# Young768/KungFu

Measured on AMD Instinct MI355X. Metric: images/sec/GPU ResNet-50 SynchronousSGD at 1/2/4/8 MI355X; scaling efficiency, higher is better.
Workload: dtype bf16

## Files before the change

csrc/kernels/bind_bn.cpp:

```cpp
#include "bind_util.hpp"

#include <vector>

using namespace kfb;

namespace {

const auto kCL = at::MemoryFormat::ChannelsLast;

kfk::BNShape bn_shape(const at::Tensor &x, const char *op) {
    check_cl4(x, op, "x", kAnyGpu);
    const int C = narrow(x.size(1), op, "x");
    TORCH_CHECK(kfk::bn_supported_channels(C), op, ": unsupported channel count ", C);
    return kfk::BNShape{x.numel() / C, C};
}

struct BNCommon {
    float *rm = nullptr, *rv = nullptr;
    int64_t *nbt = nullptr;
};

BNCommon bn_common(const char *op, int C, const Dev &dev, const at::Tensor &weight, const at::Tensor &bias,
                   const OptTensor &running_mean, const OptTensor &running_var, const OptTensor &num_batches,
                   bool training) {
    check_dense(weight, op, "weight", dev, at::kFloat, C);
    check_dense(bias, op, "bias", dev, at::kFloat, C);
    BNCommon b;
    if (has(running_mean)) {
        TORCH_CHECK(has(running_var), op, ": running_var missing");
        b.rm = running_mean->data_ptr<float>();
        b.rv = running_var->data_ptr<float>();
    }
    TORCH_CHECK(training || b.rm, op, ": eval mode needs running stats");
    if (training && has(num_batches)) {
        TORCH_CHECK(num_batches->scalar_type() == at::kLong && num_batches->numel() == 1 && num_batches->is_cuda(),
                    op, ": num_batches_tracked must be a 1-element int64 GPU tensor");
        b.nbt = num_batches->data_ptr<int64_t>();
    }
    return b;
}

at::Tensor bn_dy(at::Tensor dy, const at::Tensor &x, int C, int64_t *ld) {
    *ld = 0;
    if (dy.is_contiguous(kCL)) return dy;
    const int64_t s3 = dy.stride(3);
    const bool slice = dy.stride(1) == 1 && s3 >= C && s3 % 8 == 0 && dy.stride(2) == dy.size(3) * s3 &&
                       dy.stride(0) == dy.size(2) * dy.size(3) * s3 &&
                       reinterpret_cast<uintptr_t>(dy.data_ptr()) % 16 == 0;
    if (!slice) return dy.contiguous(kCL);
    *ld = s3;
    return dy;
}

void check_bn_dy(const at::Tensor &dy, const at::Tensor &x, const char *op) {
    TORCH_CHECK(dy.scalar_type() == at::kBFloat16 && dy.sizes() == x.sizes() && dy.device() == x.device(), op,
                ": dy must be a bf16 tensor of x's shape on its device");
}

std::vector<std::vector<at::Tensor>> bn_finalize_multi(std::vector<at::Tensor> xs, std::vector<at::Tensor> sums,
                                                       std::vector<at::Tensor> weights, std::vector<at::Tensor> biases,
                                                       std::vector<OptTensor> running_means,
                                                       std::vector<OptTensor> running_vars,
                                                       std::vector<OptTensor> num_batches,
                                                       std::vector<double> momentum, std::vector<double> eps) {
    const char *op = "bn_finalize_multi";
    const size_t n = xs.size();
    TORCH_CHECK(n >= 1 && n <= static_cast<size_t>(kfk::kBnFinMax) && sums.size() == n && weights.size() == n &&
                    biases.size() == n && running_means.size() == n && running_vars.size() == n &&
                    num_batches.size() == n && momentum.size() == n && eps.size() == n,
                "bn_finalize_multi: 1..8 BNs, every list of the same length");
    kfk::BnFinBatch b{};
    b.n = static_cast<int>(n);
    for (size_t i = 0; i < n; ++i) {
        auto sh = bn_shape(xs[i], op);
        const Dev dev = xs[0].device();
        TORCH_CHECK(xs[i].device() == *dev, "bn_finalize_multi: xs must be on one device");
        auto c = bn_common(op, sh.channels, dev, weights[i], biases[i], running_means[i], running_vars[i],
                           num_batches[i], true);
        kfk::BnFinDesc &d = b.d[i];
        TORCH_CHECK(sums[i].defined(), "bn_finalize_multi: sums must be defined");
        d.sums = stats_ptr(sums[i], op, sh.channels, dev, "sums");
        d.gamma = weights[i].data_ptr<float>(), d.beta = biases[i].data_ptr<float>();
        d.run_mean = c.rm, d.run_var = c.rv, d.nbt = c.nbt;
        d.rows = sh.rows, d.C = sh.channels;
        d.momentum = static_cast<float>(momentum[i]), d.eps = static_cast<float>(eps[i]);
    }
    std::vector<std::vector<at::Tensor>> out;
    for (size_t i = 0; i < n; ++i) {
        kfk::BnFinDesc &d = b.d[i];
        auto fopt = xs[i].options().dtype(at::kFloat);
        at::Tensor mean = at::empty({d.C}, fopt), invstd = at::empty({d.C}, fopt), coef = at::empty({2 * d.C}, fopt);
        d.mean = mean.data_ptr<float>(), d.invstd = invstd.data_ptr<float>(), d.coef = coef.data_ptr<float>();
        out.push_back({mean, invstd, coef});
    }
    c10::DeviceGuard gd(xs[0].device());
    kfk::launch_bn_sums_finalize_multi(b, stream_of(xs[0], 0));
    return out;
}

std::vector<at::Tensor> bn_forward(at::Tensor x, OptTensor res, at::Tensor weight, at::Tensor bias,
                                   OptTensor running_mean, OptTensor running_var, double momentum, double eps,
                                   bool training, bool relu, OptTensor num_batches, OptTensor sums, OptTensor res_coef,
                                   bool apply, OptTensor out, c10::optional<std::vector<at::Tensor>> pre) {
    const char *op = "bn_forward";
    auto sh = bn_shape(x, op);
    const int C = sh.channels;
    const Dev dev = x.device();
    auto b = bn_common(op, C, dev, weight, bias, running_mean, running_var, num_batches, training);
    const uint16_t *rp = nullptr;
    if (has(res)) {
        check_cl4(*res, op, "res", dev, x.sizes());
        rp = bf16(*res);
    }
    const float *rc = nullptr;
    if (has(res_coef)) {
        TORCH_CHECK(rp, "bn_forward: res_coef (the residual BN's f32 [scale(C); shift(C)]) needs res");
        check_dense(*res_coef, op, "res_coef", dev, at::kFloat, 2 * C);
        rc = res_coef->data_ptr<float>();
    }
    int64_t y_ld = 0;
    if (has(out)) {
        TORCH_CHECK(apply && !rp && relu && out->scalar_type() == at::kBFloat16 && out->sizes() == x.sizes() &&
                        out->stride(1) == 1 && out->stride(3) >= C && out->stride(3) % 8 == 0 &&
                        out->stride(2) == out->size(3) * out->stride(3) &&
                        out->stride(0) == out->size(2) * out->stride(2) &&
                        reinterpret_cast<uintptr_t>(out->data_ptr()) % 16 == 0 && out->device() == x.device(),
                    "bn_forward: out must be a 16-byte aligned channel slice of a channels_last bf16 tensor "
                    "(BN+ReLU, no residual)");
        y_ld = out->stride(3);
    }
    const bool prefin = pre.has_value();
    if (prefin) {
        TORCH_CHECK(pre->size() == 3 && training && has(sums), "bn_forward: pre must be (mean, invstd, coef) with sums");
        check_dense((*pre)[0], op, "pre[0]", dev, at::kFloat, C);
        check_dense((*pre)[1], op, "pre[1]", dev, at::kFloat, C);
        check_dense((*pre)[2], op, "pre[2]", dev, at::kFloat, 2 * C);
    }
    double *sp = training ? stats_ptr(sums, op, C, dev, "sums") : nullptr;

    c10::DeviceGuard gd(x.device());
    auto fopt = x.options().dtype(at::kFloat);
    at::Tensor y;
    if (has(out)) y = *out;
    else if (apply) y = at::empty_like(x, kCL);
    at::Tensor mean, invstd, coef;
    if (prefin) mean = (*pre)[0], invstd = (*pre)[1], coef = (*pre)[2];
    else mean = at::empty({C}, fopt), invstd = at::empty({C}, fopt), coef = at::empty({2 * C}, fopt);
    at::Tensor mask;
    if (apply && rp && relu) mask = at::empty({sh.rows * (C / 8)}, x.options().dtype(at::kByte));
    at::Tensor partial;
    if (training && !sp) partial = at::empty({2 * static_cast<int64_t>(kfk::bn_num_chunks(sh)) * C}, fopt);
    kfk::launch_bn_forward(bf16(x), rp, weight.data_ptr<float>(), bias.data_ptr<float>(),
                           apply ? bf16_mut(y) : nullptr, mask.defined() ? mask.data_ptr<uint8_t>() : nullptr, sh, relu,
                           training, b.rm, b.rv, static_cast<float>(momentum), static_cast<float>(eps),
                           partial.defined() ? partial.data_ptr<float>() : nullptr, mean.data_ptr<float>(),
                           invstd.data_ptr<float>(), coef.data_ptr<float>(), b.nbt, stream_of(x, 0), sp, rc, apply, y_ld,
                           prefin);
    return {y, mean, invstd, coef, mask};
}

std::vector<at::Tensor> bn_backward(at::Tensor dy, at::Tensor x, at::Tensor mean, at::Tensor invstd, at::Tensor weight,
                                    at::Tensor fcoef, OptTensor mask, bool relu, bool training, bool want_dres,
                                    OptTensor sums, OptTensor dres_x, OptTensor dres_sums) {
    const char *op = "bn_backward";
    auto sh = bn_shape(x, op);
    const int C = sh.channels;
    const Dev dev = x.device();
    check_bn_dy(dy, x, op);
    check_dense(mean, op, "mean", dev, at::kFloat, C);
    check_dense(invstd, op, "invstd", dev, at::kFloat, C);
    check_dense(weight, op, "weight", dev, at::kFloat, C);
    check_dense(fcoef, op, "fcoef", dev, at::kFloat, 2 * C);
    const uint8_t *mp = nullptr;
    if (has(mask)) {
        check_dense(*mask, op, "mask", dev, at::kByte, sh.rows * (C / 8));
        mp = mask->data_ptr<uint8_t>();
    }
    double *sp = stats_ptr(sums, op, C, dev, "sums");
    const uint16_t *dsx = nullptr;
    double *dsp = nullptr;
    if (has(dres_x)) {
        TORCH_CHECK(want_dres && has(dres_sums),
                    "bn_backward: dres_x (second BN's input) needs want_dres and its f64 sums workspace dres_sums");
        check_cl4(*dres_x, op, "dres_x", dev, x.sizes());
        dsx = bf16(*dres_x);
        dsp = stats_ptr(dres_sums, op, C, dev, "dres_sums");
    }
    c10::DeviceGuard gd(x.device());
    int64_t dy_ld;
    dy = bn_dy(dy, x, C, &dy_ld);
    auto fopt = x.options().dtype(at::kFloat);
    auto dx = at::empty_like(x, kCL);
    at::Tensor dres;
    if (want_dres) dres = at::empty_like(x, kCL);
    at::Tensor dw = at::empty({C}, fopt), db = at::empty({C}, fopt), coef = at::empty({3 * C}, fopt);
    at::Tensor partial;
    if (!sp) partial = at::empty({2 * static_cast<int64_t>(kfk::bn_num_chunks(sh)) * C}, fopt);
    kfk::launch_bn_backward(bf16(dy), bf16(x), fcoef.data_ptr<float>(), mp, mean.data_ptr<float>(),
                            invstd.data_ptr<float>(), weight.data_ptr<float>(), sh, relu, training,
                            partial.defined() ? partial.data_ptr<float>() : nullptr, dw.data_ptr<float>(),
                            db.data_ptr<float>(), coef.data_ptr<float>(), bf16_mut(dx),
                            want_dres ? bf16_mut(dres) : nullptr, stream_of(x, 0), sp, dsx, dsp, dy_ld);
    return {dx, dres, dw, db};
}

std::vector<std::vector<at::Tensor>> bn_backward_multi(std::vector<at::Tensor> dys, std::vector<at::Tensor> xs,
                                                       std::vector<at::Tensor> means, std::vector<at::Tensor> invstds,
                                                       std::vector<at::Tensor> weights, std::vector<at::Tensor> fcoefs) {
    const char *op = "bn_backward_multi";
    const size_t n = xs.size();
    TORCH_CHECK(n >= 1 && n <= static_cast<size_t>(kfk::kBnFinMax) && dys.size() == n && means.size() == n &&
                    invstds.size() == n && weights.size() == n && fcoefs.size() == n,
                "bn_backward_multi: 1..8 BNs, every list of the same length");
    struct Piece {
        at::Tensor dy, dx, dw, db, coef, partial;
        int64_t ld;
        kfk::BNShape sh;
    };
    std::vector<Piece> ps(n);
    const Dev dev = xs[0].device();
    for (size_t i = 0; i < n; ++i) {
        ps[i].sh = bn_shape(xs[i], op);
        const int C = ps[i].sh.channels;
        TORCH_CHECK(xs[i].device() == *dev, "bn_backward_multi: xs must be on one device");
        check_bn_dy(dys[i], xs[i], op);
        check_dense(fcoefs[i], op, "fcoefs", dev, at::kFloat, 2 * C);
        check_dense(means[i], op, "means", dev, at::kFloat, C);
        check_dense(invstds[i], op, "invstds", dev, at::kFloat, C);
        check_dense(weights[i], op, "weights", dev, at::kFloat, C);
    }
    c10::DeviceGuard gd(xs[0].device());
    kfk::BnBwdFinBatch fb{};
    fb.n = static_cast<int>(n);
    for (size_t i = 0; i < n; ++i) {
        Piece &p = ps[i];
        const int C = p.sh.channels;
        p.dy = bn_dy(dys[i], xs[i], C, &p.ld);
        auto fopt = xs[i].options().dtype(at::kFloat);
        p.dx = at::empty_like(xs[i], kCL);
        p.dw = at::empty({C}, fopt), p.db = at::empty({C}, fopt), p.coef = at::empty({3 * C}, fopt);
        p.partial = at::empty({2 * static_cast<int64_t>(kfk::bn_num_chunks(p.sh)) * C}, fopt);
        kfk::BnBwdFinDesc &d = fb.d[i];
        d.partial = p.partial.data_ptr<float>();
        d.nchunks = kfk::bn_num_chunks(p.sh), d.C = C, d.rows = p.sh.rows;
        d.gamma = weights[i].data_ptr<float>(), d.mean = means[i].data_ptr<float>(), d.invstd = invstds[i].data_ptr<float>();
        d.dgamma = p.dw.data_ptr<float>(), d.dbeta = p.db.data_ptr<float>(), d.coef = p.coef.data_ptr<float>();
    }
    const hipStream_t st = stream_of(xs[0], 0);
    for (int phase : {1, 2}) {
        if (phase == 2) kfk::launch_bn_bwd_finalize_multi(fb, st);
        for (size_t i = 0; i < n; ++i) {
            Piece &p = ps[i];
            kfk::launch_bn_backward(bf16(p.dy), bf16(xs[i]), fcoefs[i].data_ptr<float>(), nullptr,
                                    means[i].data_ptr<float>(), invstds[i].data_ptr<float>(),
                                    weights[i].data_ptr<float>(), p.sh, true, true, p.partial.data_ptr<float>(),
                                    p.dw.data_ptr<float>(), p.db.data_ptr<float>(), p.coef.data_ptr<float>(),
                                    bf16_mut(p.dx), nullptr, st, nullptr, nullptr, nullptr, p.ld, phase);
        }
    }
    std::vector<std::vector<at::Tensor>> out;
    for (auto &p : ps) out.push_back({p.dx, p.dw, p.db});
    return out;
}

std::vector<at::Tensor> bn_pool_forward(at::Tensor x, at::Tensor weight, at::Tensor bias, OptTensor running_mean,
                                        OptTensor running_var, double momentum, double eps, bool training,
                                        OptTensor num_batches, OptTensor sums) {
    const char *op = "bn_pool_forward";
    auto sh = bn_shape(x, op);
    const int C = sh.channels;
    const Dev dev = x.device();
    const int H = narrow(x.size(2), op, "x"), W = narrow(x.size(3), op, "x");
    TORCH_CHECK(kfk::bn_pool_supported(sh, H, W), "bn_pool_forward: unsupported shape");
    double *sp = training ? stats_ptr(sums, op, C, dev, "sums") : nullptr;
    auto b = bn_common(op, C, dev, weight, bias, running_mean, running_var, num_batches, training);
    c10::DeviceGuard gd(x.device());
    auto fopt = x.options().dtype(at::kFloat);
    const int OH = kfk::pool_out(H), OW = kfk::pool_out(W);
    auto yp = at::empty({x.size(0), C, OH, OW}, x.options().memory_format(kCL));
    auto arg = at::empty({x.size(0) * OH * OW * C}, x.options().dtype(at::kByte));
    auto mean = at::empty({C}, fopt), invstd = at::empty({C}, fopt), coef = at::empty({2 * C}, fopt);
    at::Tensor partial, xarg;
    if (training) {
        partial = at::empty({2 * static_cast<int64_t>(kfk::bn_num_chunks(sh)) * C}, fopt);
        xarg = at::empty_like(yp, kCL);
    }
    kfk::launch_bn_pool_forward(bf16(x), weight.data_ptr<float>(), bias.data_ptr<float>(), bf16_mut(yp),
                                arg.data_ptr<uint8_t>(), sh, H, W, training, b.rm, b.rv, static_cast<float>(momentum),
                                static_cast<float>(eps), training ? partial.data_ptr<float>() : nullptr,
                                mean.data_ptr<float>(), invstd.data_ptr<float>(), coef.data_ptr<float>(), b.nbt,
                                stream_of(x, 0), sp, xarg.defined() ? bf16_mut(xarg) : nullptr);
    return {yp, mean, invstd, coef, arg, xarg};
}

std::vector<at::Tensor> bn_pool_backward(at::Tensor dyp, at::Tensor arg, at::Tensor x, at::Tensor mean,
                                         at::Tensor invstd, at::Tensor weight, at::Tensor fcoef, bool training,
                                         OptTensor xarg, bool apply) {
    const char *op = "bn_pool_backward";
    auto sh = bn_shape(x, op);
    const int C = sh.channels;
    const Dev dev = x.device();
    const int H = narrow(x.size(2), op, "x"), W = narrow(x.size(3), op, "x");
    const int64_t psz[4] = {x.size(0), C, kfk::pool_out(H), kfk::pool_out(W)};
    TORCH_CHECK(dyp.scalar_type() == at::kBFloat16 && dyp.sizes() == at::IntArrayRef(psz) && dyp.device() == x.device(),
                "bn_pool_backward: dy must be the pooled [N, C, PH, PW] bf16 gradient on x's device");
    check_dense(arg, op, "arg", dev, at::kByte, dyp.numel());
    check_dense(mean, op, "mean", dev, at::kFloat, C);
    check_dense(invstd, op, "invstd", dev, at::kFloat, C);
    check_dense(weight, op, "weight", dev, at::kFloat, C);
    check_dense(fcoef, op, "fcoef", dev, at::kFloat, 2 * C);
    const bool pooled = training && has(xarg);
    if (pooled) check_cl4(*xarg, op, "xarg", dev, psz);
    c10::DeviceGuard gd(x.device());
    if (!dyp.is_contiguous(kCL)) dyp = dyp.contiguous(kCL);
    auto fopt = x.options().dtype(at::kFloat);
    auto dx = apply ? at::empty_like(x, kCL) : at::empty({0}, x.options());
    auto dw = at::empty({C}, fopt), db = at::empty({C}, fopt), coef = at::empty({3 * C}, fopt);
    auto partial = at::empty({2 * static_cast<int64_t>(kfk::bn_num_chunks(sh)) * C}, fopt);
    at::Tensor sums;
    if (pooled) sums = at::zeros({2 * C * kfk::kStatSlots}, x.options().dtype(at::kDouble));
    kfk::launch_bn_pool_backward(bf16(dyp), arg.data_ptr<uint8_t>(), bf16(x), fcoef.data_ptr<float>(),
                                 mean.data_ptr<float>(), invstd.data_ptr<float>(), weight.data_ptr<float>(), sh, H, W,
                                 training, partial.data_ptr<float>(), dw.data_ptr<float>(), db.data_ptr<float>(),
                                 coef.data_ptr<float>(), apply ? bf16_mut(dx) : nullptr, stream_of(x, 0),
                                 pooled ? bf16(*xarg) : nullptr, pooled ? sums.data_ptr<double>() : nullptr, apply);
    return {dx, dw, db, coef};
}

}

void bind_bn(py::module_ &m) {
    m.def("bn_supported_channels", &kfk::bn_supported_channels);
    m.def("bn_forward", &bn_forward,
          "fused NHWC BN(+residual)(+ReLU) forward -> (y, mean, invstd, coef, relu mask or None)", py::arg("x"),
          py::arg("res"), py::arg("weight"), py::arg("bias"), py::arg("running_mean"), py::arg("running_var"),
          py::arg("momentum"), py::arg("eps"), py::arg("training"), py::arg("relu"),
          py::arg("num_batches") = py::none(), py::arg("sums") = py::none(), py::arg("res_coef") = py::none(),
          py::arg("apply") = true, py::arg("out") = py::none(), py::arg("pre") = py::none());
    m.def("bn_backward_multi", &bn_backward_multi,
          "backward of several BN+ReLUs (slices of one concatenation's gradient): one batched finalize");
    m.def("bn_finalize_multi", &bn_finalize_multi,
          "batched sums-finalize of several training BNs in one launch -> [[mean, invstd, coef], ...]");
    m.def("bn_backward", &bn_backward, "fused NHWC BN(+residual)(+ReLU) backward -> (dx, dres, dweight, dbias)",
          py::arg("dy"), py::arg("x"), py::arg("mean"), py::arg("invstd"), py::arg("weight"), py::arg("fcoef"),
          py::arg("mask"), py::arg("relu"), py::arg("training"), py::arg("want_dres"), py::arg("sums") = py::none(),
          py::arg("dres_x") = py::none(), py::arg("dres_sums") = py::none());
    m.def("bn_pool_supported", [](int64_t C, int64_t H, int64_t W) {
        const char *op = "bn_pool_supported";
        return kfk::bn_pool_supported(kfk::BNShape{H * W, narrow(C, op, "C")}, narrow(H, op, "H"), narrow(W, op, "W"));
    });
    m.def("bn_pool_forward", &bn_pool_forward,
          "stem BN+ReLU+MaxPool(3,2,1) forward -> (y_pool, mean, invstd, coef, argmax)", py::arg("x"),
          py::arg("weight"), py::arg("bias"), py::arg("running_mean"), py::arg("running_var"), py::arg("momentum"),
          py::arg("eps"), py::arg("training"), py::arg("num_batches") = py::none(), py::arg("sums") = py::none());
    m.def("bn_pool_backward", &bn_pool_backward, "stem BN+ReLU+MaxPool backward -> (dx, dweight, dbias, coef)",
          py::arg("dy"), py::arg("arg"), py::arg("x"), py::arg("mean"), py::arg("invstd"), py::arg("weight"),
          py::arg("fcoef"), py::arg("training"), py::arg("xarg") = py::none(), py::arg("apply") = true);
}
```

csrc/kernels/bind_conv.cpp:

```cpp
#include "bind_util.hpp"

#include <array>
#include <optional>
#include <vector>

using namespace kfb;

namespace {

const auto kCL = at::MemoryFormat::ChannelsLast;

at::Tensor conv(at::Tensor x, at::Tensor w, int64_t stride, OptTensor stats, OptTensor out, int64_t variant,
                OptTensor bn_x, OptTensor bn_fcoef, OptTensor bn_mask, OptTensor bias, bool gate, OptTensor acc_mask,
                bool acc_even) {
    const char *op = "conv";
    check_cl4(x, op, "x", kAnyGpu);
    const Dev dev = x.device();
    check_cl4(w, op, "w", dev);
    TORCH_CHECK(w.size(2) == w.size(3) && w.size(1) == x.size(1), "conv: w must be [Cout, Cin, KS, KS] with x's Cin");
    const auto [N, C, H, W] = dims4(x, op, "x");
    const int K = narrow(w.size(0), op, "w"), ks = narrow(w.size(2), op, "w"), st = narrow(stride, op, "stride");
    TORCH_CHECK(kfk::conv_supported(C, K, ks, st), "conv: unsupported channels/kernel/stride");
    const int pad = (ks - 1) / 2;
    const int OH = (H + 2 * pad - ks) / st + 1, OW = (W + 2 * pad - ks) / st + 1;
    TORCH_CHECK(OH > 0 && OW > 0, "conv: empty output");
    check_extent32(op, "x", {N, H, W, C});
    check_extent32(op, "the output", {N, OH, OW, K});
    const int64_t ysz[4] = {N, K, OH, OW};
    const int64_t ynumel = c10::multiply_integers(at::IntArrayRef(ysz));
    double *sp = stats_ptr(stats, op, K, dev);
    const bool accum = has(out), bwd = has(bn_x);
    kfk::EpiArgs ea;
    ea.stats = sp;
    int epi = accum ? kfk::kEpiAccum : 0;
    if (has(bias)) {
        TORCH_CHECK(!accum && !sp && !bwd && !gate, "conv: bias epilogue excludes out/stats/bn_x/gate");
        check_dense(*bias, op, "bias", dev, at::kBFloat16, K);
        ea.bias = bf16(*bias);
        epi = kfk::kEpiBiasRelu;
    } else if (gate) {
        TORCH_CHECK(!accum && sp && bwd && !has(bn_mask) && !has(bn_fcoef),
                    "conv: gate needs stats and bn_x (the ReLU output), no out/bn_mask/bn_fcoef");
        check_cl4(*bn_x, op, "bn_x", dev, ysz);
        ea.bx = bf16(*bn_x);
        epi = kfk::kEpiGate;
    } else if (bwd) {
        epi |= bn_bwd_epilogue(op, ea, ysz, K, dev, sp, bn_x, bn_fcoef, bn_mask);
    } else if (sp) {
        epi |= kfk::kEpiFwdStats;
    }
    TORCH_CHECK(!(epi & kfk::kEpiFwdStats) || !(epi & kfk::kEpiAccum), "conv: stats + accumulate unsupported");
    if (has(acc_mask)) {
        TORCH_CHECK(accum && !(epi & kfk::kEpiBwdCoef), "conv: acc_mask needs out and excludes bn_fcoef");
        check_dense(*acc_mask, op, "acc_mask", dev, at::kByte, ynumel / 8);
        ea.amask = acc_mask->data_ptr<uint8_t>();
        epi |= kfk::kEpiAccMask;
    }
    if (acc_even) {
        TORCH_CHECK(accum && st == 1 && !(epi & (kfk::kEpiAccMask | kfk::kEpiBwdCoef)),
                    "conv: acc_even needs out, stride 1 and no acc_mask / bn_fcoef");
        epi |= kfk::kEpiAccEven;
    }
    const int var = narrow(variant, op, "variant");
    c10::DeviceGuard gd(x.device());
    auto y = out_or_empty(out, ysz, x.options().memory_format(kCL), op).first;
    kfk::launch_conv(bf16(x), bf16(w), bf16_mut(y), N, H, W, C, K, ks, st, ea, epi, stream_of(x, 0), var);
    return y;
}

std::vector<at::Tensor> gemm(at::Tensor x, at::Tensor w, OptTensor bias, OptTensor out, OptTensor gelu_u,
                             OptTensor stats, int64_t variant) {
    const char *op = "gemm";
    TORCH_CHECK(x.dim() == 2, "gemm: x must be 2-D [M, K]");
    check_dense(x, op, "x", kAnyGpu, at::kBFloat16, x.numel());
    const Dev dev = x.device();
    TORCH_CHECK(w.dim() == 2 && w.size(1) == x.size(1), "gemm: w must be 2-D [N, K] with x's K");
    check_dense(w, op, "w", dev, at::kBFloat16, w.numel());
    const int64_t M = x.size(0), K = x.size(1), N = w.size(0);
    TORCH_CHECK(M < (int64_t(1) << 31) && K < (int64_t(1) << 31) && N < (int64_t(1) << 31) &&
                    kfk::gemm_supported(static_cast<int>(M), static_cast<int>(K), static_cast<int>(N)),
                "gemm: unsupported shape (K, N multiples of 64)");
    kfk::EpiArgs ea;
    int epi = 0;
    auto check_mn = [&](const at::Tensor &t, const char *what) {
        TORCH_CHECK(t.dim() == 2 && t.size(0) == M && t.size(1) == N, "gemm: ", what, " must be 2-D [M, N]");
        check_dense(t, op, what, dev, at::kBFloat16, M * N);
    };
    if (has(out)) {
        TORCH_CHECK(!has(bias) && !has(gelu_u), "gemm: out (accumulate) excludes bias / gelu_u");
        check_mn(*out, "out");
        epi = kfk::kEpiAccum;
    }
    if (has(bias)) {
        check_dense(*bias, op, "bias", dev, at::kBFloat16, N);
        ea.bias = bf16(*bias);
        epi = kfk::kEpiBias;
    }
    if (has(gelu_u)) {
        TORCH_CHECK(epi == 0, "gemm: gelu_u excludes bias / out");
        check_mn(*gelu_u, "gelu_u");
        TORCH_CHECK(has(stats), "gemm: stats must be given with gelu_u (the f64 kStatSlots x 2 x N workspace)");
        ea.bx = bf16(*gelu_u);
        ea.stats = stats_ptr(stats, op, N, dev);
        epi = kfk::kEpiGeluGrad;
    }
    const int var = narrow(variant, op, "variant");
    c10::DeviceGuard gd(x.device());
    auto y = out_or_empty(out, {M, N}, x.options(), op).first;
    kfk::launch_gemm(bf16(x), bf16(w), bf16_mut(y), static_cast<int>(M), static_cast<int>(K), static_cast<int>(N), ea,
                     epi, stream_of(x, 0), var);
    return {y};
}

at::Tensor conv_dgrad_s2(at::Tensor dy, at::Tensor wt, int64_t ks, OptTensor stats, OptTensor bn_x, OptTensor bn_fcoef,
                         OptTensor bn_mask, int64_t variant, int64_t dh, int64_t dw, int64_t pad) {
    const char *op = "conv_dgrad_s2";
    check_cl4(dy, op, "dy", kAnyGpu);
    const Dev dev = dy.device();
    TORCH_CHECK(ks == 1 || ks == 3, "conv_dgrad_s2: ks must be 1 or 3");
    check_cl4(wt, op, "wt", dev);
    check_cl4(wt, op, "wt", dev, {wt.size(0), dy.size(1), ks, ks});
    const auto [N, K, OH, OW] = dims4(dy, op, "dy");
    const int C = narrow(wt.size(0), op, "wt");
    if (dh <= 0) {
        TORCH_CHECK(kfk::conv_supported(K, C, static_cast<int>(ks), 1), "conv_dgrad_s2: unsupported channels");
        dh = 2 * OH, dw = 2 * OW, pad = ks == 3 ? 1 : 0;
    } else {
        TORCH_CHECK(ks == 3 && (pad == 0 || pad == 1) && K % 8 == 0 && C % 8 == 0 && K >= 16 && C >= 16 && dw > 0 &&
                        (dh + 2 * pad - 3) / 2 + 1 == OH && (dw + 2 * pad - 3) / 2 + 1 == OW,
                    "conv_dgrad_s2: dh/dw/pad do not match a 3x3 stride-2 convolution of dy's size (channels % 8)");
    }
    check_extent32(op, "dx", {N, dh, dw, C});
    const int64_t dxsz[4] = {N, C, dh, dw};
    kfk::EpiArgs ea;
    int epi = 0;
    if (has(bn_x)) {
        TORCH_CHECK(ks == 3, "conv_dgrad_s2: BN sums need every pixel (ks = 3)");
        epi = bn_bwd_epilogue(op, ea, dxsz, C, dev, stats_ptr(stats, op, C, dev), bn_x, bn_fcoef, bn_mask);
    }
    const int var = narrow(variant, op, "variant");
    c10::DeviceGuard gd(dy.device());
    auto dx = at::empty(dxsz, dy.options().memory_format(kCL));
    kfk::launch_conv_dgrad_s2(bf16(dy), bf16(wt), bf16_mut(dx), N, OH, OW, K, C, static_cast<int>(ks), ea, epi,
                              stream_of(dy, 0), var, static_cast<int>(dh), static_cast<int>(dw), static_cast<int>(pad));
    return dx;
}

at::Tensor wgrad_launch(const char *op, const at::Tensor &dy, const at::Tensor &x, const kfk::WgradPlan &plan,
                        OptTensor out, bool accumulate, bool atomics) {
    const kfk::WgradShape &sh = plan.shape;
    const bool f32 = has(out) && out->scalar_type() == at::kFloat;
    c10::DeviceGuard gd(x.device());
    auto dw = out_or_empty(out, {sh.Cout, sh.Cin, sh.kh, sh.kw},
                           x.options().dtype(f32 ? at::kFloat : at::kBFloat16).memory_format(kCL), op).first;
    at::Tensor ws;
    if (plan.ws_floats > 0) ws = at::empty({plan.ws_floats}, x.options().dtype(at::kFloat));
    kfk::launch_conv_wgrad(bf16(dy), bf16(x), dw.data_ptr(), plan.ws_floats > 0 ? ws.data_ptr<float>() : nullptr, plan,
                           f32, accumulate, stream_of(x, 0), atomics);
    return dw;
}

void wgrad_check(const char *op, const at::Tensor &dy, const at::Tensor &x, const kfk::WgradShape &sh) {
    check_cl4(dy, op, "dy", x.device(), {sh.N, sh.Cout, sh.OH(), sh.OW()});
    check_extent32(op, "x", {sh.N, sh.H, sh.W, sh.Cin});
    check_extent32(op, "dy", {sh.N, sh.OH(), sh.OW(), sh.Cout});
}

at::Tensor conv_wgrad(at::Tensor dy, at::Tensor x, int64_t ks, int64_t stride, OptTensor out, bool accumulate,
                      int64_t variant, int64_t splits, bool atomics) {
    const char *op = "conv_wgrad";
    check_cl4(x, op, "x", kAnyGpu);
    check_cl4(dy, op, "dy", Dev(x.device()));
    const auto [N, C, H, W] = dims4(x, op, "x");
    const auto sh = kfk::wgrad_square_shape(N, H, W, C, narrow(dy.size(1), op, "dy"), narrow(ks, op, "ks"),
                                            narrow(stride, op, "stride"));
    TORCH_CHECK(kfk::conv_wgrad_supported(sh.Cin, sh.Cout, sh.kh, sh.stride), "conv_wgrad: unsupported channels/kernel/stride");
    wgrad_check(op, dy, x, sh);
    TORCH_CHECK(has(out) || !accumulate, "conv_wgrad: accumulate needs out");
    const auto plan = kfk::conv_wgrad_plan(sh, kfk::WgradFamily::Square, narrow(variant, op, "variant"),
                                           narrow(splits, op, "splits"));
    return wgrad_launch(op, dy, x, plan, out, accumulate, atomics);
}

at::Tensor conv_wgrad_rect(at::Tensor dy, at::Tensor x, int64_t kh, int64_t kw, int64_t stride, int64_t ph, int64_t pw,
                           int64_t variant) {
    const char *op = "conv_wgrad_rect";
    check_cl4(x, op, "x", kAnyGpu);
    check_cl4(dy, op, "dy", Dev(x.device()));
    const auto [N, C, H, W] = dims4(x, op, "x");
    const kfk::WgradShape sh{N, H, W, C, narrow(dy.size(1), op, "dy"), narrow(kh, op, "kh"), narrow(kw, op, "kw"),
                             narrow(ph, op, "ph"), narrow(pw, op, "pw"), narrow(stride, op, "stride")};
    TORCH_CHECK(kfk::conv_wgrad_rect_supported(sh.Cin, sh.Cout, sh.kh, sh.kw, sh.stride) && sh.ph >= 0 && sh.pw >= 0 &&
                    sh.ph < sh.kh && sh.pw < sh.kw,
                "conv_wgrad_rect: unsupported channels/window/stride/padding");
    wgrad_check(op, dy, x, sh);
    const auto plan = kfk::conv_wgrad_plan(sh, kfk::WgradFamily::Rect, narrow(variant, op, "variant"));
    return wgrad_launch(op, dy, x, plan, OptTensor(), false, true);
}

at::Tensor conv_flip_weight(at::Tensor w) {
    const char *op = "conv_flip_weight";
    check_cl4(w, op, "w", kAnyGpu);
    const auto [K, C, kh, kw] = dims4(w, op, "w");
    c10::DeviceGuard gd(w.device());
    auto wt = at::empty({C, K, kh, kw}, w.options().memory_format(kCL));
    kfk::launch_conv_flip_weight_taps(bf16(w), bf16_mut(wt), K, C, kh * kw, stream_of(w, 0));
    return wt;
}

at::Tensor conv_rect(at::Tensor x, at::Tensor w, int64_t stride, int64_t ph, int64_t pw, OptTensor stats, OptTensor out,
                     OptTensor bn_x, OptTensor bn_fcoef) {
    const char *op = "conv_rect";
    check_cl4(x, op, "x", kAnyGpu);
    const Dev dev = x.device();
    check_cl4(w, op, "w", dev);
    TORCH_CHECK(w.size(1) == x.size(1), "conv_rect: w must be [Cout, Cin, KH, KW] with x's Cin");
    const auto [N, C, H, W] = dims4(x, op, "x");
    const auto [K, wc, kh, kw] = dims4(w, op, "w");
    const int st = narrow(stride, op, "stride"), PH = narrow(ph, op, "ph"), PW = narrow(pw, op, "pw");
    TORCH_CHECK(kfk::conv_rect_supported(C, K, kh, kw, st) && PH >= 0 && PW >= 0 && PH < kh && PW < kw,
                "conv_rect: unsupported channels/window/stride/padding");
    const int OH = (H + 2 * PH - kh) / st + 1, OW = (W + 2 * PW - kw) / st + 1;
    TORCH_CHECK(OH > 0 && OW > 0, "conv_rect: empty output");
    check_extent32(op, "x", {N, H, W, C});
    check_extent32(op, "the output", {N, OH, OW, K});
    const int64_t ysz[4] = {N, K, OH, OW};
    kfk::EpiArgs ea;
    ea.stats = stats_ptr(stats, op, K, dev);
    int epi = ea.stats ? kfk::kEpiFwdStats : 0;
    const bool bwd = has(bn_x);
    if (bwd) epi = bn_bwd_epilogue(op, ea, ysz, K, dev, ea.stats, bn_x, bn_fcoef, OptTensor());
    TORCH_CHECK(!has(out) || epi == 0 || bwd, "conv_rect: out must not be combined with forward stats");
    c10::DeviceGuard gd(x.device());
    auto [y, accum] = out_or_empty(out, ysz, x.options().memory_format(kCL), op);
    if (accum) epi |= kfk::kEpiAccum;
    kfk::launch_conv_rect(bf16(x), bf16(w), bf16_mut(y), N, H, W, C, K, kh, kw, PH, PW, st, ea, epi, stream_of(x, 0));
    return y;
}

void conv_flip_weights(std::vector<at::Tensor> srcs, std::vector<at::Tensor> dsts) {
    const char *op = "conv_flip_weights";
    TORCH_CHECK(srcs.size() == dsts.size(), "conv_flip_weights: length mismatch");
    if (srcs.empty()) return;
    c10::DeviceGuard gd(srcs[0].device());
    auto s = stream_of(srcs[0], 0);
    kfk::FlipTable tab;
    tab.start[0] = 0;
    for (size_t i = 0; i < srcs.size(); ++i) {
        const auto &w = srcs[i];
        const auto &d = dsts[i];
        check_cl4(w, op, "srcs", i ? Dev(srcs[0].device()) : kAnyGpu);
        check_cl4(d, op, "dsts", w.device(), {w.size(1), w.size(0), w.size(2), w.size(3)});
        const auto [K, C, kh, kw] = dims4(w, op, "srcs");
        const int k = tab.n;
        tab.src[k] = bf16(w);
        tab.dst[k] = bf16_mut(d);
        tab.cout[k] = K;
        tab.cin[k] = C;
        tab.taps[k] = kh * kw;
        tab.start[k + 1] = tab.start[k] + w.numel();
        tab.n = k + 1;
        if (tab.n == kfk::FlipTable::kMax) {
            kfk::launch_conv_flip_multi(tab, s);
            tab.n = 0;
        }
    }
    kfk::launch_conv_flip_multi(tab, s);
}

}

void bind_conv(py::module_ &m) {
    m.def("conv", &conv, "1x1/3x3 NHWC bf16 convolution (MFMA implicit GEMM) with fused BN-statistics and "
          "accumulate epilogues", py::arg("x"), py::arg("w"), py::arg("stride") = 1, py::arg("stats") = py::none(),
          py::arg("out") = py::none(), py::arg("variant") = -1, py::arg("bn_x") = py::none(),
          py::arg("bn_fcoef") = py::none(), py::arg("bn_mask") = py::none(), py::arg("bias") = py::none(),
          py::arg("gate") = false, py::arg("acc_mask") = py::none(), py::arg("acc_even") = false);
    m.def("conv_variants", &kfk::conv_variants);
    m.def("conv_supported", &kfk::conv_supported);
    m.attr("conv_stat_slots") = kfk::kStatSlots;
    m.def("conv_rect", &conv_rect, "KH x KW NHWC bf16 convolution with zero padding (MFMA implicit GEMM; "
          "Inception-v3 windows) with an optional BN-statistics epilogue", py::arg("x"), py::arg("w"),
          py::arg("stride") = 1, py::arg("ph") = 0, py::arg("pw") = 0, py::arg("stats") = py::none(),
          py::arg("out") = py::none(), py::arg("bn_x") = py::none(), py::arg("bn_fcoef") = py::none());
    m.def("conv_rect_supported", &kfk::conv_rect_supported);
    m.def("gemm", &gemm, "linear layer x @ w^T on the MFMA kernel with bias / GELU-gradient(+bias-gradient "
          "sums) / accumulate epilogues", py::arg("x"), py::arg("w"), py::arg("bias") = py::none(),
          py::arg("out") = py::none(), py::arg("gelu_u") = py::none(),
          py::arg("stats") = py::none(), py::arg("variant") = -1);
    m.def("gemm_supported", &kfk::gemm_supported);
    m.def("conv_dgrad_s2", &conv_dgrad_s2, "data gradient of a stride-2 1x1/3x3 NHWC bf16 convolution (parity-phase "
          "MFMA implicit GEMMs)", py::arg("dy"), py::arg("wt"), py::arg("ks"), py::arg("stats") = py::none(),
          py::arg("bn_x") = py::none(), py::arg("bn_fcoef") = py::none(), py::arg("bn_mask") = py::none(),
          py::arg("variant") = -1, py::arg("dh") = 0, py::arg("dw") = 0, py::arg("pad") = 1);
    m.def("conv_wgrad_rect", &conv_wgrad_rect, "weight gradient of a KH x KW padded NHWC bf16 convolution "
          "(split-K MFMA GEMM, any channel count % 8)", py::arg("dy"), py::arg("x"), py::arg("kh"), py::arg("kw"),
          py::arg("stride") = 1, py::arg("ph") = 0, py::arg("pw") = 0, py::arg("variant") = -1);
    m.def("conv_wgrad", &conv_wgrad, "weight gradient of the 1x1/3x3 NHWC bf16 convolution (split-K MFMA GEMM)",
          py::arg("dy"), py::arg("x"), py::arg("ks"), py::arg("stride") = 1, py::arg("out") = py::none(),
          py::arg("accumulate") = false, py::arg("variant") = -1, py::arg("splits") = -1,
          py::arg("atomics") = true);
    m.def("conv_wgrad_supported", &kfk::conv_wgrad_supported);
    m.def("conv_wgrad_rect_supported", &kfk::conv_wgrad_rect_supported);
    m.def("conv_wgrad_variants", [] { return kfk::kWgradSquareVariants; });
    m.def("conv_wgrad_rows_rect_supported", [](int N, int H, int W, int Cin, int Cout, int kh, int kw, int ph, int pw,
                                               int stride) {
        return kfk::conv_wgrad_rows_rect_supported({N, H, W, Cin, Cout, kh, kw, ph, pw, stride});
    }, "a row-image weight-gradient kernel covers this multi-tap window (args: N, H, W, Cin, Cout, kh, kw, ph, pw, stride)");
    m.def("conv_wgrad_rows_rect_auto", [](int N, int H, int W, int Cin, int Cout, int kh, int kw, int ph, int pw,
                                          int stride) {
        return kfk::conv_wgrad_rows_rect_auto({N, H, W, Cin, Cout, kh, kw, ph, pw, stride});
    }, "the row-image variant conv_wgrad_rect(..., WGRAD_ROWS_AUTO) picks for this shape (args: N, H, W, Cin, Cout, kh, "
       "kw, ph, pw, stride)");
    m.def("conv_wgrad_plan", [](int N, int H, int W, int Cin, int Cout, int ks, int stride, int variant, int splits,
                                std::optional<std::array<int, 4>> window) {
        const auto p = window ? kfk::conv_wgrad_plan({N, H, W, Cin, Cout, (*window)[0], (*window)[1], (*window)[2],
                                                      (*window)[3], stride}, kfk::WgradFamily::Rect, variant)
                              : kfk::conv_wgrad_plan(kfk::wgrad_square_shape(N, H, W, Cin, Cout, ks, stride),
                                                     kfk::WgradFamily::Square, variant, splits);
        return py::make_tuple(p.variant, p.splits, p.kps, p.ws_floats, kfk::wgrad_kernel_name(p.kernel));
    }, "(variant, splits, kps, ws_floats, kernel) of conv_wgrad's plan, or with window = (kh, kw, ph, pw) of "
       "conv_wgrad_rect's (ks and splits are then unused)", py::arg("N"), py::arg("H"), py::arg("W"), py::arg("Cin"),
          py::arg("Cout"), py::arg("ks"), py::arg("stride"), py::arg("variant") = -1, py::arg("splits") = -1,
          py::arg("window") = py::none());
    m.def("conv_wgrad_route", [](int N, int H, int W, int Cin, int Cout, int kh, int kw, int ph, int pw, int stride) {
        const auto r = kfk::conv_wgrad_route({N, H, W, Cin, Cout, kh, kw, ph, pw, stride});
        return py::make_tuple(kfk::wgrad_route_name(r.route), r.variant, r.max_pixels);
    }, "(route, variant, max_pixels): 'library', or the family ('square': conv_wgrad, 'rect': conv_wgrad_rect) and the "
       "variant code that take this convolution's weight gradient, and the output pixels one launch handles",
          py::arg("N"), py::arg("H"), py::arg("W"), py::arg("Cin"), py::arg("Cout"), py::arg("kh"), py::arg("kw"),
          py::arg("ph"), py::arg("pw"), py::arg("stride"));
    m.attr("WGRAD_AUTO") = static_cast<int>(kfk::kWgradAuto);
    m.attr("WGRAD_TILE_128x128") = static_cast<int>(kfk::kWgradTile128x128);
    m.attr("WGRAD_TILE_128x64") = static_cast<int>(kfk::kWgradTile128x64);
    m.attr("WGRAD_TILE_64x128") = static_cast<int>(kfk::kWgradTile64x128);
    m.attr("WGRAD_TILE_64x64") = static_cast<int>(kfk::kWgradTile64x64);
    m.attr("WGRAD_TILE_256x128") = static_cast<int>(kfk::kWgradTile256x128);
    m.attr("WGRAD_TILE_128x256") = static_cast<int>(kfk::kWgradTile128x256);
    m.attr("WGRAD_ROWS") = static_cast<int>(kfk::kWgradRows);
    m.attr("WGRAD_TILE_256x256") = static_cast<int>(kfk::kWgradTile256x256);
    m.attr("WGRAD_RING_32x2") = static_cast<int>(kfk::kWgradRing32x2);
    m.attr("WGRAD_RING_32x3") = static_cast<int>(kfk::kWgradRing32x3);
    m.attr("WGRAD_RING_32x4") = static_cast<int>(kfk::kWgradRing32x4);
    m.attr("WGRAD_RING_64x3") = static_cast<int>(kfk::kWgradRing64x3);
    m.attr("WGRAD_RING_64x4") = static_cast<int>(kfk::kWgradRing64x4);
    m.attr("WGRAD_ROWS_AUTO") = static_cast<int>(kfk::kWgradRowsAuto);
    m.def("conv_flip_weight", &conv_flip_weight, "w[co,ci,kh,kw] -> w[ci,co,KS-1-kh,KS-1-kw] (data-gradient weights)");
    m.def("conv_flip_weights", &conv_flip_weights, "multi-tensor conv_flip_weight into preallocated outputs");
}
```

csrc/kernels/bind_util.hpp:

```cpp
#pragma once

#include <ATen/hip/HIPContext.h>
#include <c10/core/DeviceGuard.h>
#include <torch/extension.h>

#include "kernels.hpp"

#include <climits>
#include <initializer_list>
#include <utility>

namespace kfb {

using OptTensor = c10::optional<at::Tensor>;
using Dev = c10::optional<at::Device>;
inline const Dev kAnyGpu{};

inline int dtype_code(const at::Tensor &t) {
    switch (t.scalar_type()) {
    case at::kByte: return 0;
    case at::kChar: return 4;
    case at::kInt: return 6;
    case at::kLong: return 7;
    case at::kHalf: return 8;
    case at::kBFloat16: return 9;
    case at::kFloat: return 10;
    case at::kDouble: return 11;
    case at::kBool: return 12;
    default: TORCH_CHECK(false, "kungfu_amd._hip: unsupported dtype ", t.scalar_type());
    }
    return -1;
}

inline hipStream_t stream_of(const at::Tensor &t, int64_t stream) {
    if (stream) return reinterpret_cast<hipStream_t>(stream);
    return c10::hip::getCurrentHIPStream(t.device().index()).stream();
}

inline void check_gpu(const at::Tensor &t, const char *name) {
    TORCH_CHECK(t.is_cuda(), name, " must be a GPU tensor");
    TORCH_CHECK(t.is_contiguous(), name, " must be contiguous");
}

inline void hcheck(hipError_t e, const char *what) {
    TORCH_CHECK(e == hipSuccess, "hip ", what, ": ", hipGetErrorString(e));
}

inline bool has(const OptTensor &o) { return o && o->defined(); }

inline const uint16_t *bf16(const at::Tensor &t) { return reinterpret_cast<const uint16_t *>(t.data_ptr()); }
inline uint16_t *bf16_mut(const at::Tensor &t) { return reinterpret_cast<uint16_t *>(t.data_ptr()); }

inline int narrow(int64_t v, const char *op, const char *what) {
    TORCH_CHECK(v >= INT_MIN && v <= INT_MAX, op, ": ", what, " must be a 32-bit integer, got ", v);
    return static_cast<int>(v);
}

inline bool on_dev(const at::Tensor &t, const Dev &dev) { return dev ? t.device() == *dev : t.is_cuda(); }
inline const char *where(const Dev &dev) { return dev ? "on the leading tensor's device" : "on a GPU"; }

inline void check_cl4(const at::Tensor &t, const char *op, const char *name, const Dev &dev,
                      at::ScalarType dt = at::kBFloat16) {
    TORCH_CHECK(t.dim() == 4 && t.scalar_type() == dt && t.is_contiguous(at::MemoryFormat::ChannelsLast) &&
                    on_dev(t, dev),
                op, ": ", name, " must be a 4-D channels_last ", dt, " tensor ", where(dev));
}

inline void check_cl4(const at::Tensor &t, const char *op, const char *name, const Dev &dev, at::IntArrayRef nchw,
                      at::ScalarType dt = at::kBFloat16) {
    TORCH_CHECK(t.dim() == 4 && t.scalar_type() == dt && t.is_contiguous(at::MemoryFormat::ChannelsLast) &&
                    on_dev(t, dev) && t.sizes() == nchw,
                op, ": ", name, " must be a ", nchw, " channels_last ", dt, " tensor ", where(dev));
}

struct Dims4 {
    int n, c, h, w;
};
inline Dims4 dims4(const at::Tensor &t, const char *op, const char *name) {
    return {narrow(t.size(0), op, name), narrow(t.size(1), op, name), narrow(t.size(2), op, name),
            narrow(t.size(3), op, name)};
}

inline void check_dense(const at::Tensor &t, const char *op, const char *name, const Dev &dev, at::ScalarType dt,
                        int64_t numel, bool at_least = false) {
    TORCH_CHECK(t.scalar_type() == dt && t.is_contiguous() && (at_least ? t.numel() >= numel : t.numel() == numel) &&
                    on_dev(t, dev),
                op, ": ", name, " must be a contiguous ", dt, " tensor of ", at_least ? "at least " : "", numel,
                " elements ", where(dev));
}

inline double *stats_ptr(const OptTensor &o, const char *op, int64_t C, const Dev &dev, const char *name = "stats") {
    if (!has(o)) return nullptr;
    check_dense(*o, op, name, dev, at::kDouble, kfk::kStatSlots * 2 * C);
    return o->data_ptr<double>();
}

inline void check_extent32(const char *op, const char *name, std::initializer_list<int64_t> dims) {
    int64_t n = 1;
    for (int64_t d : dims) {
        TORCH_CHECK(d >= 0 && d <= INT_MAX, op, ": ", name, " too large for 32-bit offsets");
        n *= d;
        TORCH_CHECK(n <= INT_MAX, op, ": ", name, " too large for 32-bit offsets");
    }
}

inline int bn_bwd_epilogue(const char *op, kfk::EpiArgs &ea, at::IntArrayRef y_sizes, int64_t K, const Dev &dev,
                           double *stats, const OptTensor &bn_x, const OptTensor &bn_fcoef, const OptTensor &bn_mask) {
    if (!has(bn_x)) return 0;
    TORCH_CHECK(stats, op, ": stats must be given with bn_x (it receives the BN-backward sums)");
    check_cl4(*bn_x, op, "bn_x", dev, y_sizes);
    ea.stats = stats;
    ea.bx = bf16(*bn_x);
    if (has(bn_mask)) {
        check_dense(*bn_mask, op, "bn_mask", dev, at::kByte, c10::multiply_integers(y_sizes) / 8);
        ea.bmask = bn_mask->data_ptr<uint8_t>();
        return kfk::kEpiBwdBits;
    }
    TORCH_CHECK(has(bn_fcoef), op, ": bn_fcoef must be given with bn_x (forward [scale; shift], f32) unless bn_mask is");
    check_dense(*bn_fcoef, op, "bn_fcoef", dev, at::kFloat, 2 * K, true);
    ea.fcoef = bn_fcoef->data_ptr<float>();
    return kfk::kEpiBwdCoef;
}

inline std::pair<at::Tensor, bool> out_or_empty(const OptTensor &out, at::IntArrayRef sizes, const at::TensorOptions &opt,
                                                const char *op, const char *name = "out") {
    if (!has(out)) return {at::empty(sizes, opt), false};
    const auto dt = c10::typeMetaToScalarType(opt.dtype());
    if (opt.memory_format_opt() == at::MemoryFormat::ChannelsLast) check_cl4(*out, op, name, opt.device(), sizes, dt);
    else check_dense(*out, op, name, opt.device(), dt, c10::multiply_integers(sizes));
    return {*out, true};
}

}
```

csrc/kernels/bn.hip:

```cpp
#include "bn_fin.hpp"
#include "common.hpp"
#include "kernels.hpp"

#include <cstdlib>
#include <stdexcept>

namespace kfk {

namespace {

__device__ __forceinline__ void unpack8(const uint4 &v, float (&f)[8]) {
    const uint32_t w[4] = {v.x, v.y, v.z, v.w};
#pragma unroll
    for (int i = 0; i < 4; ++i) {
        f[2 * i] = __uint_as_float(w[i] << 16);
        f[2 * i + 1] = __uint_as_float(w[i] & 0xffff0000u);
    }
}

__device__ __forceinline__ uint4 pack8(const float (&f)[8]) {
    uint32_t w[4];
#pragma unroll
    for (int i = 0; i < 4; ++i)
        w[i] = pack_bf16x2(f[2 * i], f[2 * i + 1]);
// ... 328 lines not shown
        sc[k] = coef[cv * 8 + k];
        sh[k] = coef[C + cv * 8 + k];
    }
    const int64_t stride = static_cast<int64_t>(gridDim.x) * bn_threads<CVEC>();
    for (int64_t i = tid; i < nout_vec; i += stride) {
        const int64_t p = i / CVEC;
        const int ow = static_cast<int>(p % OW);
        const int64_t t = p / OW;
        const int oh = static_cast<int>(t % OH);
        const int64_t n = t / OH;
        float best[8], xb[8];
        uint32_t a[8];
#pragma unroll
        for (int k = 0; k < 8; ++k) {
            best[k] = -1.f;
            a[k] = 0;
            xb[k] = 0.f;
        }
#pragma unroll
        for (int kh = 0; kh < 3; ++kh) {
            const int h = 2 * oh - 1 + kh;
            if (h < 0 || h >= H) continue;
#pragma unroll
            for (int kw = 0; kw < 3; ++kw) {
                const int w = 2 * ow - 1 + kw;
                if (w < 0 || w >= W) continue;
                float f[8];
                unpack8(x[((n * H + h) * W + w) * CVEC + cv], f);
#pragma unroll
                for (int k = 0; k < 8; ++k) {
                    float v = f[k] * sc[k] + sh[k];
                    v = v > 0.f ? v : 0.f;
                    if (v > best[k]) {
                        best[k] = v;
                        a[k] = kh * 3 + kw;
                        xb[k] = f[k];
                    }
                }
            }
        }
        yp[i] = pack8(best);
        arg[i] = make_uint2(a[0] | (a[1] << 8) | (a[2] << 16) | (a[3] << 24),
                            a[4] | (a[5] << 8) | (a[6] << 16) | (a[7] << 24));
        if (xarg) xarg[i] = pack8(xb);
    }
}

template <int CVEC>
__global__ __launch_bounds__(kBlock) void bn_pool_bwd_sums_kernel(const uint4 *__restrict__ dy,
                                                                  const uint4 *__restrict__ xarg,
                                                                  const float *__restrict__ fcoef,
                                                                  double *__restrict__ sums, int64_t nvec) {
    constexpr int C = CVEC * 8, NT = bn_threads<CVEC>();
    const int64_t tid = static_cast<int64_t>(blockIdx.x) * NT + threadIdx.x;
    const int cv = static_cast<int>(tid % CVEC);
    float sc[8], sh[8], s1[8], s2[8];
#pragma unroll
    for (int k = 0; k < 8; ++k) {
        sc[k] = fcoef[cv * 8 + k];
        sh[k] = fcoef[C + cv * 8 + k];
        s1[k] = s2[k] = 0.f;
    }
    const int64_t stride = static_cast<int64_t>(gridDim.x) * NT;
    for (int64_t i = tid; i < nvec; i += stride) {
        float g[8], xv[8];
        unpack8(dy[i], g);
        unpack8(xarg[i], xv);
#pragma unroll
        for (int k = 0; k < 8; ++k) {
            const float dz = xv[k] * sc[k] + sh[k] > 0.f ? g[k] : 0.f;
            s1[k] += dz;
            s2[k] += dz * xv[k];
        }
    }
    __shared__ float red[kBlock][17];
    if (threadIdx.x < NT) {
#pragma unroll
        for (int k = 0; k < 8; ++k) {
            red[threadIdx.x][k] = s1[k];
            red[threadIdx.x][8 + k] = s2[k];
        }
    }
    __syncthreads();
    for (int c = threadIdx.x; c < C; c += NT) {
        const int cvi = c >> 3, k = c & 7;
        double a1 = 0, a2 = 0;
        for (int u = cvi; u < NT; u += CVEC) {
            a1 += red[u][k];
            a2 += red[u][8 + k];
        }
        double *sl = sums + (blockIdx.x % kStatSlots) * 2 * C;
        atomicAdd(sl + c, a1);
        atomicAdd(sl + C + c, a2);
    }
}


struct DirectGrad {
    const uint4 *dy;
    bool nt = false;
    using Raw = uint4;
    template <int CVEC>
    __device__ __forceinline__ Raw fetch(int64_t i, int64_t , int ) const {
        return ld16(dy + i, nt);
    }
    __device__ __forceinline__ void get(const Raw &r, float (&g)[8]) const { unpack8(r, g); }
};

struct StridedGrad {
    const uint4 *dy;
    int64_t ldv;
    using Raw = uint4;
    template <int CVEC>
    __device__ __forceinline__ Raw fetch(int64_t , int64_t row, int cv) const {
        return dy[row * ldv + cv];
    }
    __device__ __forceinline__ void get(const Raw &r, float (&g)[8]) const { unpack8(r, g); }
};

struct PoolGrad {
    const uint4 *dyp;
    const uint2 *arg;
    int H, W, OH, OW;
    uint64_t m_hw, m_w;
    struct Raw {
        uint2 am[4];
        uint4 d[4];
        uint32_t kk;
    };
    __device__ __forceinline__ void get(const Raw &r, float (&g)[8]) const {
#pragma unroll
        for (int k = 0; k < 8; ++k) g[k] = 0.f;
#pragma unroll
        for (int c = 0; c < 4; ++c) {
            const uint32_t kk = (r.kk >> (8 * c)) & 0xffu;
            float d[8];
            unpack8(r.d[c], d);
#pragma unroll
            for (int k = 0; k < 8; ++k) {
                const uint32_t ak = ((k < 4 ? r.am[c].x : r.am[c].y) >> (8 * (k & 3))) & 0xffu;
                g[k] += ak == kk ? d[k] : 0.f;
            }
        }
    }
    template <int CVEC>
    __device__ __forceinline__ Raw fetch(int64_t , int64_t row64, int cv) const {
        const uint32_t row = static_cast<uint32_t>(row64);
        const uint32_t hw = static_cast<uint32_t>(H) * static_cast<uint32_t>(W);
        const uint32_t n = static_cast<uint32_t>((static_cast<uint64_t>(row) * m_hw) >> 40);
        const uint32_t rem = row - n * hw;
        const int h = static_cast<int>((static_cast<uint64_t>(rem) * m_w) >> 40);
        const int w = static_cast<int>(rem) - h * W;
        const int oh_lo = h >> 1, oh_hi = (h + 1) >> 1;
        const int ow_lo = w >> 1, ow_hi = (w + 1) >> 1;
        Raw r;
        r.kk = 0;
        const uint32_t base = (n * OH) * OW;
#pragma unroll
        for (int c = 0; c < 4; ++c) {
            const int oh = (c & 2) ? oh_hi : oh_lo, ow = (c & 1) ? ow_hi : ow_lo;
            const bool ok = (!(c & 2) || oh_hi != oh_lo) && (!(c & 1) || ow_hi != ow_lo) && oh < OH && ow < OW;
            const uint32_t kk = ok ? static_cast<uint32_t>((h + 1 - 2 * oh) * 3 + (w + 1 - 2 * ow)) : 0xffu;
            const uint32_t o = ((base + (ok ? oh : oh_lo) * OW + (ok ? ow : ow_lo)) * CVEC) + cv;
            r.am[c] = arg[o];
            r.d[c] = dyp[o];
            r.kk |= kk << (8 * c);
        }
        return r;
    }
    template <int CVEC>
    __device__ __forceinline__ void load(int64_t i, int64_t row, int cv, float (&g)[8]) const {
        get(fetch<CVEC>(i, row, cv), g);
    }
};

enum ReluMode : int { RM_NONE = 0, RM_COEF = 1, RM_BITS = 2 };

template <int RM>
__device__ __forceinline__ void relu_gate(float (&g)[8], const float (&xv)[8], const float (&sc)[8],
                                          const float (&sh)[8], const uint8_t *mask, int64_t i) {
    if (RM == RM_COEF) {
#pragma unroll
        for (int k = 0; k < 8; ++k) g[k] = (xv[k] * sc[k] + sh[k]) > 0.f ? g[k] : 0.f;
    } else if (RM == RM_BITS) {
        const uint32_t m = mask[i];
#pragma unroll
        for (int k = 0; k < 8; ++k) g[k] = ((m >> k) & 1u) ? g[k] : 0.f;
    }
}

template <int CVEC, int RM>
__device__ __forceinline__ void load_fwd_coef(const float *fcoef, int cv, float (&sc)[8], float (&sh)[8]) {
    constexpr int C = CVEC * 8;
#pragma unroll
    for (int k = 0; k < 8; ++k) {
        sc[k] = RM == RM_COEF ? fcoef[cv * 8 + k] : 0.f;
        sh[k] = RM == RM_COEF ? fcoef[C + cv * 8 + k] : 0.f;
    }
}


template <int CVEC, int RM, class G>
__global__ __launch_bounds__(kBlock) void bn_bwd_reduce_kernel(G grad, const uint4 *__restrict__ x,
                                                               const float *__restrict__ fcoef,
                                                               const uint8_t *__restrict__ mask, int64_t rows,
                                                               int64_t rows_per_chunk, float *partial, int ntm = 0) {
    const bool ntl = ntm & 1;
    constexpr int RPI = kBlock / CVEC;
    constexpr int C = CVEC * 8;
    __shared__ float lds[2 * RPI * C];
    const int tid = threadIdx.x, cv = tid % CVEC, r0 = tid / CVEC;
    float sc[8], sh[8];
    load_fwd_coef<CVEC, RM>(fcoef, cv, sc, sh);
    float acc[2][8];
#pragma unroll
    for (int k = 0; k < 8; ++k) acc[0][k] = acc[1][k] = 0.f;
    const int64_t r_begin = static_cast<int64_t>(blockIdx.x) * rows_per_chunk;
    int64_t r_end = r_begin + rows_per_chunk;
    if (r_end > rows) r_end = rows;
    int64_t r = r_begin + r0;
    constexpr int U = 4;
    for (; r + (U - 1) * RPI < r_end; r += U * RPI) {
        typename G::Raw gr[U];
        uint4 xr[U];
#pragma unroll
        for (int u = 0; u < U; ++u) {
            const int64_t row = r + u * RPI, i = row * CVEC + cv;
            gr[u] = grad.template fetch<CVEC>(i, row, cv);
            xr[u] = ld16(x + i, ntl);
        }
#pragma unroll
        for (int u = 0; u < U; ++u) {
            float g[8], xv[8];
            grad.get(gr[u], g);
            unpack8(xr[u], xv);
            relu_gate<RM>(g, xv, sc, sh, mask, (r + u * RPI) * CVEC + cv);
#pragma unroll
            for (int k = 0; k < 8; ++k) {
                acc[0][k] += g[k];
                acc[1][k] += g[k] * xv[k];
            }
        }
    }
    for (; r < r_end; r += RPI) {
        const int64_t i = r * CVEC + cv;
        float g[8], xv[8];
        grad.get(grad.template fetch<CVEC>(i, r, cv), g);
        unpack8(x[i], xv);
        relu_gate<RM>(g, xv, sc, sh, mask, i);
#pragma unroll
        for (int k = 0; k < 8; ++k) {
            acc[0][k] += g[k];
            acc[1][k] += g[k] * xv[k];
        }
    }
    reduce_to_partials<CVEC, 2>(acc, lds, partial, C, gridDim.x);
}

__global__ __launch_bounds__(kBlock) void bn_bwd_finalize(const float *partial, int nchunks, int C, int64_t rows,
                                                          const float *gamma, const float *mean, const float *invstd,
                                                          float *dgamma, float *dbeta, float *coef, bool training) {
    const int c = blockIdx.x * kFoldCh + threadIdx.x % kFoldCh, kl = threadIdx.x / kFoldCh;
    double sums[2];
    fold_partials<2>(partial, nchunks, C, c, kl, sums);
    if (kl != 0 || c >= C) return;
    double db = sums[0], dg = static_cast<double>(invstd[c]) * (sums[1] - static_cast<double>(mean[c]) * db);
    dgamma[c] = static_cast<float>(dg);
    dbeta[c] = static_cast<float>(db);
    float g = gamma ? gamma[c] : 1.f;
    float a = g * invstd[c];
    if (training) {
        float inv_m = 1.f / static_cast<float>(rows);
        float k2 = -a * static_cast<float>(dg) * invstd[c] * inv_m;
        coef[c] = a;
        coef[C + c] = k2;
        coef[2 * C + c] = -a * static_cast<float>(db) * inv_m - k2 * mean[c];
    } else {
        coef[c] = a;
        coef[C + c] = 0.f;
        coef[2 * C + c] = 0.f;
    }
}

__global__ __launch_bounds__(kBlock) void bn_bwd_finalize_multi(BnBwdFinBatch b) {
    const BnBwdFinDesc &d = b.d[blockIdx.y];
    const int C = d.C;
    if (static_cast<int>(blockIdx.x) * kFoldCh >= C) return;
    const int c = blockIdx.x * kFoldCh + threadIdx.x % kFoldCh, kl = threadIdx.x / kFoldCh;
    double sums[2];
    fold_partials<2>(d.partial, d.nchunks, C, c, kl, sums);
    if (kl != 0 || c >= C) return;
    double db = sums[0], dg = static_cast<double>(d.invstd[c]) * (sums[1] - static_cast<double>(d.mean[c]) * db);
    d.dgamma[c] = static_cast<float>(dg);
    d.dbeta[c] = static_cast<float>(db);
    float g = d.gamma ? d.gamma[c] : 1.f;
    float a = g * d.invstd[c];
    const float inv_m = 1.f / static_cast<float>(d.rows);
    const float k2 = -a * static_cast<float>(dg) * d.invstd[c] * inv_m;
    d.coef[c] = a;
    d.coef[C + c] = k2;
    d.coef[2 * C + c] = -a * static_cast<float>(db) * inv_m - k2 * d.mean[c];
}

__global__ __launch_bounds__(256) void bn_bwd_finalize_sums(double *__restrict__ sums, int C, int64_t rows,
                                                            const float *__restrict__ gamma,
                                                            const float *__restrict__ mean,
                                                            const float *__restrict__ invstd, float *dgamma,
                                                            float *dbeta, float *coef, bool training) {
    const int c = blockIdx.x * blockDim.x + threadIdx.x;
    if (c >= C) return;
    const float g = gamma ? gamma[c] : 1.f, mu = mean[c], is = invstd[c];
    const double *sp = sums + c;
    double v0[kStatSlots], v1[kStatSlots];
#pragma unroll
    for (int k = 0; k < kStatSlots; ++k) {
        v0[k] = sp[k * 2 * C];
        v1[k] = sp[k * 2 * C + C];
    }
    double s0 = 0, s1 = 0;
#pragma unroll
    for (int k = 0; k < kStatSlots; ++k) {
        s0 += v0[k];
        s1 += v1[k];
    }
    double *zp = sums + c;
#pragma unroll
    for (int k = 0; k < kStatSlots; ++k) {
        zp[k * 2 * C] = 0.0;
        zp[k * 2 * C + C] = 0.0;
    }
    bn_fin_bwd_channel(c, C, s0, s1, rows, g, mu, is, dgamma, dbeta, coef, training);
}


template <int CVEC, int RM, bool DRES, class G>
__global__ __launch_bounds__(kBlock) void bn_bwd_apply_kernel(G grad, const uint4 *__restrict__ x,
                                                              const float *__restrict__ fcoef,
                                                              const uint8_t *__restrict__ mask,
                                                              const float *__restrict__ coef, uint4 *__restrict__ dx,
                                                              uint4 *__restrict__ dres, int64_t nvec,
                                                              const uint4 *__restrict__ dsx = nullptr,
                                                              double *__restrict__ dsums = nullptr, int ntm = 0) {
    constexpr int C = CVEC * 8;
    const bool ntl = ntm & 1, nts = ntm & 2;
    const int64_t tid = static_cast<int64_t>(blockIdx.x) * bn_threads<CVEC>() + threadIdx.x;
    const int cv = static_cast<int>(tid % CVEC);
    float k1[8], k2[8], k3[8], sc[8], sh[8];
#pragma unroll
    for (int k = 0; k < 8; ++k) {
        k1[k] = coef[cv * 8 + k];
        k2[k] = coef[C + cv * 8 + k];
        k3[k] = coef[2 * C + cv * 8 + k];
    }
    load_fwd_coef<CVEC, RM>(fcoef, cv, sc, sh);
    float d1[8], d2[8];
#pragma unroll
    for (int k = 0; k < 8; ++k) d1[k] = d2[k] = 0.f;
    const bool dsum = DRES && dsx != nullptr;
    const int64_t stride = static_cast<int64_t>(gridDim.x) * bn_threads<CVEC>();
    constexpr int U = 2;
    for (int64_t i0 = tid; i0 < nvec; i0 += U * stride) {
        typename G::Raw gr[U];
        uint4 xr[U];
#pragma unroll
        for (int u = 0; u < U; ++u) {
            const int64_t i = i0 + u * stride;
            if (i < nvec) {
                gr[u] = grad.template fetch<CVEC>(i, i / CVEC, cv);
                xr[u] = ld16(x + i, ntl);
            }
        }
#pragma unroll
        for (int u = 0; u < U; ++u) {
            const int64_t i = i0 + u * stride;
            if (i >= nvec) break;
            float g[8], xv[8];
            grad.get(gr[u], g);
            unpack8(xr[u], xv);
            relu_gate<RM>(g, xv, sc, sh, mask, i);
            if (DRES) {
                const uint4 gr = pack8(g);
                st16(dres + i, gr, nts);
                if (dsum) {
                    float gq[8], sx[8];
                    unpack8(gr, gq);
                    unpack8(dsx[i], sx);
#pragma unroll
                    for (int k = 0; k < 8; ++k) {
                        d1[k] += gq[k];
                        d2[k] += gq[k] * sx[k];
                    }
                }
            }
            float o[8];
#pragma unroll
            for (int k = 0; k < 8; ++k) o[k] = k1[k] * g[k] + k2[k] * xv[k] + k3[k];
            st16(dx + i, pack8(o), nts);
        }
    }
    if (dsum) {
        constexpr int NT = bn_threads<CVEC>();
        __shared__ float red[kBlock][17];
        if (threadIdx.x < NT) {
#pragma unroll
            for (int k = 0; k < 8; ++k) {
                red[threadIdx.x][k] = d1[k];
                red[threadIdx.x][8 + k] = d2[k];
            }
        }
        __syncthreads();
        for (int c = threadIdx.x; c < C; c += NT) {
            const int cvi = c >> 3, k = c & 7;
            double a1 = 0, a2 = 0;
            for (int u = cvi; u < NT; u += CVEC) {
                a1 += red[u][k];
                a2 += red[u][8 + k];
            }
            double *sl = dsums + (blockIdx.x % kStatSlots) * 2 * C;
            atomicAdd(sl + c, a1);
            atomicAdd(sl + C + c, a2);
        }
    }
}

template <typename F>
void dispatch_cvec(int cvec, F &&f) {
    switch (cvec) {
    case 4: f(std::integral_constant<int, 4>()); break;
    case 6: f(std::integral_constant<int, 6>()); break;
    case 10: f(std::integral_constant<int, 10>()); break;
    case 12: f(std::integral_constant<int, 12>()); break;
    case 20: f(std::integral_constant<int, 20>()); break;
    case 24: f(std::integral_constant<int, 24>()); break;
    case 40: f(std::integral_constant<int, 40>()); break;
    case 48: f(std::integral_constant<int, 48>()); break;
    case 56: f(std::integral_constant<int, 56>()); break;
    case 8: f(std::integral_constant<int, 8>()); break;
    case 16: f(std::integral_constant<int, 16>()); break;
    case 32: f(std::integral_constant<int, 32>()); break;
    case 64: f(std::integral_constant<int, 64>()); break;
    case 128: f(std::integral_constant<int, 128>()); break;
    case 256: f(std::integral_constant<int, 256>()); break;
    default: break;
    }
}

int apply_grid(int64_t nvec, int cvec) {
    const int nt = (kBlock / cvec) * cvec;
    int64_t g = (nvec + nt - 1) / nt;
    if (g > kMaxGrid) g = kMaxGrid;
    if (g < 1) g = 1;
    return static_cast<int>(g);
}

void launch_stats(const uint16_t *x, BNShape sh, const float *gamma, const float *beta, float *run_mean,
                  float *run_var, float momentum, float eps, float *partial, float *mean, float *invstd, float *coef,
                  int64_t *num_batches, hipStream_t s) {
    const int C = sh.channels, cvec = C / 8;
    Chunking ch = chunking(sh);
    dispatch_cvec(cvec, [&](auto cvc) {
        constexpr int CV = decltype(cvc)::value;
        bn_stats_kernel<CV><<<ch.nchunks, bn_threads<CV>(), 0, s>>>(reinterpret_cast<const uint4 *>(x), sh.rows,
                                                          ch.rows_per_chunk, partial);
    });
    bn_stats_finalize<<<(C + kFoldCh - 1) / kFoldCh, kBlock, 0, s>>>(partial, ch.nchunks, C, sh.rows, gamma, beta,
                                                                     mean, invstd, run_mean, run_var, momentum, eps,
                                                                     coef, num_batches);
}

template <class G>
void launch_backward_impl(G grad, const uint16_t *x, const float *fcoef, const uint8_t *mask, const float *mean,
                          const float *invstd, const float *gamma, BNShape sh, int rm, bool training, float *partial,
                          float *dgamma, float *dbeta, float *coef, uint16_t *dx, uint16_t *dres, hipStream_t s,
                          double *sums = nullptr, const uint16_t *dres_x = nullptr, double *dres_sums = nullptr,
                          int phase = 0) {
    const int C = sh.channels, cvec = C / 8;
    const int64_t nvec = sh.rows * cvec;
    Chunking ch = chunking(sh);
    const uint4 *xx = reinterpret_cast<const uint4 *>(x);
    if (phase == 2) {
    } else if (sums) {
        bn_bwd_finalize_sums<<<(C + 255) / 256, 256, 0, s>>>(sums, C, sh.rows, gamma, mean, invstd, dgamma, dbeta,
                                                             coef, training);
    } else {
    dispatch_cvec(cvec, [&](auto cvc) {
        constexpr int CV = decltype(cvc)::value;
        auto go = [&](auto rmc) {
            constexpr int RM = decltype(rmc)::value;
            bn_bwd_reduce_kernel<CV, RM, G>
                <<<ch.nchunks, bn_threads<CV>(), 0, s>>>(grad, xx, fcoef, mask, sh.rows, ch.rows_per_chunk, partial,
                                                          bn_nt_mode());
        };
        if (rm == RM_COEF) go(std::integral_constant<int, RM_COEF>());
        else if (rm == RM_BITS) go(std::integral_constant<int, RM_BITS>());
        else go(std::integral_constant<int, RM_NONE>());
    });
    if (phase == 1) return;
    bn_bwd_finalize<<<(C + kFoldCh - 1) / kFoldCh, kBlock, 0, s>>>(partial, ch.nchunks, C, sh.rows, gamma, mean,
                                                                   invstd, dgamma, dbeta, coef, training);
    }
    if (phase == 3) return;
    const int g = apply_grid(nvec, cvec);
    uint4 *o = reinterpret_cast<uint4 *>(dx), *r = reinterpret_cast<uint4 *>(dres);
    dispatch_cvec(cvec, [&](auto cvc) {
        constexpr int CV = decltype(cvc)::value;
        auto go = [&](auto rmc, auto drc) {
            constexpr int RM = decltype(rmc)::value;
            constexpr bool DR = decltype(drc)::value;
            bn_bwd_apply_kernel<CV, RM, DR, G><<<g, bn_threads<CV>(), 0, s>>>(
                grad, xx, fcoef, mask, coef, o, r, nvec, DR ? reinterpret_cast<const uint4 *>(dres_x) : nullptr,
                DR ? dres_sums : nullptr, bn_nt_mode());
        };
        using T = std::true_type;
        using F = std::false_type;
        if (rm == RM_COEF) {
            if (dres) go(std::integral_constant<int, RM_COEF>(), T());
            else go(std::integral_constant<int, RM_COEF>(), F());
        } else if (rm == RM_BITS) {
            if (dres) go(std::integral_constant<int, RM_BITS>(), T());
            else go(std::integral_constant<int, RM_BITS>(), F());
        } else {
            if (dres) go(std::integral_constant<int, RM_NONE>(), T());
            else go(std::integral_constant<int, RM_NONE>(), F());
        }
    });
}

}

void launch_bn_bwd_finalize_multi(const BnBwdFinBatch &b, hipStream_t s) {
    if (b.n <= 0) return;
    if (b.n > kBnFinMax) throw std::invalid_argument("bn_bwd_finalize_multi: too many BNs");
    int cmax = 0;
    for (int i = 0; i < b.n; ++i) cmax = b.d[i].C > cmax ? b.d[i].C : cmax;
    bn_bwd_finalize_multi<<<dim3((cmax + kFoldCh - 1) / kFoldCh, b.n), kBlock, 0, s>>>(b);
}

void launch_bn_sums_finalize_multi(const BnFinBatch &b, hipStream_t s) {
    if (b.n <= 0) return;
    if (b.n > kBnFinMax) throw std::invalid_argument("bn_sums_finalize_multi: too many BNs");
    int cmax = 0;
    for (int i = 0; i < b.n; ++i) cmax = b.d[i].C > cmax ? b.d[i].C : cmax;
    bn_sums_finalize_multi<<<dim3((cmax + 255) / 256, b.n), 256, 0, s>>>(b);
}

bool bn_supported_channels(int C) {
    if (C % 8) return false;
    switch (C / 8) {
    case 4: case 6: case 8: case 10: case 12: case 16: case 20: case 24: case 32: case 40: case 48: case 56:
    case 64: case 128: case 256:
        return true;
    default:
        return false;
    }
}

int bn_num_chunks(BNShape sh) { return chunking(sh).nchunks; }

void launch_bn_forward(const uint16_t *x, const uint16_t *res, const float *gamma, const float *beta, uint16_t *y,
                       uint8_t *mask, BNShape sh, bool relu, bool training, float *run_mean, float *run_var,
                       float momentum, float eps, float *partial, float *mean, float *invstd, float *coef,
                       int64_t *num_batches, hipStream_t s, double *sums, const float *res_coef, bool apply,
                       int64_t y_ld, bool prefinalized) {
    const int C = sh.channels, cvec = C / 8;
    if (y_ld > 0 && (y_ld % 8 || y_ld < C || res || !relu))
        throw std::invalid_argument("bn_forward: a strided output needs BN+ReLU without residual, row stride % 8");
    const int64_t nvec = sh.rows * cvec;
    if (training && sums) {
        if (!prefinalized)
            bn_sums_finalize<<<(C + 255) / 256, 256, 0, s>>>(sums, C, sh.rows, gamma, beta, mean, invstd, run_mean,
                                                             run_var, momentum, eps, coef, num_batches);
    } else if (training) {
        launch_stats(x, sh, gamma, beta, run_mean, run_var, momentum, eps, partial, mean, invstd, coef, num_batches,
                     s);
    } else {
        bn_eval_coef<<<(C + 255) / 256, 256, 0, s>>>(C, gamma, beta, run_mean, run_var, eps, mean, invstd, coef);
    }
    if (!apply) return;
    const int g = apply_grid(nvec, cvec);
    const int ntm = bn_nt_mode();
    dispatch_cvec(cvec, [&](auto cvc) {
        constexpr int CV = decltype(cvc)::value;
        constexpr int NT = bn_threads<CV>();
        const uint4 *xv = reinterpret_cast<const uint4 *>(x);
        const uint4 *rv = reinterpret_cast<const uint4 *>(res);
        uint4 *yv = reinterpret_cast<uint4 *>(y);
        if (res && res_coef) {
            if (relu) bn_apply_kernel<CV, true, true, true><<<g, NT, 0, s>>>(xv, rv, coef, yv, mask, nvec, res_coef, ntm);
            else bn_apply_kernel<CV, true, false, true><<<g, NT, 0, s>>>(xv, rv, coef, yv, mask, nvec, res_coef, ntm);
        } else if (res) {
            if (relu) bn_apply_kernel<CV, true, true><<<g, NT, 0, s>>>(xv, rv, coef, yv, mask, nvec, nullptr, ntm);
            else bn_apply_kernel<CV, true, false><<<g, NT, 0, s>>>(xv, rv, coef, yv, mask, nvec, nullptr, ntm);
        } else if (y_ld > 0 && y_ld != C) {
            bn_apply_kernel<CV, false, true, false, true><<<g, NT, 0, s>>>(xv, rv, coef, yv, mask, nvec, nullptr, ntm,
                                                                          y_ld / 8);
        } else {
            if (relu) bn_apply_kernel<CV, false, true><<<g, NT, 0, s>>>(xv, rv, coef, yv, mask, nvec, nullptr, ntm);
            else bn_apply_kernel<CV, false, false><<<g, NT, 0, s>>>(xv, rv, coef, yv, mask, nvec, nullptr, ntm);
        }
    });
}

void launch_bn_backward(const uint16_t *dy, const uint16_t *x, const float *fcoef, const uint8_t *mask,
                        const float *mean, const float *invstd, const float *gamma, BNShape sh, bool relu,
                        bool training, float *partial, float *dgamma, float *dbeta, float *coef, uint16_t *dx,
                        uint16_t *dres, hipStream_t s, double *sums, const uint16_t *dres_x, double *dres_sums,
                        int64_t dy_ld, int phase) {
    const int rm = !relu ? RM_NONE : (mask ? RM_BITS : RM_COEF);
    if (dy_ld > 0 && dy_ld != sh.channels) {
        if (dy_ld % 8) throw std::invalid_argument("bn_backward: dy row stride must be a multiple of 8");
        launch_backward_impl(StridedGrad{reinterpret_cast<const uint4 *>(dy), dy_ld / 8}, x, fcoef, mask, mean, invstd,
                             gamma, sh, rm, training, partial, dgamma, dbeta, coef, dx, dres, s, sums, dres_x,
                             dres_sums, phase);
        return;
    }
    launch_backward_impl(DirectGrad{reinterpret_cast<const uint4 *>(dy), (bn_nt_mode() & 1) != 0}, x, fcoef, mask, mean, invstd, gamma, sh, rm,
                         training, partial, dgamma, dbeta, coef, dx, dres, s, sums, dres_x, dres_sums, phase);
}

bool bn_pool_supported(BNShape sh, int H, int W) {
    return bn_supported_channels(sh.channels) && H >= 2 && W >= 2 && sh.rows % (static_cast<int64_t>(H) * W) == 0 &&
           sh.rows * (sh.channels / 8) < (int64_t(1) << 31);
}

void launch_bn_pool_forward(const uint16_t *x, const float *gamma, const float *beta, uint16_t *yp, uint8_t *arg,
                            BNShape sh, int H, int W, bool training, float *run_mean, float *run_var, float momentum,
                            float eps, float *partial, float *mean, float *invstd, float *coef, int64_t *num_batches,
                            hipStream_t s, double *sums, uint16_t *xarg) {
    const int C = sh.channels, cvec = C / 8;
    if (training && sums) {
        bn_sums_finalize<<<(C + 255) / 256, 256, 0, s>>>(sums, C, sh.rows, gamma, beta, mean, invstd, run_mean,
                                                         run_var, momentum, eps, coef, num_batches);
    } else if (training) {
        launch_stats(x, sh, gamma, beta, run_mean, run_var, momentum, eps, partial, mean, invstd, coef, num_batches,
                     s);
    } else {
        bn_eval_coef<<<(C + 255) / 256, 256, 0, s>>>(C, gamma, beta, run_mean, run_var, eps, mean, invstd, coef);
    }
    const int OH = pool_out(H), OW = pool_out(W);
    const int64_t N = sh.rows / (static_cast<int64_t>(H) * W);
    const int64_t nout = N * OH * OW * cvec;
    const int g = apply_grid(nout, cvec);
    dispatch_cvec(cvec, [&](auto cvc) {
        constexpr int CV = decltype(cvc)::value;
        bn_pool_apply_kernel<CV><<<g, bn_threads<CV>(), 0, s>>>(reinterpret_cast<const uint4 *>(x), coef,
                                                      reinterpret_cast<uint4 *>(yp), reinterpret_cast<uint2 *>(arg), H,
                                                      W, OH, OW, nout, reinterpret_cast<uint4 *>(xarg));
    });
}

void launch_bn_pool_backward(const uint16_t *dyp, const uint8_t *arg, const uint16_t *x, const float *fcoef,
                             const float *mean, const float *invstd, const float *gamma, BNShape sh, int H, int W,
                             bool training, float *partial, float *dgamma, float *dbeta, float *coef, uint16_t *dx,
                             hipStream_t s, const uint16_t *xarg, double *sums, bool apply) {
    if (xarg && sums && training) {
        const int C = sh.channels, cvec = C / 8;
        const int64_t nvec = sh.rows / (static_cast<int64_t>(H) * W) * pool_out(H) * pool_out(W) * cvec;
        const int g = apply_grid(nvec, cvec);
        dispatch_cvec(cvec, [&](auto cvc) {
            constexpr int CV = decltype(cvc)::value;
            bn_pool_bwd_sums_kernel<CV><<<g, bn_threads<CV>(), 0, s>>>(
                reinterpret_cast<const uint4 *>(dyp), reinterpret_cast<const uint4 *>(xarg), fcoef, sums, nvec);
        });
    } else {
        sums = nullptr;
    }
    const uint64_t m_hw = (uint64_t(1) << 40) / (static_cast<uint64_t>(H) * W) + 1;
    const uint64_t m_w = (uint64_t(1) << 40) / static_cast<uint64_t>(W) + 1;
    if (static_cast<uint64_t>(sh.rows) * H * W >= (uint64_t(1) << 40))
        throw std::invalid_argument("bn_pool_backward: too many rows for the 40-bit division");
    PoolGrad pg{reinterpret_cast<const uint4 *>(dyp), reinterpret_cast<const uint2 *>(arg), H, W, pool_out(H),
                pool_out(W), m_hw, m_w};
    launch_backward_impl(pg, x, fcoef, nullptr, mean, invstd, gamma, sh, RM_COEF, training, partial, dgamma, dbeta,
                         coef, dx, nullptr, s, sums, nullptr, nullptr, apply ? 0 : 3);
}

}
```

csrc/kernels/bn_fin.hpp:

```cpp
#pragma once

#include <hip/hip_runtime.h>

#include <cstdint>

namespace kfk {

__device__ __forceinline__ void bn_fin_fwd_channel(int c, int C, double s, double q, int64_t rows, float g, float b,
                                                   float rm, float rv, float *mean, float *invstd, float *run_mean,
                                                   float *run_var, float momentum, float eps, float *coef) {
    const double m = s / rows;
    double var = q / rows - m * m;
    if (var < 0) var = 0;
    const float is = rsqrtf(static_cast<float>(var) + eps);
    const float sc = g * is;
    mean[c] = static_cast<float>(m);
    invstd[c] = is;
    if (run_mean) {
        const double unbiased = rows > 1 ? var * rows / (rows - 1) : var;
        run_mean[c] = (1.f - momentum) * rm + momentum * static_cast<float>(m);
        run_var[c] = (1.f - momentum) * rv + momentum * static_cast<float>(unbiased);
    }
    coef[c] = sc;
    coef[C + c] = b - static_cast<float>(m) * sc;
}

__device__ __forceinline__ void bn_fin_bwd_channel(int c, int C, double s0, double s1, int64_t rows, float g,
                                                   float mu, float is, float *dgamma, float *dbeta, float *coef,
                                                   bool training) {
    const double db = s0, dg = static_cast<double>(is) * (s1 - static_cast<double>(mu) * db);
    dgamma[c] = static_cast<float>(dg);
    dbeta[c] = static_cast<float>(db);
    const float a = g * is;
    if (training) {
        const float inv_m = 1.f / static_cast<float>(rows);
        const float k2 = -a * static_cast<float>(dg) * is * inv_m;
        coef[c] = a;
        coef[C + c] = k2;
        coef[2 * C + c] = -a * static_cast<float>(db) * inv_m - k2 * mu;
    } else {
        coef[c] = a;
        coef[C + c] = 0.f;
        coef[2 * C + c] = 0.f;
    }
}

}
```

csrc/kernels/conv_wgrad.hip:

```cpp
#include "common.hpp"
#include "kernels.hpp"

#include <stdexcept>

namespace kfk {

const void *zero_page();

namespace {

typedef __attribute__((ext_vector_type(8))) __bf16 bf16x8;
typedef __attribute__((ext_vector_type(4))) short s16x4;
typedef __attribute__((ext_vector_type(8))) short s16x8;
typedef __attribute__((ext_vector_type(4))) float f32x4;
typedef __attribute__((address_space(3))) s16x4 lds_s16x4;

constexpr int kBK = 64;

constexpr int kWgradAux = 2;

__device__ __forceinline__ int fdiv(int p, uint64_t m) {
    return static_cast<int>((static_cast<uint64_t>(static_cast<uint32_t>(p)) * m) >> 40);
}

template <int N>
__device__ __forceinline__ void wait_vmcnt() {
    asm volatile("s_waitcnt vmcnt(%0)" ::"n"(N) : "memory");
}

template <int ROW>
__device__ __forceinline__ int hswz(int row) {
    if constexpr (ROW >= 256) return (row & 3) | (((row >> 3) & 1) << 2);
    else if constexpr (ROW == 64) return (row >> 3) & 1;
    else return ((row >> 1) & 1) | (((row >> 3) & 1) << 1);
}

__device__ __forceinline__ bf16x8 tr_frag(const uint8_t *p0, const uint8_t *p1) {
    const s16x4 lo = __builtin_amdgcn_ds_read_tr16_b64_v4i16((lds_s16x4 *)(p0));
    const s16x4 hi = __builtin_amdgcn_ds_read_tr16_b64_v4i16((lds_s16x4 *)(p1));
    const s16x8 v = __builtin_shufflevector(lo, hi, 0, 1, 2, 3, 4, 5, 6, 7);
    return __builtin_bit_cast(bf16x8, v);
}

template <int KS, int S, int WM, int WN, int STAGES, int TN = 4, int KB = 64>
__global__ __launch_bounds__(64 * WM * WN) void wgrad_kernel(const uint16_t *__restrict__ dy,
                                                             const uint16_t *__restrict__ x,
                                                             float *__restrict__ part, void *__restrict__ dw,
                                                             const uint16_t *__restrict__ zero, WGeo g,
                                                             int out_f32, int accumulate, int atomic_out,
                                                             int stagger = 0) {
    constexpr int BM = 64 * WM, BN = 16 * TN * WN, NW = WM * WN, NT = 64 * NW;
    constexpr int PAD = KS > 0 ? (KS - 1) / 2 : 0;
    constexpr int ROWA = BM * 2, ROWB = BN * 2;
    constexpr int CPRA = ROWA / 16, CPRB = ROWB / 16;
    constexpr int RPIA = 64 / CPRA, RPIB = 64 / CPRB;
    constexpr int A_BYTES = KB * ROWA, B_BYTES = KB * ROWB, STAGE = A_BYTES + B_BYTES;
    constexpr int A_INST = KB / RPIA / NW, B_INST = KB / RPIB / NW;
    constexpr int LOADS = A_INST + B_INST;
    static_assert(A_INST >= 1 && B_INST >= 1 && A_INST * NW * RPIA == KB && B_INST * NW * RPIB == KB, "split");
    static_assert(KB == 32 || KB == 64, "K-step of 32 or 64 pixels");
    constexpr bool IDENT = KS == 1 && S == 1;
    __shared__ __attribute__((aligned(1024))) uint8_t lds[STAGES * STAGE];

    const int tid = threadIdx.x, lane = tid & 63, wave = tid >> 6;
    const int nwg = gridDim.x, orig = blockIdx.x;
    const int q8 = nwg >> 3, rr = nwg & 7, xcd = orig & 7;
    const int wg = (xcd < rr ? xcd * (q8 + 1) : rr * (q8 + 1) + (xcd - rr) * q8) + (orig >> 3);
    const int split = wg / g.tiles, tile = wg - split * g.tiles;
    const int mn = g.mtiles * g.ntiles;
    const int tap = tile / mn, rem = tile - tap * mn;
    const int mt = rem / g.ntiles, nt = rem - mt * g.ntiles;
    const int kwin = KS > 0 ? KS : g.kwin;
    const int kh = tap / kwin, kw = tap - kh * kwin;
    const int pad_h = KS > 0 ? PAD : g.ph, pad_w = KS > 0 ? PAD : g.pw;
    const int m0 = mt * BM, n0 = nt * BN;
    const int p_begin = split * g.kps * kBK;
    int nsteps = (g.P - p_begin + KB - 1) / KB;
    if (nsteps > g.kps * (kBK / KB)) nsteps = g.kps * (kBK / KB);

    int a_row[A_INST], a_col[A_INST];
#pragma unroll
    for (int j = 0; j < A_INST; ++j) {
        const int r = (wave * A_INST + j) * RPIA + lane / CPRA;
        const int pc = lane % CPRA;
        const int lc = (((pc >> 1) ^ hswz<ROWA>(r)) << 1) | (pc & 1);
        a_row[j] = r;
        a_col[j] = m0 + lc * 8;
    }
    int b_row[B_INST], b_col[B_INST];
#pragma unroll
    for (int j = 0; j < B_INST; ++j) {
        const int r = (wave * B_INST + j) * RPIB + lane / CPRB;
        const int pc = lane % CPRB;
        const int lc = (((pc >> 1) ^ hswz<ROWB>(r)) << 1) | (pc & 1);
        b_row[j] = r;
        b_col[j] = n0 + lc * 8;
    }

    auto stage = [&](int ks, int buf) {
        const int p0 = p_begin + ks * KB;
        uint8_t *abase = lds + buf * STAGE;
        uint8_t *bbase = abase + A_BYTES;
#pragma unroll
        for (int j = 0; j < A_INST; ++j) {
            const int p = p0 + a_row[j];
            const uint16_t *src = p < g.P && a_col[j] < g.K ? dy + static_cast<uint32_t>(p * g.K + a_col[j]) : zero;
            __builtin_amdgcn_global_load_lds(src, abase + (wave * A_INST + j) * 1024, 16, 0, kWgradAux);
        }
#pragma unroll
        for (int j = 0; j < B_INST; ++j) {
            const int p = p0 + b_row[j];
            uint32_t eo = 0xFFFFFFFFu;
            if constexpr (IDENT) {
                if (p < g.P && b_col[j] < g.C) eo = static_cast<uint32_t>(p * g.C + b_col[j]);
            } else {
                const int n = fdiv(p, g.m_hw);
                const int r = p - n * g.HW;
                const int oh = fdiv(r, g.m_ow);
                const int ow = r - oh * g.OW;
                const int ih = oh * S + kh - pad_h, iw = ow * S + kw - pad_w;
                if (p < g.P && b_col[j] < g.C && static_cast<unsigned>(ih) < static_cast<unsigned>(g.H) &&
                    static_cast<unsigned>(iw) < static_cast<unsigned>(g.W))
                    eo = static_cast<uint32_t>(((n * g.H + ih) * g.W + iw) * g.C + b_col[j]);
            }
            const uint16_t *src = eo == 0xFFFFFFFFu ? zero : x + eo;
            __builtin_amdgcn_global_load_lds(src, bbase + (wave * B_INST + j) * 1024, 16, 0, kWgradAux);
        }
    };

    const int wm = wave / WN, wn = wave % WN;
    const int fg = lane >> 4, fq = (lane >> 2) & 3, fp = lane & 3;
    const int rowa0 = 8 * fg + fq;
    int aoff[4], boff[TN];
#pragma unroll
    for (int i = 0; i < 4; ++i) aoff[i] = rowa0 * ROWA + 32 * ((wm * 4 + i) ^ hswz<ROWA>(rowa0)) + 8 * fp;
#pragma unroll
    for (int j = 0; j < TN; ++j) boff[j] = rowa0 * ROWB + 32 * ((wn * TN + j) ^ hswz<ROWB>(rowa0)) + 8 * fp;

    f32x4 acc[4][TN];
#pragma unroll
    for (int i = 0; i < 4; ++i)
#pragma unroll
        for (int j = 0; j < TN; ++j) acc[i][j] = f32x4{0.f, 0.f, 0.f, 0.f};

    auto mfma_block = [&](const bf16x8 (&af)[4], const bf16x8 (&bfr)[TN]) {
#pragma unroll
        for (int i = 0; i < 4; ++i)
#pragma unroll
            for (int j = 0; j < TN; ++j)
                acc[i][j] = __builtin_amdgcn_mfma_f32_16x16x32_bf16(af[i], bfr[j], acc[i][j], 0, 0, 0);
    };

#pragma unroll
    for (int p = 0; p < STAGES - 1; ++p)
        if (p < nsteps) stage(p, p);
    int buf = 0;
    const bool upper = NW >= 8 && ((wave >> 2) & 1);
    const bool early = (stagger & 3) == 1 && upper, late = (stagger & 3) == 2 && upper;
    if ((stagger & 4) && upper) __builtin_amdgcn_s_setprio(1);
    for (int ks = 0; ks < nsteps; ++ks) {
        if (ks + STAGES - 1 <= nsteps) wait_vmcnt<LOADS * (STAGES - 2)>();
        else wait_vmcnt<0>();
        asm volatile("s_waitcnt lgkmcnt(0)" ::: "memory");
        __builtin_amdgcn_s_barrier();
        __builtin_amdgcn_sched_barrier(0);
        if (early && ks + STAGES - 1 < nsteps) {
            int nb = buf + STAGES - 1;
            if (nb >= STAGES) nb -= STAGES;
            stage(ks + STAGES - 1, nb);
        }
        __builtin_amdgcn_sched_barrier(0);
        const uint8_t *abase = lds + buf * STAGE;
        const uint8_t *bbase = abase + A_BYTES;
        bf16x8 af0[4], bf0[TN];
#pragma unroll
        for (int i = 0; i < 4; ++i) af0[i] = tr_frag(abase + aoff[i], abase + aoff[i] + 4 * ROWA);
#pragma unroll
        for (int j = 0; j < TN; ++j) bf0[j] = tr_frag(bbase + boff[j], bbase + boff[j] + 4 * ROWB);
        if constexpr (KB == 64) {
            bf16x8 af1[4], bf1[TN];
#pragma unroll
            for (int i = 0; i < 4; ++i) af1[i] = tr_frag(abase + aoff[i] + 32 * ROWA, abase + aoff[i] + 36 * ROWA);
#pragma unroll
            for (int j = 0; j < TN; ++j) bf1[j] = tr_frag(bbase + boff[j] + 32 * ROWB, bbase + boff[j] + 36 * ROWB);
            mfma_block(af0, bf0);
            __builtin_amdgcn_sched_barrier(0);
            if (!early && !late && ks + STAGES - 1 < nsteps) {
                int nb = buf + STAGES - 1;
                if (nb >= STAGES) nb -= STAGES;
                stage(ks + STAGES - 1, nb);
            }
            __builtin_amdgcn_sched_barrier(0);
            mfma_block(af1, bf1);
        } else {
            if (!early && !late && ks + STAGES - 1 < nsteps) {
                int nb = buf + STAGES - 1;
                if (nb >= STAGES) nb -= STAGES;
                stage(ks + STAGES - 1, nb);
            }
            __builtin_amdgcn_sched_barrier(0);
            mfma_block(af0, bf0);
        }
        if (late && ks + STAGES - 1 < nsteps) {
            __builtin_amdgcn_sched_barrier(0);
            int nb = buf + STAGES - 1;
            if (nb >= STAGES) nb -= STAGES;
            stage(ks + STAGES - 1, nb);
        }
        buf = buf + 1 == STAGES ? 0 : buf + 1;
    }
    wait_vmcnt<0>();

    if (atomic_out) {
#pragma unroll
        for (int i = 0; i < 4; ++i)
#pragma unroll
            for (int j = 0; j < TN; ++j)
#pragma unroll
                for (int r = 0; r < 4; ++r) {
                    const int co = m0 + wm * 64 + i * 16 + (lane >> 4) * 4 + r;
                    const int ci = n0 + wn * 16 * TN + j * 16 + (lane & 15);
                    if (co >= g.K || ci >= g.C) continue;
                    const int64_t e = (static_cast<int64_t>(co) * g.taps + tap) * g.C + ci;
                    atomicAdd(static_cast<float *>(dw) + e, acc[i][j][r]);
                }
    } else if (g.splits == 1) {
#pragma unroll
        for (int i = 0; i < 4; ++i)
#pragma unroll
            for (int j = 0; j < TN; ++j)
#pragma unroll
                for (int r = 0; r < 4; ++r) {
                    const int co = m0 + wm * 64 + i * 16 + (lane >> 4) * 4 + r;
                    const int ci = n0 + wn * 16 * TN + j * 16 + (lane & 15);
                    if (co >= g.K || ci >= g.C) continue;
                    const int64_t e = (static_cast<int64_t>(co) * g.taps + tap) * g.C + ci;
                    float v = acc[i][j][r];
                    if (out_f32) {
                        float *o = static_cast<float *>(dw) + e;
                        *o = accumulate ? *o + v : v;
                    } else {
                        uint16_t *o = static_cast<uint16_t *>(dw) + e;
                        if (accumulate) v += bf16_to_f32(*o);
                        *o = f32_to_bf16(v);
                    }
                }
    } else {
        f32x4 *dst = reinterpret_cast<f32x4 *>(part + static_cast<int64_t>(wg) * (BM * BN)) + tid;
#pragma unroll
        for (int i = 0; i < 4; ++i)
#pragma unroll
            for (int j = 0; j < TN; ++j) dst[(i * TN + j) * NT] = acc[i][j];
    }
}

template <int STAGES>
__global__ __launch_bounds__(576) void wgrad_rows_kernel(const uint16_t *__restrict__ dy,
                                                         const uint16_t *__restrict__ x,
                                                         float *__restrict__ part, void *__restrict__ dw,
                                                         const uint16_t *__restrict__ zero, RGeo g, int out_f32,
                                                         int accumulate, int atomic_out, int stagger = 0) {
    constexpr int ROW = 128;
    constexpr int MAXP = 4;
    constexpr int STAGE = (8 + 25 + 1) * 1024;
    constexpr int DUMMY = (8 + 25) * 1024;
    __shared__ __attribute__((aligned(1024))) uint8_t lds[STAGES * STAGE];

    const int tid = threadIdx.x, lane = tid & 63;
    const int wave = __builtin_amdgcn_readfirstlane(tid >> 6);
    const int kh = wave / 3, kw = wave - 3 * (wave / 3);
    const int nwg = gridDim.x, orig = blockIdx.x;
    const int q8 = nwg >> 3, rr8 = nwg & 7, xcd = orig & 7;
    const int wg = (xcd < rr8 ? xcd * (q8 + 1) : rr8 * (q8 + 1) + (xcd - rr8) * q8) + (orig >> 3);
    const int mn = g.mtiles * g.ntiles;
    const int split = wg / mn, ctile = wg - split * mn;
    const int mt = ctile / g.ntiles, nt = ctile - mt * g.ntiles;
    const int m0 = mt * 64, n0 = nt * 64;
    const int seg0 = split * g.kps;
    int nsteps = g.nseg - seg0;
    if (nsteps > g.kps) nsteps = g.kps;

    const int total = 8 + g.xpieces;
    int p_kind[MAXP], p_r[MAXP], p_c[MAXP], p_col[MAXP];
#pragma unroll
    for (int u = 0; u < MAXP; ++u) {
        const int pq = wave + 9 * u;
        const int pc = lane & 7;
        if (pq < 8) {
            const int t = pq * 8 + (lane >> 3);
            p_kind[u] = 0;
            p_r[u] = t / g.L;
            p_c[u] = t - p_r[u] * g.L;
            if (p_r[u] >= g.R) p_r[u] = 1 << 20;
            p_col[u] = m0 + ((((pc >> 1) ^ hswz<ROW>(t)) << 1) | (pc & 1)) * 8;
        } else if (pq < total) {
            const int t = (pq - 8) * 8 + (lane >> 3);
            p_kind[u] = 1;
            p_r[u] = t / g.XW;
            p_c[u] = t - p_r[u] * g.XW;
            if (t >= g.xrows) p_r[u] = 1 << 20;
            p_col[u] = n0 + ((((pc >> 1) ^ hswz<ROW>(t)) << 1) | (pc & 1)) * 8;
        } else {
// ... 111 lines not shown
                    const int co = m0 + i * 16 + (lane >> 4) * 4 + r;
                    const int ci = n0 + j * 16 + (lane & 15);
                    const int64_t e = (static_cast<int64_t>(co) * taps + tap) * g.C + ci;
                    float v = acc[i][j][r];
                    if (atomic_out) {
                        atomicAdd(static_cast<float *>(dw) + e, v);
                    } else if (out_f32) {
                        float *o = static_cast<float *>(dw) + e;
                        *o = accumulate ? *o + v : v;
                    } else {
                        uint16_t *o = static_cast<uint16_t *>(dw) + e;
                        if (accumulate) v += bf16_to_f32(*o);
                        *o = f32_to_bf16(v);
                    }
                }
    } else {
        const int tile = tap * mn + mt * g.ntiles + nt;
        f32x4 *dst = reinterpret_cast<f32x4 *>(part + (static_cast<int64_t>(split) * g.tiles + tile) * 4096) + lane;
#pragma unroll
        for (int i = 0; i < 4; ++i)
#pragma unroll
            for (int j = 0; j < 4; ++j) dst[(i * 4 + j) * 64] = acc[i][j];
    }
}

template <int S>
__device__ __forceinline__ void wait_ring(int n) {
    if constexpr (S <= 2) {
        wait_vmcnt<0>();
    } else {
        switch (n) {
            case 1: wait_vmcnt<1 * (S - 2)>(); break;
            case 2: wait_vmcnt<2 * (S - 2)>(); break;
            case 3: wait_vmcnt<3 * (S - 2)>(); break;
            case 4: wait_vmcnt<4 * (S - 2)>(); break;
            case 5: wait_vmcnt<5 * (S - 2)>(); break;
            default: wait_vmcnt<0>();
        }
    }
}

template <int NWV, int STAGES, int CT = 64, bool DENSE = (CT == 32)>
__global__ __launch_bounds__(64 * NWV) void wgrad_rows_rect_kernel(const uint16_t *__restrict__ dy,
                                                                   const uint16_t *__restrict__ x,
                                                                   float *__restrict__ part, void *__restrict__ dw,
                                                                   const uint16_t *__restrict__ zero, RRGeo g,
                                                                   int out_f32, int accumulate, int atomic_out,
                                                                   int stagger = 0) {
    constexpr int ROW = 2 * CT;
    constexpr int TI = CT / 16;
    constexpr int LPR = ROW / 16;
    constexpr int RPP = 64 / LPR;
    constexpr int DYP = 64 / RPP;
    constexpr int DYB = DYP * 1024;
    constexpr int MAXP = (DYP + 25 + NWV - 1) / NWV;
    static_assert(MAXP <= 5, "wait_ring covers 5 loads per stage");
    extern __shared__ __attribute__((aligned(1024))) uint8_t lds[];
    const int STAGE = g.stage;
    const int DUMMY = g.stage - 1024;

    const int tid = threadIdx.x, lane = tid & 63;
    const int wave = __builtin_amdgcn_readfirstlane(tid >> 6);
    const int nwg = gridDim.x, orig = blockIdx.x;
    const int q8 = nwg >> 3, rr8 = nwg & 7, xcd = orig & 7;
    const int wg = (xcd < rr8 ? xcd * (q8 + 1) : rr8 * (q8 + 1) + (xcd - rr8) * q8) + (orig >> 3);
    const int mn = g.mtiles * g.ntiles;
    const int per_split = mn * g.tgroups;
    const int split = wg / per_split, rem0 = wg - split * per_split;
    const int tg = rem0 / mn, ctile = rem0 - tg * mn;
    const int mt = ctile / g.ntiles, nt = ctile - mt * g.ntiles;
    const int m0 = mt * CT, n0 = nt * CT;
    const int tap = tg * NWV + wave;
    const bool has_tap = tap < g.taps;
    const int kh = has_tap ? tap / g.KW : 0, kw = has_tap ? tap - kh * g.KW : 0;
    const int seg0 = split * g.kps;
    int nsteps = g.nseg - seg0;
    if (nsteps > g.kps) nsteps = g.kps;

    const int total = DYP + g.xpieces;
    const int nload = (total + NWV - 1) / NWV;
    int p_kind[MAXP], p_r[MAXP], p_c[MAXP], p_col[MAXP];
    bool p_cok[MAXP];
#pragma unroll
    for (int u = 0; u < MAXP; ++u) {
        const int pq = wave + NWV * u;
        const int pc = lane % LPR;
        p_cok[u] = false;
        if (pq < DYP) {
            const int t = pq * RPP + lane / LPR;
            p_kind[u] = 0;
            p_r[u] = t / g.L;
            p_c[u] = t - p_r[u] * g.L;
            if (p_r[u] >= g.R) p_r[u] = 1 << 20;
            p_col[u] = m0 + ((((pc >> 1) ^ hswz<ROW>(t)) << 1) | (pc & 1)) * 8;
            p_cok[u] = p_col[u] < g.K;
        } else if (pq < total) {
            const int t = (pq - DYP) * RPP + lane / LPR;
            p_kind[u] = 1;
            p_r[u] = t / g.XW;
            p_c[u] = t - p_r[u] * g.XW;
            if (t >= g.xrows) p_r[u] = 1 << 20;
            p_col[u] = n0 + ((((pc >> 1) ^ hswz<ROW>(t)) << 1) | (pc & 1)) * 8;
            p_cok[u] = p_col[u] < g.C;
        } else {
            p_kind[u] = 2;
            p_r[u] = p_c[u] = p_col[u] = 0;
        }
    }
    const int segs_img = g.gpi * g.spr;
    auto stage = [&](int ks, int buf) {
        const int seg = seg0 + ks;
        const int n = seg / segs_img, rem = seg - n * segs_img;
        const int grp = rem / g.spr, sidx = rem - grp * g.spr;
        const int oh0 = grp * g.R, ow0 = sidx * g.L;
        uint8_t *base = lds + buf * STAGE;
#pragma unroll
        for (int u = 0; u < MAXP; ++u) {
            if (u >= nload) break;
            const int pq = wave + NWV * u;
            if constexpr (STAGES == 2) {
                if (p_kind[u] == 2 || !p_cok[u]) continue;
            }
            const uint16_t *src = zero;
            uint8_t *dst = base + DUMMY;
            if (p_kind[u] == 0) {
                const int oh = oh0 + p_r[u], ow = ow0 + p_c[u];
                if (oh < g.OH && ow < g.OW && p_cok[u])
                    src = dy + static_cast<uint32_t>(((n * g.OH + oh) * g.OW + ow) * g.K + p_col[u]);
                dst = base + pq * 1024;
            } else if (p_kind[u] == 1) {
                const int ih = oh0 * g.S + p_r[u] - g.ph, iw = ow0 * g.S + p_c[u] - g.pw;
                if (static_cast<unsigned>(ih) < static_cast<unsigned>(g.H) &&
                    static_cast<unsigned>(iw) < static_cast<unsigned>(g.W) && p_cok[u])
                    src = x + static_cast<uint32_t>(((n * g.H + ih) * g.W + iw) * g.C + p_col[u]);
                dst = base + pq * 1024;
            }
            __builtin_amdgcn_global_load_lds(src, dst, 16, 0, 0);
        }
    };

    const int fg = lane >> 4, fq = (lane >> 2) & 3, fp = lane & 3;
    const int rowa0 = 8 * fg + fq;
    int aoff[TI];
#pragma unroll
    for (int i = 0; i < TI; ++i) aoff[i] = rowa0 * ROW + 32 * (i ^ hswz<ROW>(rowa0)) + 8 * fp;
    int boff[4][TI];
#pragma unroll
    for (int s = 0; s < 4; ++s) {
        const int j = rowa0 + (s & 1) * 4 + (s >> 1) * 32;
        const int r = j / g.L, c = j - r * g.L;
        const int jrow = r < g.R ? r * g.S * g.XW + g.S * c : 0;
        const int trow = jrow + kh * g.XW + kw;
        const int h = hswz<ROW>(trow);
#pragma unroll
        for (int i = 0; i < TI; ++i) boff[s][i] = DYB + trow * ROW + 32 * (i ^ h) + 8 * fp;
    }

    f32x4 acc[TI][TI];
#pragma unroll
    for (int i = 0; i < TI; ++i)
#pragma unroll
        for (int j = 0; j < TI; ++j) acc[i][j] = f32x4{0.f, 0.f, 0.f, 0.f};
    auto mfma_block = [&](const bf16x8 (&af)[TI], const bf16x8 (&bfr)[TI]) {
#pragma unroll
        for (int i = 0; i < TI; ++i)
#pragma unroll
            for (int j = 0; j < TI; ++j)
                acc[i][j] = __builtin_amdgcn_mfma_f32_16x16x32_bf16(af[i], bfr[j], acc[i][j], 0, 0, 0);
    };

#pragma unroll
    for (int p = 0; p < STAGES - 1; ++p)
        if (p < nsteps) stage(p, p);
    int buf = 0;
    const bool early = stagger && ((wave >> 2) & 1);
    for (int ks = 0; ks < nsteps; ++ks) {
        if (ks + STAGES - 1 <= nsteps) wait_ring<STAGES>(nload);
        else wait_vmcnt<0>();
        asm volatile("s_waitcnt lgkmcnt(0)" ::: "memory");
        __builtin_amdgcn_s_barrier();
        __builtin_amdgcn_sched_barrier(0);
        if ((early || !has_tap) && ks + STAGES - 1 < nsteps) {
            int nb = buf + STAGES - 1;
            if (nb >= STAGES) nb -= STAGES;
            stage(ks + STAGES - 1, nb);
        }
        __builtin_amdgcn_sched_barrier(0);
        const uint8_t *base = lds + buf * STAGE;
        if (has_tap) {
            bf16x8 af0[TI], bf0[TI], af1[TI], bf1[TI];
#pragma unroll
            for (int i = 0; i < TI; ++i) {
                af0[i] = tr_frag(base + aoff[i], base + aoff[i] + 4 * ROW);
                bf0[i] = tr_frag(base + boff[0][i], base + boff[1][i]);
            }
#pragma unroll
            for (int i = 0; i < TI; ++i) {
                af1[i] = tr_frag(base + aoff[i] + 32 * ROW, base + aoff[i] + 36 * ROW);
                bf1[i] = tr_frag(base + boff[2][i], base + boff[3][i]);
            }
            mfma_block(af0, bf0);
            __builtin_amdgcn_sched_barrier(0);
            if (!early && ks + STAGES - 1 < nsteps) {
                int nb = buf + STAGES - 1;
                if (nb >= STAGES) nb -= STAGES;
                stage(ks + STAGES - 1, nb);
            }
            __builtin_amdgcn_sched_barrier(0);
            mfma_block(af1, bf1);
        }
        buf = buf + 1 == STAGES ? 0 : buf + 1;
    }
    wait_vmcnt<0>();
    if (!has_tap) return;

    if constexpr (DENSE) {
        if (!atomic_out && g.splits > 1) {
            float *dst = part + static_cast<int64_t>(split) * g.K * g.taps * g.C;
#pragma unroll
            for (int i = 0; i < TI; ++i)
#pragma unroll
                for (int j = 0; j < TI; ++j)
#pragma unroll
                    for (int r = 0; r < 4; ++r) {
                        const int co = m0 + i * 16 + (lane >> 4) * 4 + r;
                        const int ci = n0 + j * 16 + (lane & 15);
                        if (co < g.K && ci < g.C) dst[(static_cast<int64_t>(co) * g.taps + tap) * g.C + ci] = acc[i][j][r];
                    }
            return;
        }
    }
    if (atomic_out || g.splits == 1) {
#pragma unroll
        for (int i = 0; i < TI; ++i)
#pragma unroll
            for (int j = 0; j < TI; ++j)
#pragma unroll
                for (int r = 0; r < 4; ++r) {
                    const int co = m0 + i * 16 + (lane >> 4) * 4 + r;
                    const int ci = n0 + j * 16 + (lane & 15);
                    if (co >= g.K || ci >= g.C) continue;
                    const int64_t e = (static_cast<int64_t>(co) * g.taps + tap) * g.C + ci;
                    float v = acc[i][j][r];
                    if (atomic_out) {
                        atomicAdd(static_cast<float *>(dw) + e, v);
                    } else if (out_f32) {
                        float *o = static_cast<float *>(dw) + e;
                        *o = accumulate ? *o + v : v;
                    } else {
                        uint16_t *o = static_cast<uint16_t *>(dw) + e;
                        if (accumulate) v += bf16_to_f32(*o);
                        *o = f32_to_bf16(v);
                    }
                }
    } else if constexpr (!DENSE) {
        const int tile = tap * mn + mt * g.ntiles + nt;
        f32x4 *dst = reinterpret_cast<f32x4 *>(part + (static_cast<int64_t>(split) * g.tiles + tile) * 4096) + lane;
#pragma unroll
        for (int i = 0; i < 4; ++i)
#pragma unroll
            for (int j = 0; j < 4; ++j) dst[(i * 4 + j) * 64] = acc[i][j];
    }
}

__global__ __launch_bounds__(256) void wgrad_dense_reduce_kernel(const float *__restrict__ part, int splits, int64_t n,
                                                                 void *__restrict__ dw, int out_f32, int accumulate,
                                                                 int sgl) {
    __shared__ f32x4 red[256];
    const int G = 1 << sgl, COLS = 256 >> sgl;
    const int t = threadIdx.x, c = t & (COLS - 1), grp = t >> (8 - sgl);
    const int64_t n4 = n / 4, col = static_cast<int64_t>(blockIdx.x) * COLS + c;
    f32x4 a = f32x4{0.f, 0.f, 0.f, 0.f};
    if (col < n4) {
        const f32x4 *src = reinterpret_cast<const f32x4 *>(part) + col;
        int sp = grp;
        for (; sp + G < splits; sp += 2 * G) {
            const f32x4 u = src[sp * n4], v = src[(sp + G) * n4];
            a += u;
            a += v;
        }
        if (sp < splits) a += src[sp * n4];
    }
    red[t] = a;
    __syncthreads();
    if (grp != 0 || col >= n4) return;
    f32x4 sum = red[c];
    for (int k = 1; k < G; ++k) sum += red[k * COLS + c];
    const int64_t e = col * 4;
    if (out_f32) {
        f32x4 *o = reinterpret_cast<f32x4 *>(static_cast<float *>(dw) + e);
        if (accumulate) sum += *o;
        *o = sum;
    } else {
        uint16_t *o = static_cast<uint16_t *>(dw) + e;
#pragma unroll
        for (int k = 0; k < 4; ++k) {
            float v = sum[k];
            if (accumulate) v += bf16_to_f32(o[k]);
            o[k] = f32_to_bf16(v);
        }
    }
}

template <int WM, int WN, int TN = 4>
__global__ __launch_bounds__(256) void wgrad_reduce_kernel(const float *__restrict__ part, void *__restrict__ dw,
                                                           WGeo g, int out_f32, int accumulate, int sg_log2) {
    constexpr int BM = 64 * WM, BN = 16 * TN * WN, NT = 64 * WM * WN;
    constexpr int TILE4 = BM * BN / 4;
    __shared__ f32x4 red[256];
    const int SG = 1 << sg_log2, OUT = 256 >> sg_log2;
    const int t = threadIdx.x, o = t & (OUT - 1), sg = t >> (8 - sg_log2);
    const int64_t total = static_cast<int64_t>(g.tiles) * TILE4;
    const int64_t idx = static_cast<int64_t>(blockIdx.x) * OUT + o;
    const int64_t stride_split = total;
    f32x4 s = f32x4{0.f, 0.f, 0.f, 0.f};
    if (idx < total) {
        const f32x4 *src = reinterpret_cast<const f32x4 *>(part) + idx;
        int sp = sg;
        for (; sp + 3 * SG < g.splits; sp += 4 * SG) {
            const f32x4 a = src[sp * stride_split];
            const f32x4 b = src[(sp + SG) * stride_split];
            const f32x4 c = src[(sp + 2 * SG) * stride_split];
            const f32x4 d = src[(sp + 3 * SG) * stride_split];
            s += (a + b) + (c + d);
        }
        for (; sp < g.splits; sp += SG) s += src[sp * stride_split];
    }
    red[t] = s;
    __syncthreads();
    if (sg == 0 && idx < total) {
        for (int k = 1; k < SG; ++k) s += red[o + k * OUT];
        const int tile = static_cast<int>(idx / TILE4);
        const int rem = static_cast<int>(idx - static_cast<int64_t>(tile) * TILE4);
        const int ij = rem / NT, tid = rem - ij * NT;
        const int mn = g.mtiles * g.ntiles;
        const int tap = tile / mn, r2 = tile - tap * mn;
        const int mt = r2 / g.ntiles, nt = r2 - mt * g.ntiles;
        const int lane = tid & 63, wave = tid >> 6;
        const int wm = wave / WN, wn = wave % WN;
        const int i = ij / TN, j = ij % TN;
        const int ci = nt * BN + wn * 16 * TN + j * 16 + (lane & 15);
#pragma unroll
        for (int r = 0; r < 4; ++r) {
            const int co = mt * BM + wm * 64 + i * 16 + (lane >> 4) * 4 + r;
            if (co >= g.K || ci >= g.C) continue;
            const int64_t e = (static_cast<int64_t>(co) * g.taps + tap) * g.C + ci;
            float v = s[r];
            if (out_f32) {
                float *d = static_cast<float *>(dw) + e;
                *d = accumulate ? *d + v : v;
            } else {
                uint16_t *d = static_cast<uint16_t *>(dw) + e;
                if (accumulate) v += bf16_to_f32(*d);
                *d = f32_to_bf16(v);
            }
        }
    }
}


template <int WM, int WN, int TN = 4>
void reduce_tiles(const float *part, void *dw, const WGeo &g, bool out_f32, bool accumulate, hipStream_t s) {
    const WgradReduceLaunch r = wgrad_reduce_launch(static_cast<int64_t>(g.tiles) * (64 * WM) * (16 * TN * WN) / 4, g.splits);
    wgrad_reduce_kernel<WM, WN, TN><<<r.grid, 256, 0, s>>>(part, dw, g, out_f32, accumulate, r.sg_log2);
}

WGeo reduce_geo(int Cin, int Cout, int mtiles, int ntiles, int taps, int tiles, int splits) {
    WGeo g{};
    g.C = Cin, g.K = Cout, g.mtiles = mtiles, g.ntiles = ntiles, g.taps = taps, g.tiles = tiles, g.splits = splits;
    return g;
}

template <int KS, int S, int WM, int WN, int TN = 4>
void launch_t(const uint16_t *dy, const uint16_t *x, void *dw, float *part, const WGeo &g, bool out_f32,
              bool accumulate, bool atomic_out, hipStream_t s) {
    constexpr int STAGE_BYTES = 64 * (64 * WM + 16 * TN * WN) * 2;
    constexpr int STAGES = 3 * STAGE_BYTES <= 160 * 1024 ? 3 : 2;
    const int stagger = TN == 8 ? 1 : 0;
    wgrad_kernel<KS, S, WM, WN, STAGES, TN><<<g.tiles * g.splits, 64 * WM * WN, 0, s>>>(
        dy, x, part, dw, reinterpret_cast<const uint16_t *>(zero_page()), g, out_f32, accumulate, atomic_out, stagger);
    if (g.splits > 1 && !atomic_out) reduce_tiles<WM, WN, TN>(part, dw, g, out_f32, accumulate, s);
}

template <int KS, int S>
void launch_ks(const uint16_t *dy, const uint16_t *x, void *dw, float *part, const WGeo &g, int variant,
               bool out_f32, bool accumulate, bool atomic_out, hipStream_t s) {
    switch (variant) {
    case kWgradTile128x128: launch_t<KS, S, 2, 2>(dy, x, dw, part, g, out_f32, accumulate, atomic_out, s); break;
    case kWgradTile128x64: launch_t<KS, S, 2, 1>(dy, x, dw, part, g, out_f32, accumulate, atomic_out, s); break;
    case kWgradTile64x128: launch_t<KS, S, 1, 2>(dy, x, dw, part, g, out_f32, accumulate, atomic_out, s); break;
    case kWgradTile64x64: launch_t<KS, S, 1, 1>(dy, x, dw, part, g, out_f32, accumulate, atomic_out, s); break;
    case kWgradTile256x128: launch_t<KS, S, 4, 2>(dy, x, dw, part, g, out_f32, accumulate, atomic_out, s); break;
    case kWgradTile128x256: launch_t<KS, S, 2, 4>(dy, x, dw, part, g, out_f32, accumulate, atomic_out, s); break;
    default: launch_t<KS, S, 4, 2, 8>(dy, x, dw, part, g, out_f32, accumulate, atomic_out, s); break;
    }
}

void launch_tiled(const uint16_t *dy, const uint16_t *x, void *dw, float *part, const WgradPlan &plan, bool out_f32,
                  bool accumulate, bool atomic_out, hipStream_t s) {
    const WGeo &g = plan.tiled;
    const int64_t P = plan.shape.P();
    if (P * g.HW >= (int64_t(1) << 40) || P >= (1 << 23))
        throw std::invalid_argument("conv_wgrad: too many pixels for the 40-bit division");
    const bool k1 = g.taps == 1 && g.ph == 0 && g.pw == 0, k3 = g.taps == 9 && g.kwin == 3 && g.ph == 1 && g.pw == 1;
    if (plan.shape.stride == 1) {
        if (k1) launch_ks<1, 1>(dy, x, dw, part, g, plan.variant, out_f32, accumulate, atomic_out, s);
        else if (k3) launch_ks<3, 1>(dy, x, dw, part, g, plan.variant, out_f32, accumulate, atomic_out, s);
        else launch_ks<0, 1>(dy, x, dw, part, g, plan.variant, out_f32, accumulate, atomic_out, s);
    } else {
        if (k1) launch_ks<1, 2>(dy, x, dw, part, g, plan.variant, out_f32, accumulate, atomic_out, s);
        else if (k3) launch_ks<3, 2>(dy, x, dw, part, g, plan.variant, out_f32, accumulate, atomic_out, s);
        else launch_ks<0, 2>(dy, x, dw, part, g, plan.variant, out_f32, accumulate, atomic_out, s);
    }
}

void launch_rows_rect(const uint16_t *dy, const uint16_t *x, void *dw, float *part, const WgradPlan &plan, bool out_f32,
                      bool accumulate, bool atomic_out, hipStream_t s) {
    const RRGeo &g = plan.rect;
    const int grid = g.mtiles * g.ntiles * g.tgroups * g.splits;
    const uint16_t *z = reinterpret_cast<const uint16_t *>(zero_page());
    const int lds = plan.stages * g.stage;
    const bool t7 = g.taps % 7 == 0;
    static bool attr_set[kWgradRing64x4 + 1][2] = {};
    auto go = [&](auto kern, int nwv) {
        bool &done = attr_set[plan.variant][t7 ? 1 : 0];
        if (!done) {
            (void)hipFuncSetAttribute(reinterpret_cast<const void *>(kern), hipFuncAttributeMaxDynamicSharedMemorySize,
                                      160 * 1024);
            done = true;
        }
        kern<<<grid, 64 * nwv, lds, s>>>(dy, x, part, dw, z, g, out_f32, accumulate, atomic_out, 1);
    };
    switch (plan.variant) {
    case kWgradRows: t7 ? go(wgrad_rows_rect_kernel<7, 2>, 7) : go(wgrad_rows_rect_kernel<9, 2>, 9); break;
    case kWgradRing32x2: t7 ? go(wgrad_rows_rect_kernel<7, 2, 32, true>, 7) : go(wgrad_rows_rect_kernel<9, 2, 32, true>, 9); break;
    case kWgradRing32x3: t7 ? go(wgrad_rows_rect_kernel<7, 3, 32, true>, 7) : go(wgrad_rows_rect_kernel<9, 3, 32, true>, 9); break;
    case kWgradRing32x4: t7 ? go(wgrad_rows_rect_kernel<7, 4, 32, true>, 7) : go(wgrad_rows_rect_kernel<9, 4, 32, true>, 9); break;
    case kWgradRing64x3: t7 ? go(wgrad_rows_rect_kernel<7, 3, 64, true>, 7) : go(wgrad_rows_rect_kernel<9, 3, 64, true>, 9); break;
    default: t7 ? go(wgrad_rows_rect_kernel<7, 4, 64, true>, 7) : go(wgrad_rows_rect_kernel<9, 4, 64, true>, 9); break;
    }
    if (g.splits == 1 || atomic_out) return;
    if (plan.kernel == WgradKernel::RowsRect) {
        reduce_tiles<1, 1>(part, dw, reduce_geo(g.C, g.K, g.mtiles, g.ntiles, g.taps, g.tiles, g.splits), out_f32, accumulate, s);
    } else {
        const int64_t n = static_cast<int64_t>(g.K) * g.taps * g.C;
        int sgl = 0;
        while (sgl < 6 && (8 << sgl) < g.splits && (n / 4) * (2 << sgl) <= int64_t(1024) * 256) ++sgl;
        const int cols = 256 >> sgl;
        wgrad_dense_reduce_kernel<<<static_cast<int>((n / 4 + cols - 1) / cols), 256, 0, s>>>(part, g.splits, n, dw, out_f32,
                                                                                           accumulate, sgl);
    }
}

}

void launch_conv_wgrad(const uint16_t *dy, const uint16_t *x, void *dw, float *part, const WgradPlan &plan, bool out_f32,
                       bool accumulate, hipStream_t s, bool atomics) {
    const bool atomic_out = atomics && out_f32 && accumulate && plan.splits > 1;
    if (plan.splits > 1 && !atomic_out && part == nullptr) throw std::invalid_argument("conv_wgrad: split-K needs the workspace");
    switch (plan.kernel) {
    case WgradKernel::Tiled: launch_tiled(dy, x, dw, part, plan, out_f32, accumulate, atomic_out, s); break;
    case WgradKernel::Rows3x3: {
        const RGeo &g = plan.rows;
        wgrad_rows_kernel<2><<<g.mtiles * g.ntiles * g.splits, 576, 0, s>>>(
            dy, x, part, dw, reinterpret_cast<const uint16_t *>(zero_page()), g, out_f32, accumulate, atomic_out, 1);
        if (g.splits > 1 && !atomic_out)
            reduce_tiles<1, 1>(part, dw, reduce_geo(g.C, g.K, g.mtiles, g.ntiles, 9, g.tiles, g.splits), out_f32, accumulate, s);
        break;
    }
    default: launch_rows_rect(dy, x, dw, part, plan, out_f32, accumulate, atomic_out, s); break;
    }
}

}
```

csrc/kernels/kernels.hpp:

```cpp
#pragma once

#include <hip/hip_runtime.h>

#include "wgrad_plan.hpp"

#include <cstddef>
#include <cstdint>
#include <string>
#include <vector>

namespace kfk {

constexpr int kMaxGridHost = 2048;

void launch_reduce(void *z, const void *x, const void *y, size_t n, int dtype, int op, hipStream_t s);

void launch_embedding_backward(float *grad, const int64_t *ids, const void *dy, bool dy_bf16, int64_t T, int D,
                               int64_t V, hipStream_t s, int ch = 0);

void set_dropout_seed_base(const uint32_t *p);
const uint32_t *dropout_seed_base();

constexpr int kGemmBias = 1, kGemmAccum = 2, kGemmGeluGrad = 4;
bool gemm_nt_supported(int64_t M, int64_t N, int64_t K);
int gemm_nt_pick_bn(int64_t M, int64_t N);
void launch_gemm_nt(const uint16_t *a, const uint16_t *b, uint16_t *c, const uint16_t *bias, int M, int N, int K,
                    int epi, int bn, hipStream_t s);
bool gemm_nt_ld_supported(int64_t M, int64_t N, int64_t K, int64_t ldc);
void launch_gemm_nt_ld(const uint16_t *a, const uint16_t *b, uint16_t *c, const uint16_t *bias, int M, int N, int K,
                       int ldc, int epi, int bn, hipStream_t s);
int gemm_nt_gelu_grad_rows(int M);
void launch_gemm_nt_gelu_grad(const uint16_t *a, const uint16_t *b, uint16_t *c, const uint16_t *u, float *part, int M,
                              int N, int K, hipStream_t s);
void launch_colsum_fold(const float *part, int rows, int O, float *out_f32, uint16_t *out_bf16, hipStream_t s);

void launch_comm_emulate(const void *bucket, void *scratch, int64_t bytes, int64_t traffic_bytes, int ctas,
                         double seconds, hipStream_t s);

void launch_sgd(float *w, const float *g, float *m, uint16_t *shadow, size_t n, float lr, const float *lr_dev,
                float mu, float damp, float wd, float gscale, bool nesterov, bool first, hipStream_t s);

void launch_adam(float *w, const float *g, float *m, float *v, size_t n, float lr, const float *lr_dev, float b1,
                 float b2, float eps, float wd, bool adamw, float gscale, const float *step_dev, hipStream_t s,
                 uint16_t *shadow = nullptr);

void launch_axpby(void *y, const void *x, void *z, size_t n, float a, float b, int dtype, hipStream_t s);

void launch_scale(void *x, size_t n, float alpha, int dtype, hipStream_t s);

void launch_square(float *dst, const void *src, size_t n, int dtype, hipStream_t s);
void launch_cast(void *dst, const void *src, size_t n, int src_dt, int dst_dt, float scale, hipStream_t s);

int colsum_chunks(int64_t T, int O);
void launch_colsum_bf16(const uint16_t *x, int64_t T, int O, float *part, float *out_f32, uint16_t *out_bf16,
                        hipStream_t s);
int gelu_colsum_chunks(int64_t T, int O);
class PairPrefetcher {
  public:
    struct Job {
        uintptr_t pending_ev = 0;
        int64_t pending_ver = 0;
        uintptr_t host_copy = 0;
        int target = 0;
        std::vector<uintptr_t> src_slots;
        int64_t own_ver = 0;
        uintptr_t dst = 0;
        uintptr_t after_ev = 0;
        uintptr_t host_stage = 0;
    };
    struct Result {
        int status = 0;
        int64_t version = 0, own_ver = 0;
        std::string error;
    };
    PairPrefetcher(const std::string &libpath, int device, int self_rank, const std::string &rec_name,
                   const std::string &model_name, int64_t nbytes, int slots);
    ~PairPrefetcher();
    PairPrefetcher(const PairPrefetcher &) = delete;
    PairPrefetcher &operator=(const PairPrefetcher &) = delete;
    void start(const Job &job);
    bool busy();
    Result finish(uintptr_t wait_stream);

  private:
    struct Impl;
    Impl *d_;
};

void launch_xent_forward(const uint16_t *x, const int64_t *labels, int64_t R, int V, float *lse, float *loss,
                         hipStream_t s, int64_t ld = 0);
void launch_xent_backward(const uint16_t *x, const int64_t *labels, const float *lse, const float *scale, int64_t R,
                          int V, uint16_t *dx, hipStream_t s, int64_t ld = 0);

void launch_gelu_bwd_colsum(const uint16_t *dy, const uint16_t *u, uint16_t *du, int64_t T, int O, float *part,
                            float *out_f32, uint16_t *out_bf16, hipStream_t s);
void launch_sumsq2(const void *a, const void *b, size_t n, int dtype, float *partials, float *out, hipStream_t s);

void launch_variance(const float *s1, const float *s2, size_t n, float inv_np, float *partials, float *out,
                     hipStream_t s);

void launch_seg_variance(const float *s1, const float *s2, size_t n, float inv_np, const int64_t *seg_off, int nseg,
                         float *out, hipStream_t s);

void launch_gns_update(const float *sumsq_small, const float *sumsq_big, float b_small, float b_big, float alpha,
                       float *state, hipStream_t s);

void launch_pack(const int64_t *desc, int n_tensors, size_t total, void *flat, int flat_dtype, int src_dtype,
                 float scale, hipStream_t s);
void launch_unpack(const int64_t *desc, int n_tensors, size_t total, const void *flat, int flat_dtype,
                   int dst_dtype, float scale, hipStream_t s);

struct GradAccTable {
    static constexpr int kMax = 48;
    int n = 0;
    int src_dtype = 0;
    float scale = 1.f;
    const void *src[kMax];
    int64_t off[kMax];
    int64_t numel[kMax];
    int blk_start[kMax + 1];
};
int grad_accumulate_blocks(int64_t numel);
void launch_grad_accumulate(const GradAccTable &tab, float *flat, hipStream_t s);

constexpr int kStatSlots = 16;
bool conv_supported(int Cin, int Cout, int ks, int stride);
int conv_variants();
enum ConvEpi : int {
    kEpiFwdStats = 1, kEpiAccum = 2, kEpiBwdCoef = 4, kEpiBwdBits = 8, kEpiBiasRelu = 16, kEpiGate = 32,
    kEpiAccMask = 64, kEpiAccEven = 128, kEpiBias = 256, kEpiGeluGrad = 1024
};
struct EpiArgs {
    const uint8_t *amask = nullptr;
    const uint16_t *bias = nullptr;
    double *stats = nullptr;
    const uint16_t *bx = nullptr;
    const float *fcoef = nullptr;
    const uint8_t *bmask = nullptr;
};
void launch_conv(const uint16_t *x, const uint16_t *w, uint16_t *y, int N, int H, int W, int Cin, int Cout, int ks,
                 int stride, const EpiArgs &ea, int epi, hipStream_t s, int variant = -1);
void launch_conv_dgrad_s2(const uint16_t *dy, const uint16_t *wt, uint16_t *dx, int N, int OH, int OW, int Cout,
                          int Cin, int ks, const EpiArgs &ea, int epi, hipStream_t s, int variant = -1, int DH = 0,
                          int DW = 0, int pad = 1);
bool gemm_supported(int M, int K, int N);
void launch_gemm(const uint16_t *x, const uint16_t *w, uint16_t *y, int M, int K, int N, const EpiArgs &ea, int epi,
                 hipStream_t s, int variant = -1);
bool conv_rect_supported(int Cin, int Cout, int kh, int kw, int stride);
void launch_conv_rect(const uint16_t *x, const uint16_t *w, uint16_t *y, int N, int H, int W, int Cin, int Cout,
                      int kh, int kw, int ph, int pw, int stride, const EpiArgs &ea, int epi, hipStream_t s);
struct FlipTable {
    static constexpr int kMax = 64;
    int n = 0;
    const uint16_t *src[kMax];
    uint16_t *dst[kMax];
    int cout[kMax], cin[kMax], taps[kMax];
    int64_t start[kMax + 1];
    int tstart[kMax + 1];
};
void launch_conv_flip_multi(const FlipTable &tab, hipStream_t s);
void launch_conv_flip_weight(const uint16_t *w, uint16_t *wt, int Cout, int Cin, int ks, hipStream_t s);
void launch_conv_flip_weight_taps(const uint16_t *w, uint16_t *wt, int Cout, int Cin, int taps, hipStream_t s);

void launch_conv_wgrad(const uint16_t *dy, const uint16_t *x, void *dw, float *part, const WgradPlan &plan,
                       bool out_f32, bool accumulate, hipStream_t s, bool atomics = true);

void launch_stem_pad4(const uint16_t *x, uint16_t *x4, int64_t npix, hipStream_t s);
void launch_stem_pad4_f32(const float *x, uint16_t *x4, int64_t npix, hipStream_t s);
void launch_stem_pack_weight(const uint16_t *w, uint16_t *wp, hipStream_t s);
int stem_out(int h);
int stem3_out(int h, int k, int stride, int pad);
void launch_stem3_pack_weight(const uint16_t *w, uint16_t *wp, int Cout, int KH, int KW, hipStream_t s);
void launch_stem3_forward(const void *x, bool x_f32, const uint16_t *wp, uint16_t *y, double *stats, const float *bias,
                          bool relu, int Cout, int N, int H, int W, int KH, int KW, int stride, int ph, int pw,
                          hipStream_t s);
int stem3_wgrad_blocks(int Cout, int N, int H, int W, int KH, int KW, int stride, int ph, int pw);
int64_t stem3_wgrad_workspace(int Cout, int N, int H, int W, int KH, int KW, int stride, int ph, int pw);
void launch_stem3_wgrad(const uint16_t *dy, const void *x, bool x_f32, void *dw, bool out_f32, float *part, int Cout,
                        int N, int H, int W, int KH, int KW, int stride, int ph, int pw, hipStream_t s);
void launch_stem_forward(const uint16_t *x4, const uint16_t *wp, uint16_t *y, double *stats, int N, int H, int W,
                         hipStream_t s);
int stem_wgrad_splits(int N, int H, int W);
int64_t stem_wgrad_workspace(int N, int H, int W, int splits);
bool stem_wgrad_bnp_supported(int N, int H, int W);
void launch_stem_wgrad_bnp(const uint16_t *y, const uint16_t *x4, uint16_t *dw, float *part, int N, int H, int W,
                           int splits, const uint16_t *dyp, const uint8_t *arg, const float *fcoef,
                           const float *bcoef, hipStream_t s);
void launch_stem_wgrad(const uint16_t *dy, const uint16_t *x4, uint16_t *dw, float *part, int N, int H, int W,
                       int splits, hipStream_t s);

struct BNShape {
    int64_t rows;
    int channels;
};
bool bn_supported_channels(int C);
int bn_num_chunks(BNShape sh);
struct BnFinDesc {
    double *sums;
    const float *gamma, *beta;
    float *mean, *invstd, *run_mean, *run_var, *coef;
    int64_t *nbt;
    int64_t rows;
    int C;
    float momentum, eps;
};
constexpr int kBnFinMax = 8;
struct BnFinBatch {
    BnFinDesc d[kBnFinMax];
    int n;
};
void launch_bn_sums_finalize_multi(const BnFinBatch &b, hipStream_t s);
struct BnBwdFinDesc {
    const float *partial;
    int nchunks, C;
    int64_t rows;
    const float *gamma, *mean, *invstd;
    float *dgamma, *dbeta, *coef;
};
struct BnBwdFinBatch {
    BnBwdFinDesc d[kBnFinMax];
    int n;
};
void launch_bn_bwd_finalize_multi(const BnBwdFinBatch &b, hipStream_t s);

void launch_bn_forward(const uint16_t *x, const uint16_t *res, const float *gamma, const float *beta, uint16_t *y,
                       uint8_t *mask, BNShape sh, bool relu, bool training, float *run_mean, float *run_var,
                       float momentum, float eps, float *partial, float *mean, float *invstd, float *coef,
                       int64_t *num_batches, hipStream_t s, double *sums = nullptr, const float *res_coef = nullptr,
                       bool apply = true, int64_t y_ld = 0, bool prefinalized = false);
void launch_bn_backward(const uint16_t *dy, const uint16_t *x, const float *fcoef, const uint8_t *mask,
                        const float *mean, const float *invstd, const float *gamma, BNShape sh, bool relu,
                        bool training, float *partial, float *dgamma, float *dbeta, float *coef, uint16_t *dx,
                        uint16_t *dres, hipStream_t s, double *sums = nullptr, const uint16_t *dres_x = nullptr,
                        double *dres_sums = nullptr, int64_t dy_ld = 0, int phase = 0);

inline int pool_out(int h) { return (h + 2 - 3) / 2 + 1; }
bool bn_pool_supported(BNShape sh, int H, int W);
void launch_bn_pool_forward(const uint16_t *x, const float *gamma, const float *beta, uint16_t *yp, uint8_t *arg,
                            BNShape sh, int H, int W, bool training, float *run_mean, float *run_var, float momentum,
                            float eps, float *partial, float *mean, float *invstd, float *coef, int64_t *num_batches,
                            hipStream_t s, double *sums = nullptr, uint16_t *xarg = nullptr);
void launch_bn_pool_backward(const uint16_t *dyp, const uint8_t *arg, const uint16_t *x, const float *fcoef,
                             const float *mean, const float *invstd, const float *gamma, BNShape sh, int H, int W,
                             bool training, float *partial, float *dgamma, float *dbeta, float *coef, uint16_t *dx,
                             hipStream_t s, const uint16_t *xarg = nullptr, double *sums = nullptr, bool apply = true);

bool bias_act_supported(int C);
void launch_bias_act_forward(uint16_t *y, const float *bias, int64_t rows, int C, bool relu, hipStream_t s);
int bias_act_backward_blocks(int64_t rows, int C);
void launch_bias_act_backward(const uint16_t *dy, const uint16_t *y, uint16_t *dz, float *dbias, float *partial,
                              int64_t rows, int C, bool relu, hipStream_t s);

void launch_maxpool2x2_forward(const uint16_t *x, uint16_t *y, int64_t N, int H, int W, int C, hipStream_t s);
int maxpool3s2_out(int h, int pad);
void launch_maxpool3s2_forward(const uint16_t *x, uint16_t *y, uint8_t *arg, int64_t N, int H, int W, int C, int pad,
                               hipStream_t s);
void launch_maxpool3s2_backward(const uint16_t *dy, const uint8_t *arg, uint16_t *dx, int64_t N, int H, int W, int C,
                                int pad, hipStream_t s);
void launch_avgpool3s1(const uint16_t *x, uint16_t *y, int64_t N, int H, int W, int C, hipStream_t s);
void launch_global_avgpool_forward(const uint16_t *x, uint16_t *y, int64_t N, int HW, int C, hipStream_t s);
void launch_global_avgpool_backward(const uint16_t *dy, uint16_t *dx, int64_t N, int HW, int C, hipStream_t s);

bool layernorm_supported(int D);
int layernorm_bwd_blocks(int64_t rows);
void launch_layernorm_forward(const uint16_t *x, const uint16_t *r, const float *gamma, const float *beta, uint16_t *y,
                              uint16_t *s, float *mean, float *rstd, int64_t rows, int D, float eps, hipStream_t st,
                              float p = 0.f, uint32_t seed = 0);
void launch_layernorm_backward(const uint16_t *dy, const uint16_t *s, const float *gamma, const float *mean,
                               const float *rstd, uint16_t *ds, float *partial, float *dgamma, float *dbeta,
                               int64_t rows, int D, hipStream_t st,
                               uint16_t *dr = nullptr, float p = 0.f, uint32_t seed = 0, float *rb_f32 = nullptr,
                               uint16_t *rb_bf16 = nullptr);
void launch_maxpool2x2_backward(const uint16_t *x, const uint16_t *dy, uint16_t *dx, int64_t N, int H, int W, int C,
                                hipStream_t s, double *gate_stats = nullptr);

bool attention_supported(int S, int head_dim);
void launch_attention_forward(const uint16_t *qkv, uint16_t *out, float *lse, int B, int S, int H, float scale,
                              uint32_t seed, float p_drop, hipStream_t s);
void launch_attention_backward(const uint16_t *qkv, const uint16_t *out, const float *lse, const uint16_t *dout,
                               uint16_t *dqkv, int B, int S, int H, float scale, uint32_t seed, float p_drop,
                               hipStream_t s);

}
```

kungfu_amd/ops/conv.py:

```python
from __future__ import annotations

import os

import torch
import torch.nn as nn
import torch.nn.functional as F

from .._lib import buf_ok, hip, hip_available

_ENABLED = os.environ.get("KUNGFU_CONV3X3", "1") != "0"
_WGRAD = os.environ.get("KUNGFU_WGRAD", "1") != "0"
_WGRAD_MAX_PIXELS = 1 << 31


def set_wgrad_enabled(on: bool) -> bool:
    global _WGRAD
    old, _WGRAD = _WGRAD, bool(on)
    return old


def _cl4(t: torch.Tensor) -> bool:
    return t.dim() == 4 and t.dtype == torch.bfloat16 and t.is_contiguous(memory_format=torch.channels_last)


def wgrad(dy: torch.Tensor, x: torch.Tensor, w: torch.Tensor, stride: int, pad) -> torch.Tensor:
    stride = int(stride)
    ph, pw = _pair(pad)
    route = "library"
    if _WGRAD and x.is_cuda and _cl4(x) and _cl4(dy) and w.dim() == 4 and hip_available():
        n, kh, kw = int(x.shape[0]), int(w.shape[2]), int(w.shape[3])
        route, variant, cap = hip().conv_wgrad_route(n, int(x.shape[2]), int(x.shape[3]), int(x.shape[1]),
                                                     int(dy.shape[1]), kh, kw, ph, pw, stride)
    if route == "rect" and _WGRAD_RECT:
        return hip().conv_wgrad_rect(dy, x, kh, kw, stride, ph, pw, variant)
    if route == "square":
        per_img = int(dy.shape[2]) * int(dy.shape[3])
        cap = min(_WGRAD_MAX_PIXELS, cap)
        if n * per_img < cap:
            return hip().conv_wgrad(dy, x, kh, stride, variant=variant)
        step = max(1, (cap - 1) // per_img)
        acc = torch.zeros(w.shape, dtype=torch.float32, device=x.device).contiguous(
            memory_format=torch.channels_last)
        for i in range(0, n, step):
            hip().conv_wgrad(dy[i:i + step], x[i:i + step], kh, stride, out=acc, accumulate=True,
                             atomics=False)
        return acc.to(torch.bfloat16)
    return torch.ops.aten.convolution_backward(dy, x, w, None, [stride, stride], [ph, pw], [1, 1], False, [0, 0], 1,
                                               [False, True, False])[1]


def set_enabled(on: bool) -> bool:
    global _ENABLED
    old, _ENABLED = _ENABLED, bool(on)
    return old


def eligible(x: torch.Tensor, w: torch.Tensor, stride, padding, dilation, groups) -> bool:
    if not _ENABLED or not x.is_cuda or groups != 1:
        return False
    st = stride if isinstance(stride, int) else (stride[0] if stride[0] == stride[1] else -1)
    pd = padding if isinstance(padding, int) else (padding[0] if padding[0] == padding[1] else -1)
    dl = dilation if isinstance(dilation, int) else (dilation[0] if dilation[0] == dilation[1] else -1)
    if st not in (1, 2) or pd != 1 or dl != 1:
        return False
    if w.dim() != 4 or w.shape[2] != 3 or w.shape[3] != 3 or x.dim() != 4:
        return False
    if x.dtype != torch.bfloat16 or w.dtype != torch.bfloat16:
        return False
    if not x.is_contiguous(memory_format=torch.channels_last):
        return False
    if not w.is_contiguous(memory_format=torch.channels_last):
        return False
    if not hip_available() or not buf_ok(x.numel(), w.numel()):
        return False
    return hip().conv_supported(int(x.shape[1]), int(w.shape[0]), 3, int(st))


class _Conv3x3Fn(torch.autograd.Function):
    @staticmethod
    def forward(ctx, x, w, stride):
        ctx.save_for_backward(x, w)
        ctx.stride = stride
        return hip().conv(x, w, stride)

    @staticmethod
    def backward(ctx, dy):
        x, w = ctx.saved_tensors
        s = ctx.stride
        if not dy.is_contiguous(memory_format=torch.channels_last):
            dy = dy.contiguous(memory_format=torch.channels_last)
        need_dx, need_dw = ctx.needs_input_grad[0], ctx.needs_input_grad[1]
        dx = dw = None
        if need_dx and s == 1:
            dx = hip().conv(dy, hip().conv_flip_weight(w), 1)
            need_dx = False
        if need_dw:
            dw = wgrad(dy, x, w, s, 1)
        if need_dx:
            dx = torch.ops.aten.convolution_backward(dy, x, w, None, [s, s], [1, 1], [1, 1], False, [0, 0], 1,
                                                     [True, False, False])[0]
        return dx, dw, None


def conv3x3(x: torch.Tensor, w: torch.Tensor, stride: int = 1) -> torch.Tensor:
    if eligible(x, w, stride, 1, 1, 1):
        return _Conv3x3Fn.apply(x, w, int(stride if isinstance(stride, int) else stride[0]))
    return F.conv2d(x, w, stride=stride, padding=1)


class _BiasActFn(torch.autograd.Function):

    @staticmethod
    def forward(ctx, y, b, relu):
        hip().bias_act_forward_(y, b, relu)
        ctx.mark_dirty(y)
        ctx.save_for_backward(y)
        ctx.relu = relu
        return y

    @staticmethod
    def backward(ctx, dy):
        (y,) = ctx.saved_tensors
        dz, db = hip().bias_act_backward(dy.contiguous(memory_format=torch.channels_last), y, ctx.relu)
        return dz, db, None


def _pair(v):
    return (int(v), int(v)) if isinstance(v, int) else (int(v[0]), int(v[1]))


def rect_eligible(x: torch.Tensor, w: torch.Tensor, stride, padding, dilation, groups) -> bool:
    if not (_ENABLED and _RECT) or not x.is_cuda or groups != 1 or w.dim() != 4 or x.dim() != 4:
        return False
    st, pd, dl = _pair(stride), _pair(padding), _pair(dilation)
    if st[0] != st[1] or dl != (1, 1) or pd[0] >= w.shape[2] or pd[1] >= w.shape[3]:
        return False
    if x.dtype != torch.bfloat16 or w.dtype != torch.bfloat16 or not hip_available():
        return False
    if not x.is_contiguous(memory_format=torch.channels_last) or not w.is_contiguous(memory_format=torch.channels_last):
        return False
    if not buf_ok(x.numel(), w.numel()):
        return False
    return hip().conv_rect_supported(int(x.shape[1]), int(w.shape[0]), int(w.shape[2]), int(w.shape[3]), st[0])


class _ConvRectFn(torch.autograd.Function):

    @staticmethod
    def forward(ctx, x, w, stride, ph, pw, stats, flip=None):
        ctx.save_for_backward(x, w)
        ctx.geo = (stride, ph, pw)
        ctx.flip = flip
        ctx.link = getattr(x, "_kf_link", None)
        return hip().conv_rect(x, w, stride, ph, pw, stats)

    @staticmethod
    def backward(ctx, dy):
        x, w = ctx.saved_tensors
        s, ph, pw = ctx.geo
        if not dy.is_contiguous(memory_format=torch.channels_last):
            dy = dy.contiguous(memory_format=torch.channels_last)
        dx = dw = None
        kh, kw = int(w.shape[2]), int(w.shape[3])
        if ctx.needs_input_grad[0]:
            if s == 1:
                wt = ctx.flip[0].get(ctx.flip[1]) if ctx.flip is not None else hip().conv_flip_weight(w)
                dx = _dgrad_link(dy, wt, kh - 1 - ph, kw - 1 - pw, None, ctx.link)
            elif s == 2 and kh == kw == 3 and ph == pw and ph in (0, 1) and min(x.shape[1], dy.shape[1]) >= 16:
                wt = ctx.flip[0].get(ctx.flip[1]) if ctx.flip is not None else hip().conv_flip_weight(w)
                H = hip()
                lk = ctx.link
                if lk is not None and lk.y is not None:
                    dx = H.conv_dgrad_s2(dy, wt, 3, lk.ws, lk.y, lk.coef, None, -1, int(x.shape[2]), int(x.shape[3]), ph)
                    lk.ready, lk.dx_ptr = True, dx.data_ptr()
                else:
                    dx = H.conv_dgrad_s2(dy, wt, 3, dh=int(x.shape[2]), dw=int(x.shape[3]), pad=ph)
            else:
                dx = torch.ops.aten.convolution_backward(dy, x, w, None, [s, s], [ph, pw], [1, 1], False, [0, 0], 1,
                                                         [True, False, False])[0]
        if ctx.needs_input_grad[1]:
            dw = wgrad(dy, x, w, s, (ph, pw))
        return dx, dw, None, None, None, None, None


def _dgrad_link(dy, wt, ph, pw, out, link):
    if link is None or link.y is None:
        return hip().conv_rect(dy, wt, 1, ph, pw, None, out)
    dx = hip().conv_rect(dy, wt, 1, ph, pw, link.ws, out, link.y, link.coef)
    link.ready, link.dx_ptr = True, dx.data_ptr()
    return dx


class _SiblingConvFn(torch.autograd.Function):

    @staticmethod
    def forward(ctx, x, pads, stats, flips, *ws):
        ys = tuple(hip().conv_rect(x, w, 1, ph, pw, st) for w, (ph, pw), st in zip(ws, pads, stats))
        ctx.save_for_backward(x, *ws)
        ctx.pads, ctx.flips = pads, flips
        ctx.link = getattr(x, "_kf_link", None)
        return ys

    @staticmethod
    def backward(ctx, *dys):
        x, *ws = ctx.saved_tensors
        dx = None
        dws = []
        last = max((i for i, d in enumerate(dys) if d is not None), default=-1)
        for i, (w, dy, (ph, pw), fl) in enumerate(zip(ws, dys, ctx.pads, ctx.flips)):
            if dy is None:
                dws.append(None)
                continue
            if not dy.is_contiguous(memory_format=torch.channels_last):
                dy = dy.contiguous(memory_format=torch.channels_last)
            if ctx.needs_input_grad[0]:
                wt = fl[0].get(fl[1]) if fl is not None else hip().conv_flip_weight(w)
                kh, kw = int(w.shape[2]), int(w.shape[3])
                dx = _dgrad_link(dy, wt, kh - 1 - ph, kw - 1 - pw, dx, ctx.link if i == last else None)
            dws.append(wgrad(dy, x, w, 1, (ph, pw)))
        return (dx, None, None, None, *dws)


def sibling_convs(x, convs, stats):
    from ..parallel.mixed import direct_target, shadow

    ws, pads, flips = [], [], []
    for c in convs:
        if c.bias is not None or _pair(c.stride) != (1, 1):
            return None
        w = shadow(c.weight)
        if not rect_eligible(x, w, 1, c.padding, c.dilation, c.groups):
            return None
        ws.append(w)
        pads.append(_pair(c.padding))
        tc = direct_target(c.weight)
        if tc is not None and w is not c.weight:
            from .fused_block import _flip_cache

            fc = _flip_cache(tc[0])
            fc.register(tc[1], w)
            flips.append((fc, tc[1]))
        else:
            flips.append(None)
    return _SiblingConvFn.apply(x, tuple(pads), tuple(stats), tuple(flips), *ws)


_RECT = os.environ.get("KUNGFU_CONV_RECT", "1") != "0"
_WGRAD_RECT = os.environ.get("KUNGFU_WGRAD_RECT", "1") != "0"


def conv2d_stats(x, w, stride, padding, stats: torch.Tensor, master: torch.Tensor = None):
    if not rect_eligible(x, w, stride, padding, 1, 1):
        return None
    st, pd = _pair(stride), _pair(padding)
    flip = None
    if master is not None:
        from ..parallel.mixed import direct_target
        from .fused_block import _flip_cache

        tc = direct_target(master)
        if tc is not None and w is not master:
            fc = _flip_cache(tc[0])
            fc.register(tc[1], w)
            flip = (fc, tc[1])
    return _ConvRectFn.apply(x, w, st[0], pd[0], pd[1], stats, flip)


def conv2d(x, w, bias, stride, padding, dilation, groups, relu: bool = False):
    if bias is None and not eligible(x, w, stride, padding, dilation, groups) and \
            rect_eligible(x, w, stride, padding, dilation, groups):
        st, pd = _pair(stride), _pair(padding)
        y = _ConvRectFn.apply(x, w, st[0], pd[0], pd[1], None)
        return F.relu(y) if relu else y
    if eligible(x, w, stride, padding, dilation, groups):
        y = _Conv3x3Fn.apply(x, w, int(stride if isinstance(stride, int) else stride[0]))
        if bias is not None and hip().bias_act_supported(int(y.shape[1])):
            return _BiasActFn.apply(y, bias.float().contiguous(), bool(relu))
        if bias is not None:
            y = y + bias.view(1, -1, 1, 1).to(y.dtype)
        return F.relu(y) if relu else y
    y = F.conv2d(x, w, bias, stride, padding, dilation, groups)
    return F.relu(y) if relu else y


class Conv2dReLU(nn.Conv2d):

    kf_shadow_forward = True

    def forward(self, x):
        from ..parallel.mixed import shadow

        w = shadow(self.weight)
        b = shadow(self.bias) if self.bias is not None else None
        if b is not None and x.dim() == 4 and x.shape[1] == 3:
            from .stem import stem3_conv, stem3_eligible

            if stem3_eligible(self, x):
                return stem3_conv(self, x, w, bias=b, relu=True)
        if self.padding_mode == "zeros" and x.dtype == torch.bfloat16:
            return conv2d(x, w, b, self.stride, self.padding, self.dilation, self.groups, relu=True)
        if b is not None and x.is_cuda and hip_available() and hip().bias_act_supported(self.out_channels):
            y = self._conv_forward(x, w, None)
            if y.dtype == torch.bfloat16 and y.is_contiguous(memory_format=torch.channels_last):
                return _BiasActFn.apply(y, b.float().contiguous(), True)
            return F.relu(y + b.view(1, -1, 1, 1).to(y.dtype))
        return F.relu(self._conv_forward(x, w, b))
```

kungfu_amd/ops/fused_block.py:

```python
from __future__ import annotations

import os
from typing import List, Optional

import torch
import torch.nn.functional as F

from .._lib import buf_ok, hip, hip_available
from ..parallel.mixed import deliver, direct_target, shadow

_ENABLED = os.environ.get("KUNGFU_FUSED_BLOCK", "1") != "0"


_CAPTURE = None


def _capture(bn, kind, dz, x, mean, invstd, gate, dg, db):
    _CAPTURE.append(dict(bn=bn, kind=kind, dz=dz.detach().clone(), x=x.detach().clone(), mean=mean.clone(),
                         invstd=invstd.clone(), gate=None if gate is None else gate.clone(),
                         dg=dg.detach().clone(), db=db.detach().clone()))


def set_enabled(on: bool) -> bool:
    global _ENABLED
    old, _ENABLED = _ENABLED, bool(on)
    return old


def _cl(t: torch.Tensor) -> torch.Tensor:
    return t if t.is_contiguous(memory_format=torch.channels_last) else t.contiguous(memory_format=torch.channels_last)


def _sums(bn, dev) -> torch.Tensor:
    ws = getattr(bn, "_kf_sums", None)
    if ws is None or ws.device != dev:
        ws = torch.zeros(hip().conv_stat_slots * 2 * bn.num_features, dtype=torch.float64, device=dev)
        bn._kf_sums = ws
    return ws


def _wgrad(dy, x, w, stride, pad):
    from .conv import wgrad

    return wgrad(dy, x, w, stride, pad)


class _FlipCache:

    def __init__(self, space):
        self.space = space
        self.index = {}
        self.gen = -1

    def register(self, i: int, w: torch.Tensor):
        if i not in self.index:
            co, ci, kh, kw = w.shape
            self.index[i] = torch.empty((ci, co, kh, kw), dtype=torch.bfloat16, device=w.device).contiguous(
                memory_format=torch.channels_last)
            self.gen = -1

    def get(self, i: int) -> torch.Tensor:
        if self.gen != self.space.shadow_gen:
            idx = sorted(self.index)
            ws = [self.space.shadow_view(j) for j in idx]
            ws = [w if w.dim() == 4 else w.view(w.shape[0], w.shape[1], 1, 1) for w in ws]
            hip().conv_flip_weights(ws, [self.index[j] for j in idx])
            self.gen = self.space.shadow_gen
        return self.index[i]


def _flip_cache(space) -> _FlipCache:
    c = getattr(space, "_kf_flip", None)
    if c is None:
        c = space._kf_flip = _FlipCache(space)
    return c


def _dgrad(dy, x, w, stride, pad, out: Optional[torch.Tensor] = None, flipped: Optional[torch.Tensor] = None,
           bn=None, out_mask: Optional[torch.Tensor] = None, acc_even: bool = False):
    H = hip()
    wt = flipped if flipped is not None else None
    if stride == 1:
        wt = wt if wt is not None else H.conv_flip_weight(w)
        _dgrad.fused = bn is not None
        if bn is not None:
            ws, bx, fc, mk = bn
            return H.conv(dy, wt, 1, ws, out, -1, bx, fc, mk, acc_mask=out_mask, acc_even=acc_even)
        return H.conv(dy, wt, 1, None, out, acc_mask=out_mask, acc_even=acc_even)
    assert out_mask is None and not acc_even
    ks = w.shape[2]
    if stride == 2 and out is None and _even_s2(x, dy, ks):
        wt = wt if wt is not None else H.conv_flip_weight(w)
        if ks == 3 and bn is not None:
            ws, bx, fc, mk = bn
            _dgrad.fused = True
            return H.conv_dgrad_s2(dy, wt, 3, ws, bx, fc, mk)
        _dgrad.fused = False
        dx = H.conv_dgrad_s2(dy, wt, ks)
        if ks == 1:
            dx.view(dx.shape[0], dx.shape[1], dx.shape[2] // 2, 2, dx.shape[3] // 2, 2)[:, :, :, 1:, :, :].zero_()
            dx.view(dx.shape[0], dx.shape[1], dx.shape[2] // 2, 2, dx.shape[3] // 2, 2)[:, :, :, 0, :, 1:].zero_()
        return dx
    _dgrad.fused = False
    dx = torch.ops.aten.convolution_backward(dy, x, w, None, [stride, stride], [pad, pad], [1, 1], False, [0, 0], 1,
                                             [True, False, False])[0]
    if out is not None:
        out.add_(dx)
        return out
    return _cl(dx)


def _even_s2(x, dy, ks) -> bool:
    return (x.shape[2] == 2 * dy.shape[2] and x.shape[3] == 2 * dy.shape[3] and ks in (1, 3)
            and hip().conv_supported(dy.shape[1], x.shape[1], ks, 1))


def _dgrad_s2_even(dy, x, w, flipped=None):
    H = hip()
    wt = flipped if flipped is not None else H.conv_flip_weight(w)
    return H.conv_dgrad_s2(dy, wt, 1)


class _TailSlot:
    __slots__ = ("ws", "y3", "mask", "ready", "dx_ptr")

    def __init__(self, ws, y3, mask):
        self.ws, self.y3, self.mask = ws, y3, mask
        self.ready = False
        self.dx_ptr = 0


class _Spec:
    __slots__ = ("bns", "stride", "ds", "dtypes", "direct", "wsrc")

    def __init__(self, bns, stride, ds):
        self.bns, self.stride, self.ds = bns, stride, ds
        self.dtypes = None
        self.direct = None
        self.wsrc = None


class _BottleneckFn(torch.autograd.Function):
    @staticmethod
    def forward(ctx, spec: _Spec, x, *params):
        H = hip()
        dev = x.device
        ws = [p for p in params]
        ws_bf = [w if w.dtype == torch.bfloat16 else w.to(torch.bfloat16) for w in ws[0::3]]
        ws_bf = [_cl(w) for w in ws_bf]
        gam, bet = ws[1::3], ws[2::3]
        s = spec.stride
        outs = []

        def bn(i, y, res, relu, res_coef=None, apply=True):
            m = spec.bns[i]
            return H.bn_forward(y, res, gam[i], bet[i], m.running_mean, m.running_var, m.momentum, m.eps, True, relu,
                                m.num_batches_tracked, _sums(m, dev), res_coef=res_coef, apply=apply)

        def conv(i, inp, w_, st_):
            return H.conv(inp, w_, st_, _sums(spec.bns[i], dev))

        y1 = conv(0, x, ws_bf[0], 1)
        z1, m1, i1, c1, _ = bn(0, y1, None, True)
        y2 = conv(1, z1, ws_bf[1], s)
        z2, m2, i2, c2, _ = bn(1, y2, None, True)
        y3 = conv(2, z2, ws_bf[2], 1)
        if spec.ds:
            yd = conv(3, x, ws_bf[3], s)
            _, md, idd, cd, _ = bn(3, yd, None, False, apply=False)
            out, m3, i3, c3, mask3 = bn(2, y3, yd, True, res_coef=cd)
        else:
            yd = md = idd = cd = None
            out, m3, i3, c3, mask3 = bn(2, y3, x, True)
        ctx.prev = getattr(x, "_kf_tail", None)
        ctx.tail = _TailSlot(_sums(spec.bns[2], dev), y3, mask3)
        ctx.spec = spec
        ctx.wdtypes = [w.dtype for w in ws[0::3]]
        ctx.save_for_backward(x, y1, z1, y2, z2, y3, yd, *ws_bf, *gam, m1, i1, c1, m2, i2, c2, m3, i3, c3, mask3,
                              md, idd, cd)
        return out

    @staticmethod
    def backward(ctx, dout):
        H = hip()
        spec = ctx.spec
        nb = 4 if spec.ds else 3
        t = list(ctx.saved_tensors)
        x, y1, z1, y2, z2, y3, yd = t[:7]
        w = t[7:7 + nb]
        g = t[7 + nb:7 + 2 * nb]
        (m1, i1, c1, m2, i2, c2, m3, i3, c3, mask3, md, idd, cd) = t[7 + 2 * nb:]
        s = spec.stride
        dout = _cl(dout)
        fl = [None] * nb
        if spec.wsrc is not None:
            for k, src in enumerate(spec.wsrc):
                if src is not None:
                    fl[k] = src[0].get(src[1])
        dbn = [None] * nb
        dw = [None] * nb
        wgrad = _wgrad

        ws = [_sums(b, dout.device) for b in spec.bns]
        tail = ctx.tail
        use3 = tail.ready and dout.data_ptr() == tail.dx_ptr
        if tail.ready and not use3:
            tail.ws.zero_()
        tail.ready, tail.y3, tail.mask = False, None, None
        in_place = use3 and not spec.ds
        dy3, didt, dg3, db3 = H.bn_backward(dout, y3, m3, i3, g[2], c3, mask3, True, True, not in_place,
                                            ws[2] if use3 else None, dres_x=yd if spec.ds else None,
                                            dres_sums=ws[3] if spec.ds else None)
        dbn[2] = (dg3, db3)
        if _CAPTURE is not None:
            _capture(spec.bns[2], "mask", dout, y3, m3, i3, mask3, dg3, db3)
        dz2 = _dgrad(dy3, z2, w[2], 1, 0, flipped=fl[2], bn=(ws[1], y2, c2, None))
        dw[2] = wgrad(dy3, z2, w[2], 1, 0)
        dy2, _, dg2, db2 = H.bn_backward(dz2, y2, m2, i2, g[1], c2, None, True, True, False, ws[1])
        dbn[1] = (dg2, db2)
        if _CAPTURE is not None:
            _capture(spec.bns[1], "relu", dz2, y2, m2, i2, c2, dg2, db2)
        dz1 = _dgrad(dy2, z1, w[1], s, 1, flipped=fl[1], bn=(ws[0], y1, c1, None))
        fused1 = _dgrad.fused
        dw[1] = wgrad(dy2, z1, w[1], s, 1)
        dy1, _, dg1, db1 = H.bn_backward(dz1, y1, m1, i1, g[0], c1, None, True, True, False,
                                         ws[0] if fused1 else None)
        dbn[0] = (dg1, db1)
        if _CAPTURE is not None:
            _capture(spec.bns[0], "relu", dz1, y1, m1, i1, c1, dg1, db1)
        acc_even = False
        if spec.ds:
            dyd, _, dgd, dbd = H.bn_backward(didt, yd, md, idd, g[3], cd, None, False, True, False, ws[3])
            dbn[3] = (dgd, dbd)
            if _CAPTURE is not None:
                _capture(spec.bns[3], "plain", didt, yd, md, idd, None, dgd, dbd)
            if s == 2 and _even_s2(x, dyd, 1):
                dx = _dgrad_s2_even(dyd, x, w[3], flipped=fl[3])
                acc_even = True
            else:
                dx = _dgrad(dyd, x, w[3], s, 0, flipped=fl[3])
            dw[3] = wgrad(dyd, x, w[3], s, 0)
        elif in_place:
            dx = dout
        else:
            dx = didt
        om = mask3 if in_place else None
        prev = ctx.prev
        if prev is not None and prev.y3 is not None and prev.y3.shape == dx.shape:
            dx = _dgrad(dy1, x, w[0], 1, 0, out=dx, flipped=fl[0], bn=(prev.ws, prev.y3, None, prev.mask),
                        out_mask=om, acc_even=acc_even)
            prev.ready, prev.dx_ptr = True, dx.data_ptr()
        else:
            dx = _dgrad(dy1, x, w[0], 1, 0, out=dx, flipped=fl[0], out_mask=om, acc_even=acc_even)
        dw[0] = wgrad(dy1, x, w[0], 1, 0)
        grads: List[Optional[torch.Tensor]] = []
        for i in range(nb):
            gw = dw[i]
            if gw.dtype != ctx.wdtypes[i]:
                gw = gw.to(ctx.wdtypes[i])
            dgm, dbt = dbn[i]
            tgt = spec.direct[i] if spec.direct is not None else None
            if tgt is not None:
                deliver(tgt[0], dgm)
                deliver(tgt[1], dbt)
                dgm = dbt = None
            grads += [gw, dgm, dbt]
        return (None, dx, *grads)


def eligible(block, x: torch.Tensor) -> bool:
    if not (_ENABLED and block.training and x.is_cuda and x.dtype == torch.bfloat16 and x.dim() == 4):
        return False
    if not x.is_contiguous(memory_format=torch.channels_last) or not hip_available():
        return False
    widest = max(block.conv1.in_channels, block.conv3.out_channels, block.conv1.out_channels)
    if not buf_ok(x.numel() // x.shape[1] * widest):
        return False
    H = hip()
    convs = [block.conv1, block.conv2, block.conv3] + ([block.downsample[0]] if block.downsample is not None else [])
    for c in convs:
        if c.bias is not None or c.groups != 1 or c.dilation != (1, 1):
            return False
        if not H.conv_supported(c.in_channels, c.out_channels, c.kernel_size[0], c.stride[0]):
            return False
    if block.conv2.kernel_size != (3, 3) or block.conv2.padding != (1, 1):
        return False
    if block.downsample is not None and block.downsample[0].kernel_size != (1, 1):
        return False
    bns = [block.bn1, block.bn2, block.bn3] + ([block.downsample[1]] if block.downsample is not None else [])
    for b in bns:
        if not (b.track_running_stats and b.momentum is not None and b.affine):
            return False
        if not H.bn_supported_channels(b.num_features):
            return False
    return True


def bottleneck_forward(block, x: torch.Tensor) -> torch.Tensor:
    ds = block.downsample is not None
    convs = [block.conv1, block.conv2, block.conv3] + ([block.downsample[0]] if ds else [])
    bns = [block.bn1, block.bn2, block.bn3] + ([block.downsample[1]] if ds else [])
    spec = getattr(block, "_kf_spec", None)
    if spec is None or spec.ds != ds:
        spec = _Spec(bns, block.conv2.stride[0], ds)
        block._kf_spec = spec
    params = []
    direct = []
    wsrc = []
    for c, b in zip(convs, bns):
        w = shadow(c.weight)
        params += [w, b.weight, b.bias]
        tw, tb = direct_target(b.weight), direct_target(b.bias)
        direct.append((tw, tb) if tw is not None and tb is not None else None)
        tc = direct_target(c.weight)
        if tc is not None and w is not c.weight and w.dtype == torch.bfloat16:
            fc = _flip_cache(tc[0])
            fc.register(tc[1], w)
            wsrc.append((fc, tc[1]))
        else:
            wsrc.append(None)
    spec.direct = direct if any(d is not None for d in direct) else None
    spec.wsrc = wsrc if any(v is not None for v in wsrc) else None
    out = _BottleneckFn.apply(spec, x, *params)
    if out.grad_fn is not None:
        out._kf_tail = out.grad_fn.tail
    return out
```

Measured before the change: 12800.

## Piggyback BN backward sums-finalize onto the conv weight-gradient reduce kernel

Folds the backward batch-norm statistics finalize (the sums-to-dgamma/dbeta/coef step) into extra blocks of the wgrad split-K reduce kernel, so a following bn_backward can skip its own finalize launch (phase 2, using the precomputed values). The goal is fewer small kernel launches and less serialization in the bottleneck backward pass. This adds a rider descriptor, a template FIN path in the reduce kernel, a fallback standalone finalize when the wgrad route has no reduce, and cross-block state in the tail slot. The risk is extra blocks slowing the reduce kernel and more complex ordering of when the sums workspace gets zeroed.

```diff
diff --git a/csrc/kernels/bind_bn.cpp b/csrc/kernels/bind_bn.cpp
--- a/csrc/kernels/bind_bn.cpp
+++ b/csrc/kernels/bind_bn.cpp
@@ -161,7 +161,8 @@
 
 std::vector<at::Tensor> bn_backward(at::Tensor dy, at::Tensor x, at::Tensor mean, at::Tensor invstd, at::Tensor weight,
                                     at::Tensor fcoef, OptTensor mask, bool relu, bool training, bool want_dres,
-                                    OptTensor sums, OptTensor dres_x, OptTensor dres_sums) {
+                                    OptTensor sums, OptTensor dres_x, OptTensor dres_sums,
+                                    c10::optional<std::vector<at::Tensor>> pre) {
     const char *op = "bn_backward";
     auto sh = bn_shape(x, op);
     const int C = sh.channels;
@@ -177,6 +178,13 @@
         mp = mask->data_ptr<uint8_t>();
     }
     double *sp = stats_ptr(sums, op, C, dev, "sums");
+    const bool prefin = pre.has_value();
+    if (prefin) {
+        TORCH_CHECK(pre->size() == 3 && !sp, "bn_backward: pre must be (dgamma, dbeta, coef), without sums");
+        check_dense((*pre)[0], op, "pre[0]", dev, at::kFloat, C);
+        check_dense((*pre)[1], op, "pre[1]", dev, at::kFloat, C);
+        check_dense((*pre)[2], op, "pre[2]", dev, at::kFloat, 3 * C);
+    }
     const uint16_t *dsx = nullptr;
     double *dsp = nullptr;
     if (has(dres_x)) {
@@ -193,15 +201,28 @@
     auto dx = at::empty_like(x, kCL);
     at::Tensor dres;
     if (want_dres) dres = at::empty_like(x, kCL);
-    at::Tensor dw = at::empty({C}, fopt), db = at::empty({C}, fopt), coef = at::empty({3 * C}, fopt);
+    at::Tensor dw, db, coef;
+    if (prefin) dw = (*pre)[0], db = (*pre)[1], coef = (*pre)[2];
+    else dw = at::empty({C}, fopt), db = at::empty({C}, fopt), coef = at::empty({3 * C}, fopt);
     at::Tensor partial;
-    if (!sp) partial = at::empty({2 * static_cast<int64_t>(kfk::bn_num_chunks(sh)) * C}, fopt);
+    if (!sp && !prefin) partial = at::empty({2 * static_cast<int64_t>(kfk::bn_num_chunks(sh)) * C}, fopt);
     kfk::launch_bn_backward(bf16(dy), bf16(x), fcoef.data_ptr<float>(), mp, mean.data_ptr<float>(),
                             invstd.data_ptr<float>(), weight.data_ptr<float>(), sh, relu, training,
                             partial.defined() ? partial.data_ptr<float>() : nullptr, dw.data_ptr<float>(),
                             db.data_ptr<float>(), coef.data_ptr<float>(), bf16_mut(dx),
-                            want_dres ? bf16_mut(dres) : nullptr, stream_of(x, 0), sp, dsx, dsp, dy_ld);
+                            want_dres ? bf16_mut(dres) : nullptr, stream_of(x, 0), sp, dsx, dsp, dy_ld, prefin ? 2 : 0);
     return {dx, dres, dw, db};
+}
+
+std::vector<std::vector<at::Tensor>> bn_bwd_finalize(std::vector<FinRequest> reqs) {
+    const char *op = "bn_bwd_finalize";
+    TORCH_CHECK(!reqs.empty(), "bn_bwd_finalize: no requests");
+    const at::Tensor &lead = std::get<0>(reqs[0]);
+    TORCH_CHECK(lead.is_cuda(), "bn_bwd_finalize: sums must be on a GPU");
+    c10::DeviceGuard gd(lead.device());
+    const FinRider fr = fin_rider(op, FinRequests(reqs), Dev(lead.device()));
+    for (int i = 0; i < fr.rider.n; ++i) kfk::launch_bn_bwd_finalize_sums(fr.rider.d[i], stream_of(lead, 0));
+    return fr.out;
 }
 
 std::vector<std::vector<at::Tensor>> bn_backward_multi(std::vector<at::Tensor> dys, std::vector<at::Tensor> xs,
@@ -344,7 +365,10 @@
     m.def("bn_backward", &bn_backward, "fused NHWC BN(+residual)(+ReLU) backward -> (dx, dres, dweight, dbias)",
           py::arg("dy"), py::arg("x"), py::arg("mean"), py::arg("invstd"), py::arg("weight"), py::arg("fcoef"),
           py::arg("mask"), py::arg("relu"), py::arg("training"), py::arg("want_dres"), py::arg("sums") = py::none(),
-          py::arg("dres_x") = py::none(), py::arg("dres_sums") = py::none());
+          py::arg("dres_x") = py::none(), py::arg("dres_sums") = py::none(), py::arg("pre") = py::none());
+    m.def("bn_bwd_finalize", &bn_bwd_finalize,
+          "stand-alone backward sums-finalize of up to two BNs: [(sums, mean, invstd, gamma, rows, training)] -> "
+          "[[dgamma, dbeta, coef], ...] (sums re-zeroed)");
     m.def("bn_pool_supported", [](int64_t C, int64_t H, int64_t W) {
         const char *op = "bn_pool_supported";
         return kfk::bn_pool_supported(kfk::BNShape{H * W, narrow(C, op, "C")}, narrow(H, op, "H"), narrow(W, op, "W"));
diff --git a/csrc/kernels/bind_conv.cpp b/csrc/kernels/bind_conv.cpp
--- a/csrc/kernels/bind_conv.cpp
+++ b/csrc/kernels/bind_conv.cpp
@@ -146,18 +146,23 @@
     return dx;
 }
 
-at::Tensor wgrad_launch(const char *op, const at::Tensor &dy, const at::Tensor &x, const kfk::WgradPlan &plan,
-                        OptTensor out, bool accumulate, bool atomics) {
+py::object wgrad_launch(const char *op, const at::Tensor &dy, const at::Tensor &x, const kfk::WgradPlan &plan,
+                        OptTensor out, bool accumulate, bool atomics, const FinRequests &fin) {
     const kfk::WgradShape &sh = plan.shape;
     const bool f32 = has(out) && out->scalar_type() == at::kFloat;
     c10::DeviceGuard gd(x.device());
+    const FinRider fr = fin_rider(op, fin, Dev(x.device()));
     auto dw = out_or_empty(out, {sh.Cout, sh.Cin, sh.kh, sh.kw},
                            x.options().dtype(f32 ? at::kFloat : at::kBFloat16).memory_format(kCL), op).first;
     at::Tensor ws;
     if (plan.ws_floats > 0) ws = at::empty({plan.ws_floats}, x.options().dtype(at::kFloat));
     kfk::launch_conv_wgrad(bf16(dy), bf16(x), dw.data_ptr(), plan.ws_floats > 0 ? ws.data_ptr<float>() : nullptr, plan,
-                           f32, accumulate, stream_of(x, 0), atomics);
-    return dw;
+                           f32, accumulate, stream_of(x, 0), atomics, &fr.rider);
+    if (!fin) return py::cast(dw);
+    py::tuple res(1 + fr.out.size());
+    res[0] = py::cast(dw);
+    for (size_t i = 0; i < fr.out.size(); ++i) res[1 + i] = py::make_tuple(fr.out[i][0], fr.out[i][1], fr.out[i][2]);
+    return res;
 }
 
 void wgrad_check(const char *op, const at::Tensor &dy, const at::Tensor &x, const kfk::WgradShape &sh) {
@@ -166,8 +171,8 @@
     check_extent32(op, "dy", {sh.N, sh.OH(), sh.OW(), sh.Cout});
 }
 
-at::Tensor conv_wgrad(at::Tensor dy, at::Tensor x, int64_t ks, int64_t stride, OptTensor out, bool accumulate,
-                      int64_t variant, int64_t splits, bool atomics) {
+py::object conv_wgrad(at::Tensor dy, at::Tensor x, int64_t ks, int64_t stride, OptTensor out, bool accumulate,
+                      int64_t variant, int64_t splits, bool atomics, FinRequests fin) {
     const char *op = "conv_wgrad";
     check_cl4(x, op, "x", kAnyGpu);
     check_cl4(dy, op, "dy", Dev(x.device()));
@@ -179,11 +184,11 @@
     TORCH_CHECK(has(out) || !accumulate, "conv_wgrad: accumulate needs out");
     const auto plan = kfk::conv_wgrad_plan(sh, kfk::WgradFamily::Square, narrow(variant, op, "variant"),
                                            narrow(splits, op, "splits"));
-    return wgrad_launch(op, dy, x, plan, out, accumulate, atomics);
-}
-
-at::Tensor conv_wgrad_rect(at::Tensor dy, at::Tensor x, int64_t kh, int64_t kw, int64_t stride, int64_t ph, int64_t pw,
-                           int64_t variant) {
+    return wgrad_launch(op, dy, x, plan, out, accumulate, atomics, fin);
+}
+
+py::object conv_wgrad_rect(at::Tensor dy, at::Tensor x, int64_t kh, int64_t kw, int64_t stride, int64_t ph, int64_t pw,
+                           int64_t variant, FinRequests fin) {
     const char *op = "conv_wgrad_rect";
     check_cl4(x, op, "x", kAnyGpu);
     check_cl4(dy, op, "dy", Dev(x.device()));
@@ -195,7 +200,7 @@
                 "conv_wgrad_rect: unsupported channels/window/stride/padding");
     wgrad_check(op, dy, x, sh);
     const auto plan = kfk::conv_wgrad_plan(sh, kfk::WgradFamily::Rect, narrow(variant, op, "variant"));
-    return wgrad_launch(op, dy, x, plan, OptTensor(), false, true);
+    return wgrad_launch(op, dy, x, plan, OptTensor(), false, true, fin);
 }
 
 at::Tensor conv_flip_weight(at::Tensor w) {
@@ -295,11 +300,12 @@
           py::arg("variant") = -1, py::arg("dh") = 0, py::arg("dw") = 0, py::arg("pad") = 1);
     m.def("conv_wgrad_rect", &conv_wgrad_rect, "weight gradient of a KH x KW padded NHWC bf16 convolution "
           "(split-K MFMA GEMM, any channel count % 8)", py::arg("dy"), py::arg("x"), py::arg("kh"), py::arg("kw"),
-          py::arg("stride") = 1, py::arg("ph") = 0, py::arg("pw") = 0, py::arg("variant") = -1);
+          py::arg("stride") = 1, py::arg("ph") = 0, py::arg("pw") = 0, py::arg("variant") = -1,
+          py::arg("fin") = py::none());
     m.def("conv_wgrad", &conv_wgrad, "weight gradient of the 1x1/3x3 NHWC bf16 convolution (split-K MFMA GEMM)",
           py::arg("dy"), py::arg("x"), py::arg("ks"), py::arg("stride") = 1, py::arg("out") = py::none(),
           py::arg("accumulate") = false, py::arg("variant") = -1, py::arg("splits") = -1,
-          py::arg("atomics") = true);
+          py::arg("atomics") = true, py::arg("fin") = py::none());
     m.def("conv_wgrad_supported", &kfk::conv_wgrad_supported);
     m.def("conv_wgrad_rect_supported", &kfk::conv_wgrad_rect_supported);
     m.def("conv_wgrad_variants", [] { return kfk::kWgradSquareVariants; });
diff --git a/csrc/kernels/bind_util.hpp b/csrc/kernels/bind_util.hpp
--- a/csrc/kernels/bind_util.hpp
+++ b/csrc/kernels/bind_util.hpp
@@ -8,7 +8,9 @@
 
 #include <climits>
 #include <initializer_list>
+#include <tuple>
 #include <utility>
+#include <vector>
 
 namespace kfb {
 
@@ -122,6 +124,37 @@
     return kfk::kEpiBwdCoef;
 }
 
+using FinRequest = std::tuple<at::Tensor, at::Tensor, at::Tensor, at::Tensor, int64_t, bool>;
+using FinRequests = c10::optional<std::vector<FinRequest>>;
+struct FinRider {
+    kfk::BnFinRider rider;
+    std::vector<std::vector<at::Tensor>> out;
+};
+inline FinRider fin_rider(const char *op, const FinRequests &reqs, const Dev &dev) {
+    FinRider f;
+    if (!reqs) return f;
+    TORCH_CHECK(reqs->size() <= static_cast<size_t>(kfk::kFinRiderMax), op, ": fin must be at most ", kfk::kFinRiderMax,
+                " requests (sums, mean, invstd, gamma, rows, training)");
+    for (const auto &[sums, mean, invstd, gamma, rows, training] : *reqs) {
+        const int64_t C = mean.numel();
+        TORCH_CHECK(C > 0 && C <= INT_MAX / (2 * kfk::kStatSlots), op, ": fin mean must have 1 .. 2^26 - 1 channels");
+        TORCH_CHECK(rows > 0, op, ": fin rows must be positive, got ", rows);
+        check_dense(mean, op, "fin mean", dev, at::kFloat, C);
+        check_dense(invstd, op, "fin invstd", dev, at::kFloat, C);
+        check_dense(gamma, op, "fin gamma", dev, at::kFloat, C);
+        kfk::BnBwdSumsDesc &d = f.rider.d[f.rider.n++];
+        d.sums = stats_ptr(OptTensor(sums), op, C, dev, "fin sums");
+        TORCH_CHECK(d.sums, op, ": fin sums must be the f64 statistics workspace");
+        const auto fopt = mean.options();
+        f.out.push_back({at::empty({C}, fopt), at::empty({C}, fopt), at::empty({3 * C}, fopt)});
+        d.gamma = gamma.data_ptr<float>(), d.mean = mean.data_ptr<float>(), d.invstd = invstd.data_ptr<float>();
+        d.dgamma = f.out.back()[0].data_ptr<float>(), d.dbeta = f.out.back()[1].data_ptr<float>();
+        d.coef = f.out.back()[2].data_ptr<float>();
+        d.rows = rows, d.C = static_cast<int>(C), d.training = training;
+    }
+    return f;
+}
+
 inline std::pair<at::Tensor, bool> out_or_empty(const OptTensor &out, at::IntArrayRef sizes, const at::TensorOptions &opt,
                                                 const char *op, const char *name = "out") {
     if (!has(out)) return {at::empty(sizes, opt), false};
diff --git a/csrc/kernels/bn.hip b/csrc/kernels/bn.hip
--- a/csrc/kernels/bn.hip
+++ b/csrc/kernels/bn.hip
@@ -654,34 +654,8 @@
     d.coef[2 * C + c] = -a * static_cast<float>(db) * inv_m - k2 * d.mean[c];
 }
 
-__global__ __launch_bounds__(256) void bn_bwd_finalize_sums(double *__restrict__ sums, int C, int64_t rows,
-                                                            const float *__restrict__ gamma,
-                                                            const float *__restrict__ mean,
-                                                            const float *__restrict__ invstd, float *dgamma,
-                                                            float *dbeta, float *coef, bool training) {
-    const int c = blockIdx.x * blockDim.x + threadIdx.x;
-    if (c >= C) return;
-    const float g = gamma ? gamma[c] : 1.f, mu = mean[c], is = invstd[c];
-    const double *sp = sums + c;
-    double v0[kStatSlots], v1[kStatSlots];
-#pragma unroll
-    for (int k = 0; k < kStatSlots; ++k) {
-        v0[k] = sp[k * 2 * C];
-        v1[k] = sp[k * 2 * C + C];
-    }
-    double s0 = 0, s1 = 0;
-#pragma unroll
-    for (int k = 0; k < kStatSlots; ++k) {
-        s0 += v0[k];
-        s1 += v1[k];
-    }
-    double *zp = sums + c;
-#pragma unroll
-    for (int k = 0; k < kStatSlots; ++k) {
-        zp[k * 2 * C] = 0.0;
-        zp[k * 2 * C + C] = 0.0;
-    }
-    bn_fin_bwd_channel(c, C, s0, s1, rows, g, mu, is, dgamma, dbeta, coef, training);
+__global__ __launch_bounds__(256) void bn_bwd_finalize_sums(BnBwdSumsDesc d) {
+    bn_fin_bwd_sums(d, blockIdx.x * blockDim.x + threadIdx.x, gridDim.x * blockDim.x);
 }
 
 
@@ -832,8 +806,7 @@
     const uint4 *xx = reinterpret_cast<const uint4 *>(x);
     if (phase == 2) {
     } else if (sums) {
-        bn_bwd_finalize_sums<<<(C + 255) / 256, 256, 0, s>>>(sums, C, sh.rows, gamma, mean, invstd, dgamma, dbeta,
-                                                             coef, training);
+        launch_bn_bwd_finalize_sums({sums, gamma, mean, invstd, dgamma, dbeta, coef, sh.rows, C, training}, s);
     } else {
     dispatch_cvec(cvec, [&](auto cvc) {
         constexpr int CV = decltype(cvc)::value;
@@ -880,6 +853,10 @@
 
 }
 
+void launch_bn_bwd_finalize_sums(const BnBwdSumsDesc &d, hipStream_t s) {
+    bn_bwd_finalize_sums<<<(d.C + 255) / 256, 256, 0, s>>>(d);
+}
+
 void launch_bn_bwd_finalize_multi(const BnBwdFinBatch &b, hipStream_t s) {
     if (b.n <= 0) return;
     if (b.n > kBnFinMax) throw std::invalid_argument("bn_bwd_finalize_multi: too many BNs");
diff --git a/csrc/kernels/bn_fin.hpp b/csrc/kernels/bn_fin.hpp
--- a/csrc/kernels/bn_fin.hpp
+++ b/csrc/kernels/bn_fin.hpp
@@ -1,6 +1,8 @@
 #pragma once
 
 #include <hip/hip_runtime.h>
+
+#include "kernels.hpp"
 
 #include <cstdint>
 
@@ -45,4 +47,34 @@
     }
 }
 
+__device__ __forceinline__ void bn_fin_bwd_sums(const BnBwdSumsDesc &d, int tid, int nthreads) {
+    const int C = d.C;
+    for (int c = tid; c < C; c += nthreads) {
+        const float g = d.gamma ? d.gamma[c] : 1.f, mu = d.mean[c], is = d.invstd[c];
+        double *sp = d.sums + c;
+        double v0[kStatSlots], v1[kStatSlots];
+#pragma unroll
+        for (int k = 0; k < kStatSlots; ++k) {
+            v0[k] = sp[k * 2 * C];
+            v1[k] = sp[k * 2 * C + C];
+        }
+        double s0 = 0, s1 = 0;
+#pragma unroll
+        for (int k = 0; k < kStatSlots; ++k) {
+            s0 += v0[k];
+            s1 += v1[k];
+        }
+#pragma unroll
+        for (int k = 0; k < kStatSlots; ++k) {
+            sp[k * 2 * C] = 0.0;
+            sp[k * 2 * C + C] = 0.0;
+        }
+        bn_fin_bwd_channel(c, C, s0, s1, d.rows, g, mu, is, d.dgamma, d.dbeta, d.coef, d.training);
+    }
 }
+
+__device__ __forceinline__ void bn_fin_ride(const BnFinRider &r, int tid, int nthreads) {
+    for (int i = 0; i < r.n && i < kFinRiderMax; ++i) bn_fin_bwd_sums(r.d[i], tid, nthreads);
+}
+
+}
diff --git a/csrc/kernels/conv_wgrad.hip b/csrc/kernels/conv_wgrad.hip
--- a/csrc/kernels/conv_wgrad.hip
+++ b/csrc/kernels/conv_wgrad.hip
@@ -1,3 +1,4 @@
+#include "bn_fin.hpp"
 #include "common.hpp"
 #include "kernels.hpp"
 
@@ -715,16 +716,23 @@
     }
 }
 
-template <int WM, int WN, int TN = 4>
+template <int WM, int WN, int TN = 4, bool FIN = false>
 __global__ __launch_bounds__(256) void wgrad_reduce_kernel(const float *__restrict__ part, void *__restrict__ dw,
-                                                           WGeo g, int out_f32, int accumulate, int sg_log2) {
+                                                           WGeo g, int out_f32, int accumulate, int sg_log2,
+                                                           int fin_blocks, BnFinRider fin) {
+    if constexpr (FIN) {
+        if (static_cast<int>(blockIdx.x) < fin_blocks) {
+            bn_fin_ride(fin, blockIdx.x * 256 + threadIdx.x, fin_blocks * 256);
+            return;
+        }
+    }
     constexpr int BM = 64 * WM, BN = 16 * TN * WN, NT = 64 * WM * WN;
     constexpr int TILE4 = BM * BN / 4;
     __shared__ f32x4 red[256];
     const int SG = 1 << sg_log2, OUT = 256 >> sg_log2;
     const int t = threadIdx.x, o = t & (OUT - 1), sg = t >> (8 - sg_log2);
     const int64_t total = static_cast<int64_t>(g.tiles) * TILE4;
-    const int64_t idx = static_cast<int64_t>(blockIdx.x) * OUT + o;
+    const int64_t idx = static_cast<int64_t>(FIN ? static_cast<int>(blockIdx.x) - fin_blocks : blockIdx.x) * OUT + o;
     const int64_t stride_split = total;
     f32x4 s = f32x4{0.f, 0.f, 0.f, 0.f};
     if (idx < total) {
@@ -773,9 +781,20 @@
 
 
 template <int WM, int WN, int TN = 4>
-void reduce_tiles(const float *part, void *dw, const WGeo &g, bool out_f32, bool accumulate, hipStream_t s) {
+void reduce_tiles(const float *part, void *dw, const WGeo &g, bool out_f32, bool accumulate, hipStream_t s,
+                  const BnFinRider &fin) {
     const WgradReduceLaunch r = wgrad_reduce_launch(static_cast<int64_t>(g.tiles) * (64 * WM) * (16 * TN * WN) / 4, g.splits);
-    wgrad_reduce_kernel<WM, WN, TN><<<r.grid, 256, 0, s>>>(part, dw, g, out_f32, accumulate, r.sg_log2);
+    int cmax = 0;
+    for (int i = 0; i < fin.n; ++i) cmax = fin.d[i].C > cmax ? fin.d[i].C : cmax;
+    const int fb = (cmax + 255) / 256;
+    if (fb > 0)
+        wgrad_reduce_kernel<WM, WN, TN, true><<<r.grid + fb, 256, 0, s>>>(part, dw, g, out_f32, accumulate, r.sg_log2, fb, fin);
+    else
+        wgrad_reduce_kernel<WM, WN, TN, false><<<r.grid, 256, 0, s>>>(part, dw, g, out_f32, accumulate, r.sg_log2, 0, fin);
+}
+
+void finalize_alone(const BnFinRider &fin, hipStream_t s) {
+    for (int i = 0; i < fin.n; ++i) launch_bn_bwd_finalize_sums(fin.d[i], s);
 }
 
 WGeo reduce_geo(int Cin, int Cout, int mtiles, int ntiles, int taps, int tiles, int splits) {
@@ -786,49 +805,50 @@
 
 template <int KS, int S, int WM, int WN, int TN = 4>
 void launch_t(const uint16_t *dy, const uint16_t *x, void *dw, float *part, const WGeo &g, bool out_f32,
-              bool accumulate, bool atomic_out, hipStream_t s) {
+              bool accumulate, bool atomic_out, hipStream_t s, const BnFinRider &fin) {
     constexpr int STAGE_BYTES = 64 * (64 * WM + 16 * TN * WN) * 2;
     constexpr int STAGES = 3 * STAGE_BYTES <= 160 * 1024 ? 3 : 2;
     const int stagger = TN == 8 ? 1 : 0;
     wgrad_kernel<KS, S, WM, WN, STAGES, TN><<<g.tiles * g.splits, 64 * WM * WN, 0, s>>>(
         dy, x, part, dw, reinterpret_cast<const uint16_t *>(zero_page()), g, out_f32, accumulate, atomic_out, stagger);
-    if (g.splits > 1 && !atomic_out) reduce_tiles<WM, WN, TN>(part, dw, g, out_f32, accumulate, s);
+    if (g.splits > 1 && !atomic_out) reduce_tiles<WM, WN, TN>(part, dw, g, out_f32, accumulate, s, fin);
+    else finalize_alone(fin, s);
 }
 
 template <int KS, int S>
 void launch_ks(const uint16_t *dy, const uint16_t *x, void *dw, float *part, const WGeo &g, int variant,
-               bool out_f32, bool accumulate, bool atomic_out, hipStream_t s) {
+               bool out_f32, bool accumulate, bool atomic_out, hipStream_t s, const BnFinRider &fin) {
     switch (variant) {
-    case kWgradTile128x128: launch_t<KS, S, 2, 2>(dy, x, dw, part, g, out_f32, accumulate, atomic_out, s); break;
-    case kWgradTile128x64: launch_t<KS, S, 2, 1>(dy, x, dw, part, g, out_f32, accumulate, atomic_out, s); break;
-    case kWgradTile64x128: launch_t<KS, S, 1, 2>(dy, x, dw, part, g, out_f32, accumulate, atomic_out, s); break;
-    case kWgradTile64x64: launch_t<KS, S, 1, 1>(dy, x, dw, part, g, out_f32, accumulate, atomic_out, s); break;
-    case kWgradTile256x128: launch_t<KS, S, 4, 2>(dy, x, dw, part, g, out_f32, accumulate, atomic_out, s); break;
-    case kWgradTile128x256: launch_t<KS, S, 2, 4>(dy, x, dw, part, g, out_f32, accumulate, atomic_out, s); break;
-    default: launch_t<KS, S, 4, 2, 8>(dy, x, dw, part, g, out_f32, accumulate, atomic_out, s); break;
+    case kWgradTile128x128: launch_t<KS, S, 2, 2>(dy, x, dw, part, g, out_f32, accumulate, atomic_out, s, fin); break;
+    case kWgradTile128x64: launch_t<KS, S, 2, 1>(dy, x, dw, part, g, out_f32, accumulate, atomic_out, s, fin); break;
+    case kWgradTile64x128: launch_t<KS, S, 1, 2>(dy, x, dw, part, g, out_f32, accumulate, atomic_out, s, fin); break;
+    case kWgradTile64x64: launch_t<KS, S, 1, 1>(dy, x, dw, part, g, out_f32, accumulate, atomic_out, s, fin); break;
+    case kWgradTile256x128: launch_t<KS, S, 4, 2>(dy, x, dw, part, g, out_f32, accumulate, atomic_out, s, fin); break;
+    case kWgradTile128x256: launch_t<KS, S, 2, 4>(dy, x, dw, part, g, out_f32, accumulate, atomic_out, s, fin); break;
+    default: launch_t<KS, S, 4, 2, 8>(dy, x, dw, part, g, out_f32, accumulate, atomic_out, s, fin); break;
     }
 }
 
 void launch_tiled(const uint16_t *dy, const uint16_t *x, void *dw, float *part, const WgradPlan &plan, bool out_f32,
-                  bool accumulate, bool atomic_out, hipStream_t s) {
+                  bool accumulate, bool atomic_out, hipStream_t s, const BnFinRider &fin) {
     const WGeo &g = plan.tiled;
     const int64_t P = plan.shape.P();
     if (P * g.HW >= (int64_t(1) << 40) || P >= (1 << 23))
         throw std::invalid_argument("conv_wgrad: too many pixels for the 40-bit division");
     const bool k1 = g.taps == 1 && g.ph == 0 && g.pw == 0, k3 = g.taps == 9 && g.kwin == 3 && g.ph == 1 && g.pw == 1;
     if (plan.shape.stride == 1) {
-        if (k1) launch_ks<1, 1>(dy, x, dw, part, g, plan.variant, out_f32, accumulate, atomic_out, s);
-        else if (k3) launch_ks<3, 1>(dy, x, dw, part, g, plan.variant, out_f32, accumulate, atomic_out, s);
-        else launch_ks<0, 1>(dy, x, dw, part, g, plan.variant, out_f32, accumulate, atomic_out, s);
+        if (k1) launch_ks<1, 1>(dy, x, dw, part, g, plan.variant, out_f32, accumulate, atomic_out, s, fin);
+        else if (k3) launch_ks<3, 1>(dy, x, dw, part, g, plan.variant, out_f32, accumulate, atomic_out, s, fin);
+        else launch_ks<0, 1>(dy, x, dw, part, g, plan.variant, out_f32, accumulate, atomic_out, s, fin);
     } else {
-        if (k1) launch_ks<1, 2>(dy, x, dw, part, g, plan.variant, out_f32, accumulate, atomic_out, s);
-        else if (k3) launch_ks<3, 2>(dy, x, dw, part, g, plan.variant, out_f32, accumulate, atomic_out, s);
-        else launch_ks<0, 2>(dy, x, dw, part, g, plan.variant, out_f32, accumulate, atomic_out, s);
+        if (k1) launch_ks<1, 2>(dy, x, dw, part, g, plan.variant, out_f32, accumulate, atomic_out, s, fin);
+        else if (k3) launch_ks<3, 2>(dy, x, dw, part, g, plan.variant, out_f32, accumulate, atomic_out, s, fin);
+        else launch_ks<0, 2>(dy, x, dw, part, g, plan.variant, out_f32, accumulate, atomic_out, s, fin);
     }
 }
 
 void launch_rows_rect(const uint16_t *dy, const uint16_t *x, void *dw, float *part, const WgradPlan &plan, bool out_f32,
-                      bool accumulate, bool atomic_out, hipStream_t s) {
+                      bool accumulate, bool atomic_out, hipStream_t s, const BnFinRider &fin) {
     const RRGeo &g = plan.rect;
     const int grid = g.mtiles * g.ntiles * g.tgroups * g.splits;
     const uint16_t *z = reinterpret_cast<const uint16_t *>(zero_page());
@@ -852,10 +872,12 @@
     case kWgradRing64x3: t7 ? go(wgrad_rows_rect_kernel<7, 3, 64, true>, 7) : go(wgrad_rows_rect_kernel<9, 3, 64, true>, 9); break;
     default: t7 ? go(wgrad_rows_rect_kernel<7, 4, 64, true>, 7) : go(wgrad_rows_rect_kernel<9, 4, 64, true>, 9); break;
     }
-    if (g.splits == 1 || atomic_out) return;
+    if (g.splits == 1 || atomic_out) return finalize_alone(fin, s);
     if (plan.kernel == WgradKernel::RowsRect) {
-        reduce_tiles<1, 1>(part, dw, reduce_geo(g.C, g.K, g.mtiles, g.ntiles, g.taps, g.tiles, g.splits), out_f32, accumulate, s);
+        reduce_tiles<1, 1>(part, dw, reduce_geo(g.C, g.K, g.mtiles, g.ntiles, g.taps, g.tiles, g.splits), out_f32, accumulate, s,
+                           fin);
     } else {
+        finalize_alone(fin, s);
         const int64_t n = static_cast<int64_t>(g.K) * g.taps * g.C;
         int sgl = 0;
         while (sgl < 6 && (8 << sgl) < g.splits && (n / 4) * (2 << sgl) <= int64_t(1024) * 256) ++sgl;
@@ -868,21 +890,26 @@
 }
 
 void launch_conv_wgrad(const uint16_t *dy, const uint16_t *x, void *dw, float *part, const WgradPlan &plan, bool out_f32,
-                       bool accumulate, hipStream_t s, bool atomics) {
+                       bool accumulate, hipStream_t s, bool atomics, const BnFinRider *finp) {
+    const BnFinRider none{};
+    const BnFinRider &fin = finp ? *finp : none;
+    if (fin.n < 0 || fin.n > kFinRiderMax) throw std::invalid_argument("conv_wgrad: at most two BN finalizes ride on a launch");
     const bool atomic_out = atomics && out_f32 && accumulate && plan.splits > 1;
     if (plan.splits > 1 && !atomic_out && part == nullptr) throw std::invalid_argument("conv_wgrad: split-K needs the workspace");
     switch (plan.kernel) {
-    case WgradKernel::Tiled: launch_tiled(dy, x, dw, part, plan, out_f32, accumulate, atomic_out, s); break;
+    case WgradKernel::Tiled: launch_tiled(dy, x, dw, part, plan, out_f32, accumulate, atomic_out, s, fin); break;
     case WgradKernel::Rows3x3: {
         const RGeo &g = plan.rows;
         wgrad_rows_kernel<2><<<g.mtiles * g.ntiles * g.splits, 576, 0, s>>>(
             dy, x, part, dw, reinterpret_cast<const uint16_t *>(zero_page()), g, out_f32, accumulate, atomic_out, 1);
         if (g.splits > 1 && !atomic_out)
-            reduce_tiles<1, 1>(part, dw, reduce_geo(g.C, g.K, g.mtiles, g.ntiles, 9, g.tiles, g.splits), out_f32, accumulate, s);
+            reduce_tiles<1, 1>(part, dw, reduce_geo(g.C, g.K, g.mtiles, g.ntiles, 9, g.tiles, g.splits), out_f32, accumulate, s,
+                               fin);
+        else finalize_alone(fin, s);
         break;
     }
-    default: launch_rows_rect(dy, x, dw, part, plan, out_f32, accumulate, atomic_out, s); break;
-    }
-}
-
-}
+    default: launch_rows_rect(dy, x, dw, part, plan, out_f32, accumulate, atomic_out, s, fin); break;
+    }
+}
+
+}
diff --git a/csrc/kernels/kernels.hpp b/csrc/kernels/kernels.hpp
--- a/csrc/kernels/kernels.hpp
+++ b/csrc/kernels/kernels.hpp
@@ -162,8 +162,10 @@
 void launch_conv_flip_weight(const uint16_t *w, uint16_t *wt, int Cout, int Cin, int ks, hipStream_t s);
 void launch_conv_flip_weight_taps(const uint16_t *w, uint16_t *wt, int Cout, int Cin, int taps, hipStream_t s);
 
+struct BnFinRider;
 void launch_conv_wgrad(const uint16_t *dy, const uint16_t *x, void *dw, float *part, const WgradPlan &plan,
-                       bool out_f32, bool accumulate, hipStream_t s, bool atomics = true);
+                       bool out_f32, bool accumulate, hipStream_t s, bool atomics = true,
+                       const BnFinRider *fin = nullptr);
 
 void launch_stem_pad4(const uint16_t *x, uint16_t *x4, int64_t npix, hipStream_t s);
 void launch_stem_pad4_f32(const float *x, uint16_t *x4, int64_t npix, hipStream_t s);
@@ -222,6 +224,20 @@
     int n;
 };
 void launch_bn_bwd_finalize_multi(const BnBwdFinBatch &b, hipStream_t s);
+struct BnBwdSumsDesc {
+    double *sums;
+    const float *gamma, *mean, *invstd;
+    float *dgamma, *dbeta, *coef;
+    int64_t rows;
+    int C;
+    bool training;
+};
+void launch_bn_bwd_finalize_sums(const BnBwdSumsDesc &d, hipStream_t s);
+constexpr int kFinRiderMax = 2;
+struct BnFinRider {
+    BnBwdSumsDesc d[kFinRiderMax];
+    int n = 0;
+};
 
 void launch_bn_forward(const uint16_t *x, const uint16_t *res, const float *gamma, const float *beta, uint16_t *y,
                        uint8_t *mask, BNShape sh, bool relu, bool training, float *run_mean, float *run_var,
diff --git a/kungfu_amd/ops/conv.py b/kungfu_amd/ops/conv.py
--- a/kungfu_amd/ops/conv.py
+++ b/kungfu_amd/ops/conv.py
@@ -23,7 +23,18 @@
     return t.dim() == 4 and t.dtype == torch.bfloat16 and t.is_contiguous(memory_format=torch.channels_last)
 
 
-def wgrad(dy: torch.Tensor, x: torch.Tensor, w: torch.Tensor, stride: int, pad) -> torch.Tensor:
+def wgrad(dy: torch.Tensor, x: torch.Tensor, w: torch.Tensor, stride: int, pad, fin=None):
+    if fin is not None:
+        fin = list(fin)
+        if not fin:
+            return wgrad(dy, x, w, stride, pad), []
+        rode = []
+        dw = _wgrad(dy, x, w, stride, pad, fin, rode)
+        return dw, rode[0] if rode else [tuple(t) for t in hip().bn_bwd_finalize(fin)]
+    return _wgrad(dy, x, w, stride, pad, None, None)
+
+
+def _wgrad(dy, x, w, stride, pad, fin, rode):
     stride = int(stride)
     ph, pw = _pair(pad)
     route = "library"
@@ -37,7 +48,11 @@
         per_img = int(dy.shape[2]) * int(dy.shape[3])
         cap = min(_WGRAD_MAX_PIXELS, cap)
         if n * per_img < cap:
-            return hip().conv_wgrad(dy, x, kh, stride, variant=variant)
+            if fin is None:
+                return hip().conv_wgrad(dy, x, kh, stride, variant=variant)
+            dw, *res = hip().conv_wgrad(dy, x, kh, stride, variant=variant, fin=fin)
+            rode.append(res)
+            return dw
         step = max(1, (cap - 1) // per_img)
         acc = torch.zeros(w.shape, dtype=torch.float32, device=x.device).contiguous(
             memory_format=torch.channels_last)
diff --git a/kungfu_amd/ops/fused_block.py b/kungfu_amd/ops/fused_block.py
--- a/kungfu_amd/ops/fused_block.py
+++ b/kungfu_amd/ops/fused_block.py
@@ -24,6 +24,15 @@
 def set_enabled(on: bool) -> bool:
     global _ENABLED
     old, _ENABLED = _ENABLED, bool(on)
+    return old
+
+
+_FIN_RIDER = True
+
+
+def set_fin_rider(on: bool) -> bool:
+    global _FIN_RIDER
+    old, _FIN_RIDER = _FIN_RIDER, bool(on)
     return old
 
 
@@ -39,10 +48,14 @@
     return ws
 
 
-def _wgrad(dy, x, w, stride, pad):
+def _wgrad(dy, x, w, stride, pad, fin=None):
     from .conv import wgrad
 
-    return wgrad(dy, x, w, stride, pad)
+    return wgrad(dy, x, w, stride, pad, fin)
+
+
+def _fin_req(ws, mean, invstd, gamma, y):
+    return (ws, mean, invstd, gamma, y.numel() // y.shape[1], True)
 
 
 class _FlipCache:
@@ -122,12 +135,14 @@
 
 
 class _TailSlot:
-    __slots__ = ("ws", "y3", "mask", "ready", "dx_ptr")
-
-    def __init__(self, ws, y3, mask):
+    __slots__ = ("ws", "y3", "mask", "ready", "dx_ptr", "gamma", "mean", "invstd", "pre")
+
+    def __init__(self, ws, y3, mask, gamma, mean, invstd):
         self.ws, self.y3, self.mask = ws, y3, mask
+        self.gamma, self.mean, self.invstd = gamma, mean, invstd
         self.ready = False
         self.dx_ptr = 0
+        self.pre = None
 
 
 class _Spec:
@@ -173,7 +188,7 @@
             yd = md = idd = cd = None
             out, m3, i3, c3, mask3 = bn(2, y3, x, True)
         ctx.prev = getattr(x, "_kf_tail", None)
-        ctx.tail = _TailSlot(_sums(spec.bns[2], dev), y3, mask3)
+        ctx.tail = _TailSlot(_sums(spec.bns[2], dev), y3, mask3, gam[2].detach(), m3, i3)
         ctx.spec = spec
         ctx.wdtypes = [w.dtype for w in ws[0::3]]
         ctx.save_for_backward(x, y1, z1, y2, z2, y3, yd, *ws_bf, *gam, m1, i1, c1, m2, i2, c2, m3, i3, c3, mask3,
@@ -204,33 +219,49 @@
         ws = [_sums(b, dout.device) for b in spec.bns]
         tail = ctx.tail
         use3 = tail.ready and dout.data_ptr() == tail.dx_ptr
-        if tail.ready and not use3:
+        pre3 = tail.pre if use3 else None
+        if tail.ready and not use3 and tail.pre is None:
             tail.ws.zero_()
-        tail.ready, tail.y3, tail.mask = False, None, None
+        tail.ready, tail.y3, tail.mask, tail.pre = False, None, None, None
+        tail.gamma = tail.mean = tail.invstd = None
+        rider = _FIN_RIDER
         in_place = use3 and not spec.ds
         dy3, didt, dg3, db3 = H.bn_backward(dout, y3, m3, i3, g[2], c3, mask3, True, True, not in_place,
-                                            ws[2] if use3 else None, dres_x=yd if spec.ds else None,
-                                            dres_sums=ws[3] if spec.ds else None)
+                                            ws[2] if use3 and pre3 is None else None,
+                                            dres_x=yd if spec.ds else None, dres_sums=ws[3] if spec.ds else None,
+                                            pre=pre3)
         dbn[2] = (dg3, db3)
         if _CAPTURE is not None:
             _capture(spec.bns[2], "mask", dout, y3, m3, i3, mask3, dg3, db3)
         dz2 = _dgrad(dy3, z2, w[2], 1, 0, flipped=fl[2], bn=(ws[1], y2, c2, None))
-        dw[2] = wgrad(dy3, z2, w[2], 1, 0)
-        dy2, _, dg2, db2 = H.bn_backward(dz2, y2, m2, i2, g[1], c2, None, True, True, False, ws[1])
+        pre2 = pred = None
+        if rider:
+            reqs = [_fin_req(ws[1], m2, i2, g[1], y2)] + ([_fin_req(ws[3], md, idd, g[3], yd)] if spec.ds else [])
+            dw[2], fins = wgrad(dy3, z2, w[2], 1, 0, reqs)
+            pre2, pred = fins[0], (fins[1] if spec.ds else None)
+        else:
+            dw[2] = wgrad(dy3, z2, w[2], 1, 0)
+        dy2, _, dg2, db2 = H.bn_backward(dz2, y2, m2, i2, g[1], c2, None, True, True, False,
+                                         ws[1] if pre2 is None else None, pre=pre2)
         dbn[1] = (dg2, db2)
         if _CAPTURE is not None:
             _capture(spec.bns[1], "relu", dz2, y2, m2, i2, c2, dg2, db2)
         dz1 = _dgrad(dy2, z1, w[1], s, 1, flipped=fl[1], bn=(ws[0], y1, c1, None))
         fused1 = _dgrad.fused
-        dw[1] = wgrad(dy2, z1, w[1], s, 1)
+        pre1 = None
+        if rider and fused1:
+            dw[1], (pre1,) = wgrad(dy2, z1, w[1], s, 1, [_fin_req(ws[0], m1, i1, g[0], y1)])
+        else:
+            dw[1] = wgrad(dy2, z1, w[1], s, 1)
         dy1, _, dg1, db1 = H.bn_backward(dz1, y1, m1, i1, g[0], c1, None, True, True, False,
-                                         ws[0] if fused1 else None)
+                                         ws[0] if fused1 and pre1 is None else None, pre=pre1)
         dbn[0] = (dg1, db1)
         if _CAPTURE is not None:
             _capture(spec.bns[0], "relu", dz1, y1, m1, i1, c1, dg1, db1)
         acc_even = False
         if spec.ds:
-            dyd, _, dgd, dbd = H.bn_backward(didt, yd, md, idd, g[3], cd, None, False, True, False, ws[3])
+            dyd, _, dgd, dbd = H.bn_backward(didt, yd, md, idd, g[3], cd, None, False, True, False,
+                                             ws[3] if pred is None else None, pre=pred)
             dbn[3] = (dgd, dbd)
             if _CAPTURE is not None:
                 _capture(spec.bns[3], "plain", didt, yd, md, idd, None, dgd, dbd)
@@ -250,9 +281,14 @@
             dx = _dgrad(dy1, x, w[0], 1, 0, out=dx, flipped=fl[0], bn=(prev.ws, prev.y3, None, prev.mask),
                         out_mask=om, acc_even=acc_even)
             prev.ready, prev.dx_ptr = True, dx.data_ptr()
+            if rider:
+                dw[0], (prev.pre,) = wgrad(dy1, x, w[0], 1, 0,
+                                           [_fin_req(prev.ws, prev.mean, prev.invstd, prev.gamma, prev.y3)])
+            else:
+                dw[0] = wgrad(dy1, x, w[0], 1, 0)
         else:
             dx = _dgrad(dy1, x, w[0], 1, 0, out=dx, flipped=fl[0], out_mask=om, acc_even=acc_even)
-        dw[0] = wgrad(dy1, x, w[0], 1, 0)
+            dw[0] = wgrad(dy1, x, w[0], 1, 0)
         grads: List[Optional[torch.Tensor]] = []
         for i in range(nb):
             gw = dw[i]
```

Result: no change. 12890, median of 6 (+0.7%).
